# nianticlabs/mickey

Hardware: NVIDIA H100
Metric: image-pairs/sec @720x540 (higher is better)
Workload: dtype f16 operands / f32 accumulate (tensor core), f32 matcher+solver

## Files before the change

include/mickey_b200.h:

```cpp
#ifndef MICKEY_B200_H
#define MICKEY_B200_H

#ifdef __cplusplus
extern "C" {
#endif

typedef struct mk_handle mk_handle;

typedef struct mk_config {
  int embed_dim, depth, heads;
  int down_factor;
  int block_dims[4];
  int desc_dim;
  int use_softmax;
  int depth_sigmoid;
  float max_depth;
  int kp_pos_enc, dsc_pos_enc;
  int norm_dsc;
  float temperature;
  int use_dustbin;
  int it_matches, it_ransac;
  int num_sampled, num_corr, num_refine;
  float th_inlier, th_soft_inlier;
} mk_config;

int mk_create(int device, const mk_config* cfg, mk_handle** out);
int mk_destroy(mk_handle* h);
const char* mk_last_error(void);
const char* mk_version(void);
int mk_sizeof(const char* type);

int mk_set_tensor(mk_handle* h, const char* name, const void* ptr_dev, int dtype, long long numel);
int mk_finalize(mk_handle* h, int img_h, int img_w);

long long mk_workspace_bytes(mk_handle* h, int n_pairs, int img_h, int img_w);
long long mk_workspace_bytes_for(mk_handle* h, int n_img, int n_pairs, int img_h, int img_w);
long long mk_workspace_offset(mk_handle* h, const char* name, int n_pairs, int img_h, int img_w);

int mk_extract(mk_handle* h, const float* images_dev, int n_pairs, int img_h, int img_w, float* kps_dev,
               float* depth_dev, float* scr_dev, float* dsc_dev, void* ws_dev, long long ws_bytes, void* stream);

int mk_extract_u8(mk_handle* h, const unsigned char* images_u8_dev, int n_pairs, int img_h, int img_w, float* kps_dev,
                  float* depth_dev, float* scr_dev, float* dsc_dev, void* ws_dev, long long ws_bytes, void* stream);

int mk_extract_images(mk_handle* h, const float* images_dev, int n_img, int img_h, int img_w, float* kps_dev,
                      float* depth_dev, float* scr_dev, float* dsc_dev, void* ws_dev, long long ws_bytes, void* stream);
int mk_extract_images_u8(mk_handle* h, const unsigned char* images_u8_dev, int n_img, int img_h, int img_w, float* kps_dev,
                         float* depth_dev, float* scr_dev, float* dsc_dev, void* ws_dev, long long ws_bytes, void* stream);

long long mk_backbone_ws_bytes(mk_handle* h, int n_img, int img_h, int img_w);
int mk_backbone_features(mk_handle* h, const float* images_dev, int n_img, int img_h, int img_w, float* out_dev,
                         void* ws_dev, long long ws_bytes, void* stream);

int mk_match(mk_handle* h, int n_pairs, float* scores_dev, float* kp_scores_dev, float* final_scores_dev, long long nn_pitch,
             void* ws_dev, long long ws_bytes, void* stream);

int mk_solve_pose(mk_handle* h, const float* final_scores_dev, long long nn_pitch, const float* kps_dev, const float* depth_dev,
                  const float* K0_dev, const float* K1_dev, int n_pairs, int n_kpts, unsigned long long seed,
                  const int* outer_idx_dev, const int* inner_idx_dev, float* pose_dev, int* best_set_dev,
                  float* inlier_mask_dev, int* sampled_idx_out_dev, float* hyp_scores_out_dev, int* status_dev,
                  void* ws_dev, long long ws_bytes, void* stream);

long long mk_procrustes_ws_bytes(int B, int N, int it_matches, int it_ransac, int num_sampled);
int mk_procrustes_solve(const float* final_scores_dev, long long nn_pitch, const float* kps_dev, const float* depth_dev,
                        const float* K0_dev, const float* K1_dev, int B, int N, int it_matches, int it_ransac,
                        int num_sampled, int num_corr, int num_refine, float th_inlier, float th_soft_inlier,
                        unsigned long long seed, const int* outer_idx_dev, const int* inner_idx_dev, float* pose_dev,
                        int* best_set_dev, float* inlier_mask_dev, int* sampled_idx_out_dev, float* hyp_scores_out_dev,
                        int* status_dev, void* ws_dev, long long ws_bytes, void* stream);

#define MK_VCRE_POINTS 196
#define MK_MAPFREE_MAX_FRAMES 67108863
int mk_mapfree_frame_metrics(const double* q_est_dev, const double* t_est_dev, const double* q_gt_dev,
                             const double* t_gt_dev, const double* K_dev, const double* grid_dev, int P, int W, int H,
                             double* err_dev, void* stream);

int mk_forward(mk_handle* h, const float* images_dev, const float* K0_dev, const float* K1_dev, int n_pairs,
               int img_h, int img_w, unsigned long long seed, float* kps_dev, float* depth_dev, float* scr_dev,
               float* dsc_dev, float* scores_dev, float* kp_scores_dev, float* final_scores_dev, long long nn_pitch,
               float* pose_dev, int* best_set_dev, float* inlier_mask_dev, int* sampled_idx_out_dev, int* status_dev,
               void* ws_dev, long long ws_bytes, void* stream);

int mk_forward_u8(mk_handle* h, const unsigned char* images_u8_dev, const float* K0_dev, const float* K1_dev, int n_pairs,
                  int img_h, int img_w, unsigned long long seed, float* kps_dev, float* depth_dev, float* scr_dev,
                  float* dsc_dev, float* scores_dev, float* kp_scores_dev, float* final_scores_dev, long long nn_pitch,
                  float* pose_dev, int* best_set_dev, float* inlier_mask_dev, int* sampled_idx_out_dev, int* status_dev,
                  void* ws_dev, long long ws_bytes, void* stream);

int mk_forward_pairs(mk_handle* h, const float* kps0_dev, const float* depth0_dev, const float* scr0_dev, const float* dsc0_dev,
                     int n0, const float* kps1_dev, const float* depth1_dev, const float* scr1_dev, const float* dsc1_dev, int n1,
                     const int* idx0_dev, const int* idx1_dev, const float* K0_dev, const float* K1_dev, int n_pairs,
                     unsigned long long seed, float* kps_dev, float* depth_dev, float* scores_dev, float* kp_scores_dev,
                     float* final_scores_dev, long long nn_pitch, float* pose_dev, int* best_set_dev, float* inlier_mask_dev,
                     int* sampled_idx_out_dev, int* status_dev, void* ws_dev, long long ws_bytes, void* stream);

int mk_pose_to_submission(const float* pose_dev, int n_pairs, double* out_dev, void* stream);

int mk_mutual_matches(const float* scores_dev, long long nn_pitch, int B, int N, float min_conf, int* matches_dev,
                      float* match_scores_dev, int* count_dev, void* ws_dev, long long ws_bytes, void* stream);
long long mk_mutual_matches_ws_bytes(int B, int N);

#define MK_LOSS_STATUS_PRECHECK 16
#define MK_LOSS_STATUS_INNER 32
int mk_loss_search(const float* final_scores_dev, long long nn_pitch, const float* kps0_dev, const float* depth0_dev,
                   const float* kps1_dev, const float* depth1_dev, const float* K0_dev, const float* K1_dev, int B, int N,
                   int it_matches, int it_ransac, int n_sample, int n_corr, int n_ref, float th_ref, unsigned long long seed,
                   const int* outer_idx_dev, const int* inner_idx_dev, int* sampled_idx_out_dev, int* inner_idx_out_dev,
                   unsigned int* inliers_out_dev, int* status_dev, void* ws_dev, long long ws_bytes, void* stream);
long long mk_loss_search_ws_bytes(int B, int it_matches);
int mk_loss_gradient(const int* sampled_idx_dev, const float* loss_value_dev, const float* baseline_dev, const float* mask_topk_dev,
                     int B, int N, int it_matches, int n_sample, float* probs_grad_dev, void* ws_dev, long long ws_bytes,
                     void* stream);
long long mk_loss_gradient_ws_bytes(int B, int it_matches, int n_sample);

long long mk_dual_softmax_ws_bytes(int B, int N);
long long mk_dual_softmax_backward_ws_bytes(int B, int N);
int mk_dual_softmax(const float* dsc0_dev, const float* dsc1_dev, const float* scr0_dev, const float* scr1_dev,
                    const float* dustbin_dev, float temperature, int B, int N, int unit_norm, float* scores_dev,
                    float* kp_scores_dev, float* final_scores_dev, long long nn_pitch, float* lse_r_dev, float* lse_c_dev,
                    void* ws_dev, long long ws_bytes, void* stream);
int mk_dual_softmax_backward(const float* dsc0_dev, const float* dsc1_dev, const float* scr0_dev, const float* scr1_dev,
                             const float* dustbin_dev, float temperature, int B, int N, const float* lse_r_dev,
                             const float* lse_c_dev, const float* grad_scores_dev, long long gs_pitch, const float* grad_kp_dev,
                             long long gk_pitch, const float* grad_final_dev, long long gf_pitch, float* ddsc0_dev,
                             float* ddsc1_dev, float* dscr0_dev, float* dscr1_dev, float* ddustbin_dev, void* ws_dev,
                             long long ws_bytes, void* stream);

typedef struct mk_htr_layer {
  const float* q_proj; const float* k_proj; const float* v_proj; const float* merge; const float* mlp0; const float* mlp2;
  const float* norm1_w; const float* norm1_b; const float* norm2_w; const float* norm2_b;
} mk_htr_layer;
typedef struct mk_htr_layer_grads {
  float* q_proj; float* k_proj; float* v_proj; float* merge; float* mlp0; float* mlp2;
  float* norm1_w; float* norm1_b; float* norm2_w; float* norm2_b;
} mk_htr_layer_grads;
long long mk_head_transformer_ws_bytes(int B, int h, int w, int num_layers, int save);
long long mk_head_transformer_backward_ws_bytes(int B, int h, int w, int num_layers);
int mk_head_transformer(const float* x_dev, const float* pe_dev, int B, int h, int w, const mk_htr_layer* layers_host,
                        int num_layers, float* out_dev, int save, void* ws_dev, long long ws_bytes, void* stream);
int mk_head_transformer_backward(const void* saved_dev, const float* grad_out_dev, int B, int h, int w,
                                 const mk_htr_layer* layers_host, int num_layers, float* grad_x_dev,
                                 mk_htr_layer_grads* grads_host, void* ws_dev, long long ws_bytes, void* stream);

#define MK_RB_TRAIN 1
#define MK_RB_RELU 2
#define MK_RB_SAVE 4
#define MK_RB_BN 8
#define MK_RB_GRAD_X 1
#define MK_RB_GRAD_W1 2
#define MK_RB_GRAD_W2 4
#define MK_RB_GRAD_WSC 8
#define MK_RB_GRAD_BN1_W 16
#define MK_RB_GRAD_BN1_B 32
#define MK_RB_GRAD_BN2_W 64
#define MK_RB_GRAD_BN2_B 128
typedef struct mk_resblock_params {
  const float* w1; const float* w2; const float* wsc;
  const float* bn1_w; const float* bn1_b; float* bn1_mean; float* bn1_var;
  const float* bn2_w; const float* bn2_b; float* bn2_mean; float* bn2_var;
  float eps1, eps2, momentum1, momentum2;
} mk_resblock_params;
typedef struct mk_resblock_grads {
  float* dx; float* w1; float* w2; float* wsc; float* bn1_w; float* bn1_b; float* bn2_w; float* bn2_b;
} mk_resblock_grads;
long long mk_resblock_ws_bytes(int B, int h, int w, int cin, int cout);
long long mk_resblock_saved_bytes(int B, int h, int w, int cin, int cout);
long long mk_resblock_backward_ws_bytes(int B, int h, int w, int cin, int cout);
int mk_resblock_forward(const float* x_dev, const long long* x_strides_host, int B, int h, int w, int cin, int cout,
                        const mk_resblock_params* params_host, int flags, float* out_dev, void* saved_dev,
                        long long saved_bytes, void* ws_dev, long long ws_bytes, void* stream);
int mk_resblock_backward(const void* saved_dev, const float* grad_out_dev, const long long* g_strides_host,
                         const float* out_dev, int B, int h, int w, int cin, int cout, const mk_resblock_params* params_host,
                         int flags, int want, const mk_resblock_grads* grads_host, void* ws_dev, long long ws_bytes,
                         void* stream);

#define MK_HO_SCORE_SOFTMAX 0
#define MK_HO_SCORE_SIGMOID 1
#define MK_HO_OFFSET 2
#define MK_HO_DEPTH 3
#define MK_HO_DEPTH_SIGMOID 4
#define MK_HO_DESC_L2 5
long long mk_head_out_backward_ws_bytes(int kind, int B, int h, int w, int C);
int mk_head_out_forward(int kind, const float* x_dev, const long long* x_strides_host, int B, int C, int h, int w,
                        const float* weight_dev, const float* eps_dev, float temperature, float max_depth, float* out_dev,
                        float* norm_dev, void* stream);
int mk_head_out_backward(int kind, const float* x_dev, const long long* x_strides_host, int B, int C, int h, int w,
                         const float* weight_dev, float temperature, float max_depth, const float* out_dev,
                         const float* norm_dev, const float* grad_out_dev, float* grad_x_dev, float* grad_w_dev, void* ws_dev,
                         long long ws_bytes, void* stream);

int mk_set_seed(mk_handle* h, unsigned long long seed, void* stream);

long long mk_launch_count(mk_handle* h);
int mk_pdl_enabled(void);
int mk_profile_enable(mk_handle* h, int enable);
int mk_profile_read(mk_handle* h, char* buf, int buf_bytes);

typedef struct mk_gemm_args {
  int epi;
  int impl;
  const void* a; long long a_rows, a_cols, a_ld;
  const void* b; long long b_rows, b_cols, b_ld;
  int M, N, k_chunks, chunks_per_tap, num_taps;
  int tap_shift[9];
  int groups, a_row_group_off, a_col_group_off, a_col_base, b_row_group_off;
  int act;
  const float* bias; int bias_group_off;
  const float* gamma; const float* beta; int ln_group_off;
  float* out_f; long long out_f_ld, out_f_group_off;
  void* out_h; long long out_h_ld, out_h_group_off;
  const void* res_h; long long res_h_ld, res_h_group_off;
  const float* aux; int aux_group_mask;
  int pad_h2, pad_w2, tok_per_img;
  float eps;
  int n_valid; float inv_temp;
  const float* dustbin;
  float* part_row; float* part_col; int part_ld;
  const float* lse_r; const float* lse_c;
  const float* scr0; const float* scr1;
  float* scores; float* kp_scores; float* final_scores;
  float lse_bound;
  long long out_pitch;
} mk_gemm_args;

int mk_op_gemm(const mk_gemm_args* args, void* stream);
int mk_op_patch_gather(const float* img, void* patches_h, int n_img, int H, int W, int kpad, float* x_f,
                       const float* cls_pos, int D, void* stream);
int mk_op_ingest_u8(const unsigned char* img_u8, void* patches_h, int n_img, int H, int W, int kpad, float* x_f,
                    const float* cls_pos, int D, void* stream);
int mk_op_layernorm(const float* x, const float* w, const float* b, void* out_h, int rows, int D, float eps, int mode,
                    int gh, int gw, void* stream);
int mk_op_attention(const void* qkv_h, void* out_h, int n_img, int T, int D, int heads, int impl, void* stream);
int mk_op_linattn(const float* qkv_f, float* kv_part_f, float* kv_f, void* msg_h, int n_img, int G, int h2, int w2, float eps,
                  void* stream);
int mk_op_matcher_reduce(const float* part_row, const float* part_col, const float* dustbin, int B, int N, int part_ld,
                         float* lse_r, float* lse_c, void* stream);
int mk_op_sample(const float* final_scores, int B, int N, long long pitch, int IM, int n_sample, unsigned long long seed, void* ws,
                 long long ws_bytes, int* idx_out, int* status, void* stream);
long long mk_op_sample_workspace_bytes(int B, int IM);
int mk_op_kabsch(const double* H, double* R, int n, void* stream);

int mk_resblock_layout(int B, int h, int w, int cin, int cout, long long* saved_off, long long* bwd_off);
long long mk_op_conv_tf32_ws_bytes(int mode, int B, int h, int w, int cin, int cout, int taps);
int mk_op_conv_tf32(int mode, const float* a, const float* b, float* out, int B, int h, int w, int cin, int cout, int taps,
                    void* ws, long long ws_bytes, void* stream);

#ifdef __cplusplus
}
#endif
#endif
```

mickey_b200/_lib.py:

```python
from __future__ import annotations

import ctypes as C
import math
import os

import torch

_HERE = os.path.dirname(os.path.abspath(__file__))
LIB_PATH = os.path.join(_HERE, "_C", "libmickey_b200.so")


class MkConfig(C.Structure):
    _fields_ = [
        ("embed_dim", C.c_int), ("depth", C.c_int), ("heads", C.c_int),
        ("down_factor", C.c_int),
        ("block_dims", C.c_int * 4),
        ("desc_dim", C.c_int),
        ("use_softmax", C.c_int), ("depth_sigmoid", C.c_int), ("max_depth", C.c_float),
        ("kp_pos_enc", C.c_int), ("dsc_pos_enc", C.c_int), ("norm_dsc", C.c_int),
        ("temperature", C.c_float), ("use_dustbin", C.c_int),
        ("it_matches", C.c_int), ("it_ransac", C.c_int),
        ("num_sampled", C.c_int), ("num_corr", C.c_int), ("num_refine", C.c_int),
        ("th_inlier", C.c_float), ("th_soft_inlier", C.c_float),
    ]


class MkGemmArgs(C.Structure):
    _fields_ = [
        ("epi", C.c_int), ("impl", C.c_int),
        ("a", C.c_void_p), ("a_rows", C.c_longlong), ("a_cols", C.c_longlong), ("a_ld", C.c_longlong),
        ("b", C.c_void_p), ("b_rows", C.c_longlong), ("b_cols", C.c_longlong), ("b_ld", C.c_longlong),
        ("M", C.c_int), ("N", C.c_int), ("k_chunks", C.c_int), ("chunks_per_tap", C.c_int), ("num_taps", C.c_int),
        ("tap_shift", C.c_int * 9),
        ("groups", C.c_int), ("a_row_group_off", C.c_int), ("a_col_group_off", C.c_int), ("a_col_base", C.c_int),
        ("b_row_group_off", C.c_int),
        ("act", C.c_int),
        ("bias", C.c_void_p), ("bias_group_off", C.c_int),
        ("gamma", C.c_void_p), ("beta", C.c_void_p), ("ln_group_off", C.c_int),
        ("out_f", C.c_void_p), ("out_f_ld", C.c_longlong), ("out_f_group_off", C.c_longlong),
        ("out_h", C.c_void_p), ("out_h_ld", C.c_longlong), ("out_h_group_off", C.c_longlong),
        ("res_h", C.c_void_p), ("res_h_ld", C.c_longlong), ("res_h_group_off", C.c_longlong),
        ("aux", C.c_void_p), ("aux_group_mask", C.c_int),
        ("pad_h2", C.c_int), ("pad_w2", C.c_int), ("tok_per_img", C.c_int),
        ("eps", C.c_float),
        ("n_valid", C.c_int), ("inv_temp", C.c_float),
        ("dustbin", C.c_void_p),
        ("part_row", C.c_void_p), ("part_col", C.c_void_p), ("part_ld", C.c_int),
        ("lse_r", C.c_void_p), ("lse_c", C.c_void_p), ("scr0", C.c_void_p), ("scr1", C.c_void_p),
        ("scores", C.c_void_p), ("kp_scores", C.c_void_p), ("final_scores", C.c_void_p),
        ("lse_bound", C.c_float),
        ("out_pitch", C.c_longlong),
    ]


class MkHtrLayer(C.Structure):
    _fields_ = [(n, C.c_void_p) for n in ("q_proj", "k_proj", "v_proj", "merge", "mlp0", "mlp2",
                                          "norm1_w", "norm1_b", "norm2_w", "norm2_b")]


MkHtrLayerGrads = MkHtrLayer


class MkResblockParams(C.Structure):
    _fields_ = [(n, C.c_void_p) for n in ("w1", "w2", "wsc", "bn1_w", "bn1_b", "bn1_mean", "bn1_var",
                                          "bn2_w", "bn2_b", "bn2_mean", "bn2_var")] + \
               [(n, C.c_float) for n in ("eps1", "eps2", "momentum1", "momentum2")]


class MkResblockGrads(C.Structure):
    _fields_ = [(n, C.c_void_p) for n in ("dx", "w1", "w2", "wsc", "bn1_w", "bn1_b", "bn2_w", "bn2_b")]


EXPORTS = {
    "mk_create": (C.c_int, [C.c_int, C.POINTER(MkConfig), C.POINTER(C.c_void_p)]),
    "mk_destroy": (C.c_int, [C.c_void_p]),
    "mk_last_error": (C.c_char_p, []),
    "mk_version": (C.c_char_p, []),
    "mk_sizeof": (C.c_int, [C.c_char_p]),
    "mk_set_tensor": (C.c_int, [C.c_void_p, C.c_char_p, C.c_void_p, C.c_int, C.c_longlong]),
    "mk_finalize": (C.c_int, [C.c_void_p, C.c_int, C.c_int]),
    "mk_workspace_bytes": (C.c_longlong, [C.c_void_p, C.c_int, C.c_int, C.c_int]),
    "mk_workspace_offset": (C.c_longlong, [C.c_void_p, C.c_char_p, C.c_int, C.c_int, C.c_int]),
    "mk_extract": (C.c_int, [C.c_void_p, C.c_void_p, C.c_int, C.c_int, C.c_int, C.c_void_p, C.c_void_p, C.c_void_p,
                             C.c_void_p, C.c_void_p, C.c_longlong, C.c_void_p]),
    "mk_extract_u8": (C.c_int, [C.c_void_p, C.c_void_p, C.c_int, C.c_int, C.c_int, C.c_void_p, C.c_void_p, C.c_void_p,
                                C.c_void_p, C.c_void_p, C.c_longlong, C.c_void_p]),
    "mk_workspace_bytes_for": (C.c_longlong, [C.c_void_p, C.c_int, C.c_int, C.c_int, C.c_int]),
    "mk_extract_images": (C.c_int, [C.c_void_p, C.c_void_p, C.c_int, C.c_int, C.c_int, C.c_void_p, C.c_void_p, C.c_void_p,
                                    C.c_void_p, C.c_void_p, C.c_longlong, C.c_void_p]),
    "mk_extract_images_u8": (C.c_int, [C.c_void_p, C.c_void_p, C.c_int, C.c_int, C.c_int, C.c_void_p, C.c_void_p, C.c_void_p,
                                       C.c_void_p, C.c_void_p, C.c_longlong, C.c_void_p]),
    "mk_forward_pairs": (C.c_int, [C.c_void_p, C.c_void_p, C.c_void_p, C.c_void_p, C.c_void_p, C.c_int,
                                   C.c_void_p, C.c_void_p, C.c_void_p, C.c_void_p, C.c_int,
                                   C.c_void_p, C.c_void_p, C.c_void_p, C.c_void_p, C.c_int, C.c_ulonglong,
                                   C.c_void_p, C.c_void_p, C.c_void_p, C.c_void_p, C.c_void_p, C.c_longlong,
                                   C.c_void_p, C.c_void_p, C.c_void_p, C.c_void_p, C.c_void_p, C.c_void_p, C.c_longlong,
                                   C.c_void_p]),
    "mk_backbone_ws_bytes": (C.c_longlong, [C.c_void_p, C.c_int, C.c_int, C.c_int]),
    "mk_backbone_features": (C.c_int, [C.c_void_p, C.c_void_p, C.c_int, C.c_int, C.c_int, C.c_void_p, C.c_void_p,
                                       C.c_longlong, C.c_void_p]),
    "mk_match": (C.c_int, [C.c_void_p, C.c_int, C.c_void_p, C.c_void_p, C.c_void_p, C.c_longlong, C.c_void_p, C.c_longlong, C.c_void_p]),
    "mk_solve_pose": (C.c_int, [C.c_void_p, C.c_void_p, C.c_longlong, C.c_void_p, C.c_void_p, C.c_void_p, C.c_void_p, C.c_int, C.c_int,
                                C.c_ulonglong, C.c_void_p, C.c_void_p, C.c_void_p, C.c_void_p, C.c_void_p, C.c_void_p,
                                C.c_void_p, C.c_void_p, C.c_void_p, C.c_longlong, C.c_void_p]),
    "mk_procrustes_ws_bytes": (C.c_longlong, [C.c_int, C.c_int, C.c_int, C.c_int, C.c_int]),
    "mk_procrustes_solve": (C.c_int, [C.c_void_p, C.c_longlong, C.c_void_p, C.c_void_p, C.c_void_p, C.c_void_p, C.c_int,
                                      C.c_int, C.c_int, C.c_int, C.c_int, C.c_int, C.c_int, C.c_float, C.c_float,
                                      C.c_ulonglong, C.c_void_p, C.c_void_p, C.c_void_p, C.c_void_p, C.c_void_p,
                                      C.c_void_p, C.c_void_p, C.c_void_p, C.c_void_p, C.c_longlong, C.c_void_p]),
    "mk_mapfree_frame_metrics": (C.c_int, [C.c_void_p, C.c_void_p, C.c_void_p, C.c_void_p, C.c_void_p, C.c_void_p,
                                           C.c_int, C.c_int, C.c_int, C.c_void_p, C.c_void_p]),
    "mk_forward": (C.c_int, [C.c_void_p, C.c_void_p, C.c_void_p, C.c_void_p, C.c_int, C.c_int, C.c_int, C.c_ulonglong,
                             C.c_void_p, C.c_void_p, C.c_void_p, C.c_void_p, C.c_void_p, C.c_void_p, C.c_void_p, C.c_longlong,
                             C.c_void_p, C.c_void_p, C.c_void_p, C.c_void_p, C.c_void_p, C.c_void_p, C.c_longlong,
                             C.c_void_p]),
    "mk_forward_u8": (C.c_int, [C.c_void_p, C.c_void_p, C.c_void_p, C.c_void_p, C.c_int, C.c_int, C.c_int, C.c_ulonglong,
                                C.c_void_p, C.c_void_p, C.c_void_p, C.c_void_p, C.c_void_p, C.c_void_p, C.c_void_p, C.c_longlong,
                                C.c_void_p, C.c_void_p, C.c_void_p, C.c_void_p, C.c_void_p, C.c_void_p, C.c_longlong,
                                C.c_void_p]),
    "mk_mutual_matches": (C.c_int, [C.c_void_p, C.c_longlong, C.c_int, C.c_int, C.c_float, C.c_void_p, C.c_void_p,
                                    C.c_void_p, C.c_void_p, C.c_longlong, C.c_void_p]),
    "mk_mutual_matches_ws_bytes": (C.c_longlong, [C.c_int, C.c_int]),
    "mk_loss_search": (C.c_int, [C.c_void_p, C.c_longlong, C.c_void_p, C.c_void_p, C.c_void_p, C.c_void_p, C.c_void_p,
                                 C.c_void_p, C.c_int, C.c_int, C.c_int, C.c_int, C.c_int, C.c_int, C.c_int, C.c_float,
                                 C.c_ulonglong, C.c_void_p, C.c_void_p, C.c_void_p, C.c_void_p, C.c_void_p, C.c_void_p,
                                 C.c_void_p, C.c_longlong, C.c_void_p]),
    "mk_loss_search_ws_bytes": (C.c_longlong, [C.c_int, C.c_int]),
    "mk_loss_gradient": (C.c_int, [C.c_void_p, C.c_void_p, C.c_void_p, C.c_void_p, C.c_int, C.c_int, C.c_int, C.c_int,
                                   C.c_void_p, C.c_void_p, C.c_longlong, C.c_void_p]),
    "mk_loss_gradient_ws_bytes": (C.c_longlong, [C.c_int, C.c_int, C.c_int]),
    "mk_dual_softmax_ws_bytes": (C.c_longlong, [C.c_int, C.c_int]),
    "mk_dual_softmax_backward_ws_bytes": (C.c_longlong, [C.c_int, C.c_int]),
    "mk_dual_softmax": (C.c_int, [C.c_void_p, C.c_void_p, C.c_void_p, C.c_void_p, C.c_void_p, C.c_float, C.c_int, C.c_int,
                                  C.c_int, C.c_void_p, C.c_void_p, C.c_void_p, C.c_longlong, C.c_void_p, C.c_void_p,
                                  C.c_void_p, C.c_longlong, C.c_void_p]),
    "mk_dual_softmax_backward": (C.c_int, [C.c_void_p, C.c_void_p, C.c_void_p, C.c_void_p, C.c_void_p, C.c_float, C.c_int,
                                           C.c_int, C.c_void_p, C.c_void_p, C.c_void_p, C.c_longlong, C.c_void_p,
                                           C.c_longlong, C.c_void_p, C.c_longlong, C.c_void_p, C.c_void_p, C.c_void_p,
                                           C.c_void_p, C.c_void_p, C.c_void_p, C.c_longlong, C.c_void_p]),
    "mk_head_transformer_ws_bytes": (C.c_longlong, [C.c_int, C.c_int, C.c_int, C.c_int, C.c_int]),
    "mk_head_transformer_backward_ws_bytes": (C.c_longlong, [C.c_int, C.c_int, C.c_int, C.c_int]),
    "mk_head_transformer": (C.c_int, [C.c_void_p, C.c_void_p, C.c_int, C.c_int, C.c_int, C.POINTER(MkHtrLayer), C.c_int,
                                      C.c_void_p, C.c_int, C.c_void_p, C.c_longlong, C.c_void_p]),
    "mk_head_transformer_backward": (C.c_int, [C.c_void_p, C.c_void_p, C.c_int, C.c_int, C.c_int, C.POINTER(MkHtrLayer),
                                               C.c_int, C.c_void_p, C.POINTER(MkHtrLayerGrads), C.c_void_p, C.c_longlong,
                                               C.c_void_p]),
    "mk_resblock_ws_bytes": (C.c_longlong, [C.c_int, C.c_int, C.c_int, C.c_int, C.c_int]),
    "mk_resblock_saved_bytes": (C.c_longlong, [C.c_int, C.c_int, C.c_int, C.c_int, C.c_int]),
    "mk_resblock_backward_ws_bytes": (C.c_longlong, [C.c_int, C.c_int, C.c_int, C.c_int, C.c_int]),
    "mk_resblock_forward": (C.c_int, [C.c_void_p, C.POINTER(C.c_longlong), C.c_int, C.c_int, C.c_int, C.c_int, C.c_int,
                                      C.POINTER(MkResblockParams), C.c_int, C.c_void_p, C.c_void_p, C.c_longlong,
                                      C.c_void_p, C.c_longlong, C.c_void_p]),
    "mk_resblock_layout": (C.c_int, [C.c_int, C.c_int, C.c_int, C.c_int, C.c_int, C.POINTER(C.c_longlong),
                                     C.POINTER(C.c_longlong)]),
    "mk_resblock_backward": (C.c_int, [C.c_void_p, C.c_void_p, C.POINTER(C.c_longlong), C.c_void_p, C.c_int, C.c_int,
                                       C.c_int, C.c_int, C.c_int, C.POINTER(MkResblockParams), C.c_int, C.c_int,
                                       C.POINTER(MkResblockGrads), C.c_void_p, C.c_longlong, C.c_void_p]),
    "mk_head_out_backward_ws_bytes": (C.c_longlong, [C.c_int, C.c_int, C.c_int, C.c_int, C.c_int]),
    "mk_head_out_forward": (C.c_int, [C.c_int, C.c_void_p, C.POINTER(C.c_longlong), C.c_int, C.c_int, C.c_int, C.c_int,
                                      C.c_void_p, C.c_void_p, C.c_float, C.c_float, C.c_void_p, C.c_void_p, C.c_void_p]),
    "mk_head_out_backward": (C.c_int, [C.c_int, C.c_void_p, C.POINTER(C.c_longlong), C.c_int, C.c_int, C.c_int, C.c_int,
                                       C.c_void_p, C.c_float, C.c_float, C.c_void_p, C.c_void_p, C.c_void_p, C.c_void_p,
                                       C.c_void_p, C.c_void_p, C.c_longlong, C.c_void_p]),
    "mk_pose_to_submission": (C.c_int, [C.c_void_p, C.c_int, C.c_void_p, C.c_void_p]),
    "mk_launch_count": (C.c_longlong, [C.c_void_p]),
    "mk_pdl_enabled": (C.c_int, []),
    "mk_set_seed": (C.c_int, [C.c_void_p, C.c_ulonglong, C.c_void_p]),
    "mk_profile_enable": (C.c_int, [C.c_void_p, C.c_int]),
    "mk_profile_read": (C.c_int, [C.c_void_p, C.c_char_p, C.c_int]),
    "mk_op_gemm": (C.c_int, [C.POINTER(MkGemmArgs), C.c_void_p]),
    "mk_op_patch_gather": (C.c_int, [C.c_void_p, C.c_void_p, C.c_int, C.c_int, C.c_int, C.c_int, C.c_void_p, C.c_void_p,
                                     C.c_int, C.c_void_p]),
    "mk_op_ingest_u8": (C.c_int, [C.c_void_p, C.c_void_p, C.c_int, C.c_int, C.c_int, C.c_int, C.c_void_p, C.c_void_p,
                                  C.c_int, C.c_void_p]),
    "mk_op_layernorm": (C.c_int, [C.c_void_p, C.c_void_p, C.c_void_p, C.c_void_p, C.c_int, C.c_int, C.c_float, C.c_int,
                                  C.c_int, C.c_int, C.c_void_p]),
    "mk_op_attention": (C.c_int, [C.c_void_p, C.c_void_p, C.c_int, C.c_int, C.c_int, C.c_int, C.c_int, C.c_void_p]),
    "mk_op_linattn": (C.c_int, [C.c_void_p, C.c_void_p, C.c_void_p, C.c_void_p, C.c_int, C.c_int, C.c_int, C.c_int, C.c_float, C.c_void_p]),
    "mk_op_matcher_reduce": (C.c_int, [C.c_void_p, C.c_void_p, C.c_void_p, C.c_int, C.c_int, C.c_int, C.c_void_p, C.c_void_p, C.c_void_p]),
    "mk_op_sample": (C.c_int, [C.c_void_p, C.c_int, C.c_int, C.c_longlong, C.c_int, C.c_int, C.c_ulonglong, C.c_void_p, C.c_longlong,
                               C.c_void_p, C.c_void_p, C.c_void_p]),
    "mk_op_sample_workspace_bytes": (C.c_longlong, [C.c_int, C.c_int]),
    "mk_op_kabsch": (C.c_int, [C.c_void_p, C.c_void_p, C.c_int, C.c_void_p]),
    "mk_op_conv_tf32_ws_bytes": (C.c_longlong, [C.c_int, C.c_int, C.c_int, C.c_int, C.c_int, C.c_int, C.c_int]),
    "mk_op_conv_tf32": (C.c_int, [C.c_int, C.c_void_p, C.c_void_p, C.c_void_p, C.c_int, C.c_int, C.c_int, C.c_int, C.c_int,
                                  C.c_int, C.c_void_p, C.c_longlong, C.c_void_p]),
}

STRUCTS = {"mk_config": MkConfig, "mk_gemm_args": MkGemmArgs, "mk_htr_layer": MkHtrLayer,
           "mk_htr_layer_grads": MkHtrLayerGrads, "mk_resblock_params": MkResblockParams,
           "mk_resblock_grads": MkResblockGrads}

_lib = None


class MickeyB200Error(RuntimeError):
    pass


def load():
    global _lib
    if _lib is not None:
        return _lib
    if not os.path.exists(LIB_PATH):
        raise MickeyB200Error(
            f"{LIB_PATH} not found. Build it with `python -m mickey_b200.build` (needs nvcc; sm_90a only). "
            "mickey_b200 has no CPU or PyTorch fallback.")
    lib = C.CDLL(LIB_PATH)
    for name, (res, args) in EXPORTS.items():
        fn = getattr(lib, name)
        fn.restype = res
        fn.argtypes = args
    sizes = {name: (lib.mk_sizeof(name.encode()), C.sizeof(st)) for name, st in STRUCTS.items()}
    bad = [f"{name} {lib_size} vs {py_size}" for name, (lib_size, py_size) in sizes.items() if lib_size != py_size]
    if bad:
        raise MickeyB200Error("ctypes struct layout does not match the library (stale build?): " + ", ".join(bad))
    _lib = lib
    return lib


def check(rc: int, what: str = ""):
    if rc != 0:
        msg = load().mk_last_error().decode(errors="replace")
        raise MickeyB200Error(f"{what} failed (code {rc}): {msg}")


def ptr(t):
    return None if t is None else C.c_void_p(t.data_ptr())


def stream(dev=None):
    return C.c_void_p(torch.cuda.current_stream(dev).cuda_stream)


def workspace(nbytes, dev, what: str):
    nbytes = int(nbytes)
    if nbytes < 0:
        raise MickeyB200Error(f"{what} returned {nbytes}: {load().mk_last_error().decode(errors='replace')}")
    return torch.empty(max(nbytes, 1), dtype=torch.uint8, device=dev)


def pitched(t):
    B, N, _ = t.shape
    s0, s1, s2 = t.stride()
    if s2 == 1 and s1 >= N and (B == 1 or s0 == N * s1):
        return t, s1
    return t.contiguous(), N


class Handle:

    def __init__(self, device, cfg: MkConfig):
        self.lib = load()
        self.device = device
        h = C.c_void_p()
        check(self.lib.mk_create(device.index or 0, C.byref(cfg), C.byref(h)), "mk_create")
        self.h = h

    def __del__(self):
        try:
            if getattr(self, "h", None):
                self.lib.mk_destroy(self.h)
        except Exception:
            pass

    def register(self, name: str, t):
        assert t.is_contiguous() and t.device == self.device
        dt = {torch.float32: 0, torch.float16: 1}[t.dtype]
        check(self.lib.mk_set_tensor(self.h, name.encode(), ptr(t), dt, t.numel()), f"mk_set_tensor({name})")

    def workspace_view(self, ws, n_pairs: int, H: int, W: int, name: str, dtype, shape):
        off = self.lib.mk_workspace_offset(self.h, name.encode(), n_pairs, H, W)
        if off < 0:
            raise MickeyB200Error(self.lib.mk_last_error().decode())
        nbytes = math.prod(shape) * torch.empty((), dtype=dtype).element_size()
        return ws[off:off + nbytes].view(dtype).reshape(shape)
```

mickey_b200/csrc/engine.cu:

```cuda
#include "../../include/mickey_b200.h"
#include "gemm.h"
#include "ops.h"

#include <algorithm>
#include <cfloat>
#include <cstring>
#include <string>
#include <unordered_map>
#include <vector>

using namespace mk;

struct Tensor { const void* ptr; int dtype; long long numel; };

struct mk_handle {
  int device;
  mk_config cfg;
  std::unordered_map<std::string, Tensor> tensors;
  int geo_h = 0, geo_w = 0;
  bool finalized = false;
  unsigned long long* seed_dev = nullptr;
  long long launches = 0;
  bool profiling = false;
  struct ProfRec { std::string tag; cudaEvent_t e0, e1; };
  std::vector<ProfRec> prof;
};

namespace {

struct Geo {
  int H, W, gh, gw, N, T, h2, w2, per_img, n_img, n_pairs;
  long long M, Mp, R;
};

Geo make_geo(int n_img, int n_pairs, int H, int W) {
  Geo g;
  g.H = H; g.W = W; g.gh = H / 14; g.gw = W / 14;
  g.N = g.gh * g.gw; g.T = g.N + 1; g.h2 = g.gh + 2; g.w2 = g.gw + 2; g.per_img = g.h2 * g.w2;
  g.n_img = n_img; g.n_pairs = n_pairs;
  g.M = (long long)g.n_img * g.T; g.Mp = (long long)g.n_img * g.N; g.R = (long long)g.n_img * g.per_img;
  return g;
}

constexpr int KPAD = 640;
constexpr int G = 4;

struct Carver {
  uint8_t* base; size_t off = 0;
  explicit Carver(void* b) : base(reinterpret_cast<uint8_t*>(b)) {}
  template <typename T> T* take(size_t count) {
    off = (off + 255) & ~(size_t)255;
    T* p = base ? reinterpret_cast<T*>(base + off) : nullptr;
    off += count * sizeof(T);
    return p;
  }
};

struct SolverWs { void* samp_ws; int* idx; float* hyp_scores; float* hyp_Rt; int* status; int* best_hyp; };

void carve_solver(Carver& cv, int n_pairs, int it_matches, int it_ransac, int num_sampled, SolverWs& s) {
  const size_t streams = (size_t)n_pairs * it_matches;
  s.samp_ws = cv.take<uint8_t>(sampler_workspace_bytes(n_pairs, it_matches));
  s.idx = cv.take<int>(streams * num_sampled);
  s.hyp_scores = cv.take<float>(streams * it_ransac);
  s.hyp_Rt = cv.take<float>(streams * it_ransac * 12);
  s.status = cv.take<int>(SOLVER_COUNTER_BASE + n_pairs);
  s.best_hyp = cv.take<int>(n_pairs);
}

struct Workspace {
  __half* P; float* X; __half* XN; __half* QKV; __half* ATT; __half* H1;
  __half* F; __half *T1, *S1, *O1, *T2, *S2, *O2, *T3, *S3, *CAT, *MSG, *HM, *T4k, *S4k, *T4d;
  float *X32, *QKV32, *KV, *KVP, *Y4k, *Y4d;
  float* score_raw; __half* DSCX; float* nrm2; float* scr_copy;
  float *part_row, *part_col, *lse_r, *lse_c;
  SolverWs sol;
  size_t bytes;
};

void carve_backbone(Carver& cv, const mk_config& c, const Geo& g, Workspace& w) {
  const size_t D = c.embed_dim, M = g.M;
  w.P = cv.take<__half>((size_t)g.Mp * KPAD);
  w.X = cv.take<float>(M * D);
  w.XN = cv.take<__half>(M * D);
  w.QKV = cv.take<__half>(M * 3 * D);
  w.ATT = cv.take<__half>(M * D);
  w.H1 = cv.take<__half>(M * 4 * D);
}

size_t backbone_ws_bytes(const mk_config& c, const Geo& g) {
  Carver cv(nullptr);
  Workspace w;
  carve_backbone(cv, c, g, w);
  return (cv.off + 255) & ~(size_t)255;
}

Workspace carve(void* base, const mk_config& c, const Geo& g) {
  Workspace w;
  Carver cv(base);
  const int n_pairs = g.n_pairs;
  const size_t D = c.embed_dim, R = g.R;
  const size_t n_op = (size_t)std::max(g.n_img, 2 * g.n_pairs);
  const int* bd = c.block_dims;
  carve_backbone(cv, c, g, w);
  w.F = cv.take<__half>(R * D);
  w.T1 = cv.take<__half>(R * G * bd[0]); w.S1 = cv.take<__half>(R * G * bd[0]); w.O1 = cv.take<__half>(R * G * bd[0]);
  w.T2 = cv.take<__half>(R * G * bd[1]); w.S2 = cv.take<__half>(R * G * bd[1]); w.O2 = cv.take<__half>(R * G * bd[1]);
  w.T3 = cv.take<__half>(R * G * bd[2]); w.S3 = cv.take<__half>(R * G * bd[2]);
  w.CAT = cv.take<__half>(R * G * 256); w.MSG = cv.take<__half>(R * G * 128); w.HM = cv.take<__half>(R * G * 256);
  w.T4k = cv.take<__half>(R * 3 * bd[3]); w.S4k = cv.take<__half>(R * 3 * bd[3]); w.T4d = cv.take<__half>(R * c.desc_dim);
  w.X32 = cv.take<float>(R * G * 128); w.QKV32 = cv.take<float>(R * G * 384);
  w.KV = cv.take<float>((size_t)g.n_img * G * 8 * 272);
  w.KVP = cv.take<float>((size_t)g.n_img * G * linattn_kv_chunks(g.h2, g.w2) * 8 * 272);
  w.Y4k = cv.take<float>(R * 3 * bd[3]); w.Y4d = cv.take<float>(R * c.desc_dim);
  w.score_raw = cv.take<float>((size_t)g.n_img * g.N);
  w.DSCX = cv.take<__half>(n_op * g.N * 384);
  w.nrm2 = cv.take<float>((size_t)g.n_img * g.N);
  w.scr_copy = cv.take<float>(n_op * g.N);
  const size_t npad = (size_t)ceil_div(g.N, 128) * 128;
  w.part_row = cv.take<float>((size_t)n_pairs * (npad / 64) * npad * 2); w.part_col = cv.take<float>((size_t)n_pairs * (npad / 32) * npad * 2);
  w.lse_r = cv.take<float>((size_t)n_pairs * npad); w.lse_c = cv.take<float>((size_t)n_pairs * npad);
  carve_solver(cv, n_pairs, c.it_matches, c.it_ransac, c.num_sampled, w.sol);
  w.bytes = cv.off + 256;
  return w;
}

struct Lookup {
  mk_handle* h; bool ok = true;
  const void* get(const std::string& name, int dtype, long long numel) {
    auto it = h->tensors.find(name);
    if (it == h->tensors.end()) { set_last_error("missing tensor '%s'", name.c_str()); ok = false; return nullptr; }
    if (it->second.dtype != dtype || it->second.numel != numel) {
      set_last_error("tensor '%s': expected dtype %d numel %lld, got dtype %d numel %lld", name.c_str(), dtype, numel,
                     it->second.dtype, it->second.numel);
      ok = false; return nullptr;
    }
    return it->second.ptr;
  }
  const float* f(const std::string& n, long long numel) { return reinterpret_cast<const float*>(get(n, 0, numel)); }
  const __half* hh(const std::string& n, long long numel) { return reinterpret_cast<const __half*>(get(n, 1, numel)); }
};

GemmParams base_params(long long M, int N, int K) {
  GemmParams p;
  memset(&p, 0, sizeof(p));
  p.M = (int)M; p.N = N; p.k_chunks = K / 64; p.chunks_per_tap = p.k_chunks; p.num_taps = 1; p.groups = 1;
  return p;
}

void set_conv_taps(GemmParams& p, int cin, int w2, bool three) {
  p.chunks_per_tap = cin / 64;
  if (three) {
    p.num_taps = 9;
    for (int ky = 0; ky < 3; ++ky)
      for (int kx = 0; kx < 3; ++kx) p.tap_shift[ky * 3 + kx] = (ky - 1) * w2 + (kx - 1);
  } else {
    p.num_taps = 1; p.tap_shift[0] = 0;
  }
  p.k_chunks = p.num_taps * p.chunks_per_tap;
}

struct ProfScope {
  mk_handle* h; cudaStream_t st; int slot = -1;
  ProfScope(mk_handle* h_, const char* tag, cudaStream_t st_) : h(h_), st(st_) {
    if (!h || !h->profiling) return;
    mk_handle::ProfRec r;
    r.tag = tag;
    if (cudaEventCreate(&r.e0) != cudaSuccess || cudaEventCreate(&r.e1) != cudaSuccess) return;
    cudaEventRecord(r.e0, st);
    h->prof.push_back(r);
    slot = (int)h->prof.size() - 1;
  }
  ~ProfScope() { if (slot >= 0) cudaEventRecord(h->prof[slot].e1, st); }
};

int gemm(mk_handle* h, const char* tag, int epi, const void* a, long long a_rows, long long a_cols, const void* b,
         long long b_rows, long long b_cols, const GemmParams& p, cudaStream_t st) {
  GemmOperand A{a, a_rows, a_cols, a_cols}, B{b, b_rows, b_cols, b_cols};
  h->launches++;
  ProfScope ps(h, tag, st);
  return launch_gemm(epi, A, B, p, st);
}
#define MK_KERNEL(tag, call) do { ProfScope ps_(h, tag, st); h->launches++; MK_TRY(call); } while (0)

int run_backbone(mk_handle* h, const void* images, int img_fmt, const Geo& g, Workspace& w, cudaStream_t st) {
  const mk_config& c = h->cfg;
  const int H = g.H, W = g.W;
  const int D = c.embed_dim;
  Lookup L{h};
  if (img_fmt == 1)
    MK_KERNEL("vit.ingest_u8", ingest_u8(reinterpret_cast<const uint8_t*>(images), w.P, g.n_img, H, W, KPAD, w.X, L.f("patch.clspos", D), D, st));
  else
    MK_KERNEL("vit.patch_gather", patch_gather(reinterpret_cast<const float*>(images), w.P, g.n_img, H, W, KPAD, w.X, L.f("patch.clspos", D), D, st));
  {
    GemmParams p = base_params(g.Mp, D, KPAD);
    p.aux = L.f("patch.posb", (long long)g.N * D); p.tok_per_img = g.N; p.out_f = w.X; p.out_f_ld = D;
    const __half* wt = L.hh("patch.w", (long long)D * KPAD);
    if (!L.ok) return MK_ERR_MISSING_TENSOR;
    MK_TRY(gemm(h, "vit.patch_embed", EPI_PATCH, w.P, g.Mp, KPAD, wt, D, KPAD, p, st));
  }
  const bool fuse_ln = gemm_resid_ln_supported((int)g.M, D, D / 64) && gemm_resid_ln_supported((int)g.M, D, 4 * D / 64);
  for (int i = 0; i < c.depth; ++i) {
    const std::string b = "blk" + std::to_string(i) + ".";
    const float *ln1w = L.f(b + "ln1.w", D), *ln1b = L.f(b + "ln1.b", D), *ln2w = L.f(b + "ln2.w", D), *ln2b = L.f(b + "ln2.b", D);
    const __half *wqkv = L.hh(b + "qkv.w", 3LL * D * D), *wproj = L.hh(b + "proj.w", (long long)D * D);
    const __half *wfc1 = L.hh(b + "fc1.w", 4LL * D * D), *wfc2 = L.hh(b + "fc2.w", 4LL * D * D);
    const float *bqkv = L.f(b + "qkv.b", 3 * D), *bproj = L.f(b + "proj.b", D), *bfc1 = L.f(b + "fc1.b", 4 * D), *bfc2 = L.f(b + "fc2.b", D);
    const float *ls1 = L.f(b + "ls1", D), *ls2 = L.f(b + "ls2", D);
    if (!L.ok) return MK_ERR_MISSING_TENSOR;
    if (i == 0 || !fuse_ln) MK_KERNEL("vit.layernorm", layernorm(w.X, ln1w, ln1b, w.XN, (int)g.M, D, 1e-6f, 0, 0, 0, st));
    { GemmParams p = base_params(g.M, 3 * D, D); p.bias = bqkv; p.out_h = w.QKV; p.out_h_ld = 3 * D;
      MK_TRY(gemm(h, "vit.qkv", EPI_STORE_H, w.XN, g.M, D, wqkv, 3 * D, D, p, st)); }
    MK_KERNEL("vit.attention", attention_dispatch(w.QKV, w.ATT, g.n_img, g.T, D, c.heads, 0, st));
    { GemmParams p = base_params(g.M, D, D); p.bias = bproj; p.gamma = ls1; p.out_f = w.X; p.out_f_ld = D;
      if (fuse_ln) { p.aux = ln2w; p.beta = ln2b; p.out_h = w.XN; p.out_h_ld = D; p.eps = 1e-6f; }
      MK_TRY(gemm(h, "vit.proj", fuse_ln ? EPI_RESID_LN : EPI_RESID_F, w.ATT, g.M, D, wproj, D, D, p, st)); }
    if (!fuse_ln) MK_KERNEL("vit.layernorm", layernorm(w.X, ln2w, ln2b, w.XN, (int)g.M, D, 1e-6f, 0, 0, 0, st));
    { GemmParams p = base_params(g.M, 4 * D, D); p.bias = bfc1; p.act = ACT_GELU; p.out_h = w.H1; p.out_h_ld = 4 * D;
      MK_TRY(gemm(h, "vit.fc1", EPI_STORE_H, w.XN, g.M, D, wfc1, 4 * D, D, p, st)); }
    { GemmParams p = base_params(g.M, D, 4 * D); p.bias = bfc2; p.gamma = ls2; p.out_f = w.X; p.out_f_ld = D;
      const bool fuse_next = fuse_ln && i + 1 < c.depth;
      if (fuse_next) {
        const std::string nb = "blk" + std::to_string(i + 1) + ".";
        p.aux = L.f(nb + "ln1.w", D); p.beta = L.f(nb + "ln1.b", D); p.out_h = w.XN; p.out_h_ld = D; p.eps = 1e-6f;
        if (!L.ok) return MK_ERR_MISSING_TENSOR;
      }
      MK_TRY(gemm(h, "vit.fc2", fuse_next ? EPI_RESID_LN : EPI_RESID_F, w.H1, g.M, 4 * D, wfc2, D, 4 * D, p, st)); }
  }
  return MK_OK;
}

int run_extract(mk_handle* h, const void* images, int img_fmt, const Geo& g, float* kps, float* depth, float* scr,
                float* dsc, Workspace& w, cudaStream_t st) {
  const mk_config& c = h->cfg;
  const int D = c.embed_dim;
  Lookup L{h};
  MK_TRY(run_backbone(h, images, img_fmt, g, w, st));
  MK_CUDA_CHECK(cudaMemsetAsync(w.F, 0, (size_t)g.R * D * sizeof(__half), st));
  MK_KERNEL("vit.layernorm", layernorm(w.X, L.f("norm.w", D), L.f("norm.b", D), w.F, (int)g.M, D, 1e-6f, 1, g.gh, g.gw, st));
  if (!L.ok) return MK_ERR_MISSING_TENSOR;

  const int* bd = c.block_dims;
  struct Rb { const char* name; const __half* in; int cin; int in_goff; __half *T, *S, *O; int cout; };
  const Rb rbs[3] = {{"rb1", w.F, D, 0, w.T1, w.S1, w.O1, bd[0]},
                     {"rb2", w.O1, bd[0], bd[0], w.T2, w.S2, w.O2, bd[1]},
                     {"rb3", w.O2, bd[1], bd[1], w.T3, w.S3, nullptr, bd[2]}};
  if (bd[2] != 128) { set_last_error("KP_HEADS.BLOCKS_DIM[2] must be 128 (transformer width)"); return MK_ERR_UNSUPPORTED; }
  for (int r = 0; r < 3; ++r) {
    const Rb& rb = rbs[r];
    const std::string n = std::string(rb.name) + ".";
    const long long in_cols = (r == 0) ? D : (long long)G * rb.cin;
    const __half *wc1 = L.hh(n + "c1.w", (long long)G * rb.cout * 9 * rb.cin), *wsc = L.hh(n + "sc.w", (long long)G * rb.cout * rb.cin);
    const __half* wc2 = L.hh(n + "c2.w", (long long)G * rb.cout * 9 * rb.cout);
    const float *b1 = L.f(n + "c1.b", G * rb.cout), *b2 = L.f(n + "c2.b", G * rb.cout);
    if (!L.ok) return MK_ERR_MISSING_TENSOR;
    {
      GemmParams p = base_params(g.R, rb.cout, 64); set_conv_taps(p, rb.cin, g.w2, true);
      p.groups = G; p.a_col_group_off = rb.in_goff; p.b_row_group_off = rb.cout; p.bias = b1; p.bias_group_off = rb.cout;
      p.act = ACT_RELU; p.pad_h2 = g.h2; p.pad_w2 = g.w2; p.out_h = rb.T; p.out_h_ld = (long long)G * rb.cout; p.out_h_group_off = rb.cout;
      MK_TRY(gemm(h, "head.conv3x3", EPI_CONV, rb.in, g.R, in_cols, wc1, (long long)G * rb.cout, 9LL * rb.cin, p, st));
    }
    {
      GemmParams p = base_params(g.R, rb.cout, 64); set_conv_taps(p, rb.cin, g.w2, false);
      p.groups = G; p.a_col_group_off = rb.in_goff; p.b_row_group_off = rb.cout;
      p.out_h = rb.S; p.out_h_ld = (long long)G * rb.cout; p.out_h_group_off = rb.cout;
      MK_TRY(gemm(h, "head.conv1x1", EPI_CONV, rb.in, g.R, in_cols, wsc, (long long)G * rb.cout, rb.cin, p, st));
    }
    {
      GemmParams p = base_params(g.R, rb.cout, 64); set_conv_taps(p, rb.cout, g.w2, true);
      p.groups = G; p.a_col_group_off = rb.cout; p.b_row_group_off = rb.cout; p.bias = b2; p.bias_group_off = rb.cout;
      p.res_h = rb.S; p.res_h_ld = (long long)G * rb.cout; p.res_h_group_off = rb.cout;
      p.act = ACT_RELU; p.pad_h2 = g.h2; p.pad_w2 = g.w2;
      if (r < 2) { p.out_h = rb.O; p.out_h_ld = (long long)G * rb.cout; p.out_h_group_off = rb.cout; }
      else {
        p.out_h = w.CAT; p.out_h_ld = G * 256; p.out_h_group_off = 256;
        p.out_f = w.X32; p.out_f_ld = G * 128; p.out_f_group_off = 128;
        p.aux = L.f("head.pe", (long long)g.per_img * 128);
        p.aux_group_mask = (c.kp_pos_enc ? 0x7 : 0) | (c.dsc_pos_enc ? 0x8 : 0);
        if (!L.ok) return MK_ERR_MISSING_TENSOR;
      }
      MK_TRY(gemm(h, "head.conv3x3", EPI_CONV, rb.T, g.R, (long long)G * rb.cout, wc2, (long long)G * rb.cout, 9LL * rb.cout, p, st));
    }
  }
  for (int l = 0; l < 3; ++l) {
    const std::string n = "att" + std::to_string(l) + ".";
    const __half *wqkv = L.hh(n + "qkv.w", (long long)G * 384 * 128), *wmerge = L.hh(n + "merge.w", (long long)G * 128 * 128);
    const __half *wm0 = L.hh(n + "mlp0.w", (long long)G * 256 * 256), *wm2 = L.hh(n + "mlp2.w", (long long)G * 128 * 256);
    const float *n1w = L.f(n + "n1.w", G * 128), *n1b = L.f(n + "n1.b", G * 128), *n2w = L.f(n + "n2.w", G * 128), *n2b = L.f(n + "n2.b", G * 128);
    if (!L.ok) return MK_ERR_MISSING_TENSOR;
    { GemmParams p = base_params(g.R, 384, 128); p.groups = G; p.a_col_group_off = 256; p.b_row_group_off = 384;
      p.out_f = w.QKV32; p.out_f_ld = G * 384; p.out_f_group_off = 384;
      MK_TRY(gemm(h, "head.att.qkv", EPI_STORE_F, w.CAT, g.R, G * 256, wqkv, G * 384, 128, p, st)); }
    { ProfScope ps_(h, "head.att.kv", st); h->launches += 2; MK_TRY(linattn_kv(w.QKV32, w.KVP, w.KV, g.n_img, G, g.h2, g.w2, st)); }
    MK_KERNEL("head.att.msg", linattn_msg(w.QKV32, w.KV, w.MSG, g.n_img, G, g.h2, g.w2, 1e-6f, st));
    { GemmParams p = base_params(g.R, 128, 128); p.groups = G; p.a_col_group_off = 128; p.b_row_group_off = 128;
      p.gamma = n1w; p.beta = n1b; p.ln_group_off = 128; p.eps = 1e-5f;
      p.out_h = w.CAT + 128; p.out_h_ld = G * 256; p.out_h_group_off = 256;
      MK_TRY(gemm(h, "head.att.merge_ln", EPI_LN, w.MSG, g.R, G * 128, wmerge, G * 128, 128, p, st)); }
    { GemmParams p = base_params(g.R, 256, 256); p.groups = G; p.a_col_group_off = 256; p.b_row_group_off = 256; p.act = ACT_RELU;
      p.out_h = w.HM; p.out_h_ld = G * 256; p.out_h_group_off = 256;
      MK_TRY(gemm(h, "head.att.mlp0", EPI_STORE_H, w.CAT, g.R, G * 256, wm0, G * 256, 256, p, st)); }
    { GemmParams p = base_params(g.R, 128, 256); p.groups = G; p.a_col_group_off = 256; p.b_row_group_off = 128;
      p.gamma = n2w; p.beta = n2b; p.ln_group_off = 128; p.eps = 1e-5f;
      p.out_f = w.X32; p.out_f_ld = G * 128; p.out_f_group_off = 128;
      p.out_h = w.CAT; p.out_h_ld = G * 256; p.out_h_group_off = 256;
      if (l == 2) { p.pad_h2 = g.h2; p.pad_w2 = g.w2; }
      MK_TRY(gemm(h, "head.att.mlp2_ln", EPI_LN, w.HM, g.R, G * 256, wm2, G * 128, 256, p, st)); }
  }
  {
    const int co = bd[3];
    const __half *wc1 = L.hh("rb4k.c1.w", 3LL * co * 9 * 128), *wsc = L.hh("rb4k.sc.w", 3LL * co * 128), *wc2 = L.hh("rb4k.c2.w", 3LL * co * 9 * co);
    const float *b1 = L.f("rb4k.c1.b", 3 * co), *b2 = L.f("rb4k.c2.b", 3 * co);
    if (!L.ok) return MK_ERR_MISSING_TENSOR;
    { GemmParams p = base_params(g.R, co, 64); set_conv_taps(p, 128, g.w2, true);
      p.groups = 3; p.a_col_group_off = 256; p.b_row_group_off = co; p.bias = b1; p.bias_group_off = co; p.act = ACT_RELU;
      p.pad_h2 = g.h2; p.pad_w2 = g.w2; p.out_h = w.T4k; p.out_h_ld = 3 * co; p.out_h_group_off = co;
      MK_TRY(gemm(h, "head.conv3x3", EPI_CONV, w.CAT, g.R, G * 256, wc1, 3 * co, 9 * 128, p, st)); }
    { GemmParams p = base_params(g.R, co, 64); set_conv_taps(p, 128, g.w2, false);
      p.groups = 3; p.a_col_group_off = 256; p.b_row_group_off = co; p.out_h = w.S4k; p.out_h_ld = 3 * co; p.out_h_group_off = co;
      MK_TRY(gemm(h, "head.conv1x1", EPI_CONV, w.CAT, g.R, G * 256, wsc, 3 * co, 128, p, st)); }
    { GemmParams p = base_params(g.R, co, 64); set_conv_taps(p, co, g.w2, true);
      p.groups = 3; p.a_col_group_off = co; p.b_row_group_off = co; p.bias = b2; p.bias_group_off = co; p.act = ACT_RELU;
      p.res_h = w.S4k; p.res_h_ld = 3 * co; p.res_h_group_off = co; p.pad_h2 = g.h2; p.pad_w2 = g.w2;
      p.out_f = w.Y4k; p.out_f_ld = 3 * co; p.out_f_group_off = co;
      MK_TRY(gemm(h, "head.conv3x3", EPI_CONV, w.T4k, g.R, 3 * co, wc2, 3 * co, 9 * co, p, st)); }
  }
  {
    const int co = c.desc_dim;
    const __half *wc1 = L.hh("rb4d.c1.w", (long long)co * 9 * 128), *wc2 = L.hh("rb4d.c2.w", (long long)co * 9 * co);
    const float *b1 = L.f("rb4d.c1.b", co), *b2 = L.f("rb4d.c2.b", co);
    if (co != 128) { set_last_error("DSC_HEAD.LAST_DIM must be 128"); return MK_ERR_UNSUPPORTED; }
    if (!L.ok) return MK_ERR_MISSING_TENSOR;
    { GemmParams p = base_params(g.R, co, 64); set_conv_taps(p, 128, g.w2, true);
      p.a_col_base = 3 * 256; p.bias = b1; p.act = ACT_RELU; p.pad_h2 = g.h2; p.pad_w2 = g.w2; p.out_h = w.T4d; p.out_h_ld = co;
      MK_TRY(gemm(h, "head.conv3x3", EPI_CONV, w.CAT, g.R, G * 256, wc1, co, 9 * 128, p, st)); }
    { GemmParams p = base_params(g.R, co, 64); set_conv_taps(p, co, g.w2, true);
      p.bias = b2; p.act = ACT_NONE; p.res_h = w.CAT + 3 * 256; p.res_h_ld = G * 256;
      p.pad_h2 = g.h2; p.pad_w2 = g.w2; p.out_f = w.Y4d; p.out_f_ld = co;
      MK_TRY(gemm(h, "head.conv3x3", EPI_CONV, w.T4d, g.R, co, wc2, co, 9 * co, p, st)); }
  }
  { ProfScope ps_(h, "head.kp_out", st); h->launches += 2;
    MK_TRY(kp_head_out(w.Y4k, L.f("out.depth.w", bd[3]), L.f("out.xy.w", 2 * bd[3]), L.f("out.score.w", bd[3]), depth, kps,
                       w.score_raw, scr, g.n_img, g.gh, g.gw, c.depth_sigmoid, c.max_depth, (float)c.down_factor, c.use_softmax, st)); }
  if (!L.ok) return MK_ERR_MISSING_TENSOR;
  if (bd[3] != 64) { set_last_error("KP_HEADS.BLOCKS_DIM[3] must be 64"); return MK_ERR_UNSUPPORTED; }
  MK_KERNEL("head.desc_out", desc_out(w.Y4d, dsc, w.DSCX, w.nrm2, g.n_img, g.gh, g.gw, c.norm_dsc, st));
  MK_CUDA_CHECK(cudaMemcpyAsync(w.scr_copy, scr, (size_t)g.n_img * g.N * sizeof(float), cudaMemcpyDeviceToDevice, st));
  return MK_OK;
}

int run_match(mk_handle* h, int n_pairs, int N, float* scores, float* kp_scores, float* final_scores, long long nn_pitch,
              Workspace& w, cudaStream_t st) {
  const mk_config& c = h->cfg;
  Lookup L{h};
  const float* dust = c.use_dustbin ? L.f("dustbin", 1) : nullptr;
  if (!L.ok) return MK_ERR_MISSING_TENSOR;
  if (!final_scores || ((scores == nullptr) != (kp_scores == nullptr))) {
    set_last_error("mk_match: final_scores is required; scores and kp_scores are given together or both NULL (lean mode)");
    return MK_ERR_INVALID;
  }
  MK_TRY(resolve_pitch(nn_pitch, N, "mk_match: nn_pitch"));
  const bool tma_ok = nn_pitch % 4 == 0 && reinterpret_cast<uintptr_t>(final_scores) % 16 == 0 &&
                      (!scores || (reinterpret_cast<uintptr_t>(scores) % 16 == 0 && reinterpret_cast<uintptr_t>(kp_scores) % 16 == 0));
  const float inv_t = 1.0f / c.temperature;
  const __half* A0 = w.DSCX;
  const __half* A1 = w.DSCX + (size_t)n_pairs * N * 384;
  const long long rows = (long long)n_pairs * N;
  const int npad = ceil_div(N, 128) * 128;
  auto mp = [&]() {
    GemmParams p = base_params(N, N, 384);
    p.groups = n_pairs; p.a_row_group_off = N; p.b_row_group_off = N; p.n_valid = N; p.inv_temp = inv_t; p.part_ld = npad;
    return p;
  };
  { GemmParams p = mp(); p.part_row = reinterpret_cast<float2*>(w.part_row); p.part_col = reinterpret_cast<float2*>(w.part_col);
    p.lse_bound = (c.norm_dsc && inv_t <= 25.0f) ? 1.001f : 0.0f;
    MK_TRY(gemm(h, "match.lse", EPI_LSE, A0, rows, 384, A1, rows, 384, p, st)); }
  MK_KERNEL("match.reduce", matcher_lse_reduce(w.part_row, w.part_col, dust, n_pairs, N, npad, w.lse_r, w.lse_c, st));
  { GemmParams p = mp(); p.lse_r = w.lse_r; p.lse_c = w.lse_c; p.scr0 = w.scr_copy; p.scr1 = w.scr_copy + (size_t)n_pairs * N;
    p.scores = scores; p.kp_scores = kp_scores; p.final_scores = final_scores; p.out_pitch = nn_pitch; p.out_tma = tma_ok ? 1 : 0;
    MK_TRY(gemm(h, "match.dual_softmax", EPI_DUAL, A0, rows, 384, A1, rows, 384, p, st)); }
  return MK_OK;
}

int run_solve(mk_handle* h, const RansacParams& rp, const float* final_scores, long long nn_pitch, const float* kps,
              const float* depth, const float* K0, const float* K1, int n_pairs, int N, const int* outer_idx,
              const int* inner_idx, float* pose, int* best_set, float* inl_mask, int* sampled_out, float* hyp_scores_out,
              int* status_out, const SolverWs& s, cudaStream_t st) {
  MK_CUDA_CHECK(cudaMemsetAsync(s.status, 0, (size_t)(SOLVER_COUNTER_BASE + n_pairs) * sizeof(int), st));
  const size_t n_idx = (size_t)n_pairs * rp.it_matches * rp.n_sample;
  const int* idx = outer_idx;
  if (!idx) {
    { ProfScope ps_(h, "solve.sample_outer", st); if (h) h->launches += 4;
      MK_TRY(sample_outer(final_scores, n_pairs, N, nn_pitch, rp.it_matches, rp.n_sample, rp.seed, s.samp_ws, s.idx, s.status, st)); }
    idx = s.idx;
  }
  const float* kps0 = kps;
  const float* kps1 = kps + (size_t)n_pairs * 2 * N;
  const float* d0 = depth;
  const float* d1 = depth + (size_t)n_pairs * N;
  int* bs = best_set ? best_set : s.best_hyp;
  { ProfScope ps_(h, "solve.ransac", st); if (h) h->launches += 1;
    MK_TRY(ransac_solve(final_scores, nn_pitch, kps0, d0, kps1, d1, K0, K1, n_pairs, N, rp, idx, inner_idx, s.hyp_scores,
                        s.hyp_Rt, s.status, pose, bs, inl_mask, best_set ? s.best_hyp : nullptr, st)); }
  if (sampled_out) MK_CUDA_CHECK(cudaMemcpyAsync(sampled_out, idx, n_idx * sizeof(int), cudaMemcpyDeviceToDevice, st));
  if (hyp_scores_out)
    MK_CUDA_CHECK(cudaMemcpyAsync(hyp_scores_out, s.hyp_scores, (size_t)n_pairs * rp.it_matches * rp.it_ransac * sizeof(float),
                                  cudaMemcpyDeviceToDevice, st));
  if (status_out) MK_CUDA_CHECK(cudaMemcpyAsync(status_out, s.status, sizeof(int), cudaMemcpyDeviceToDevice, st));
  return MK_OK;
}

int run_solve_handle(mk_handle* h, const float* final_scores, long long nn_pitch, const float* kps, const float* depth,
                     const float* K0, const float* K1, int n_pairs, int N, unsigned long long seed, const int* outer_idx,
                     const int* inner_idx, float* pose, int* best_set, float* inl_mask, int* sampled_out,
                     float* hyp_scores_out, int* status_out, Workspace& w, cudaStream_t st) {
  const mk_config& c = h->cfg;
  RansacParams rp{c.it_matches, c.it_ransac, c.num_sampled, c.num_corr, c.num_refine, c.th_inlier, c.th_soft_inlier, h->seed_dev};
  MK_TRY(resolve_pitch(nn_pitch, N, "mk_solve_pose: nn_pitch"));
  if (seed != 0) MK_TRY(seed_set(h->seed_dev, seed, st));
  MK_TRY(run_solve(h, rp, final_scores, nn_pitch, kps, depth, K0, K1, n_pairs, N, outer_idx, inner_idx, pose, best_set,
                   inl_mask, sampled_out, hyp_scores_out, status_out, w.sol, st));
  return seed_advance(h->seed_dev, st);
}

constexpr int PROC_MAX_SAMPLED = 2048, PROC_SAMPLED_STEP = 256, PROC_MAX_GRID = 65535;

bool procrustes_sizes_ok(int B, int N, int it_matches, int it_ransac, int num_sampled) {
  return B >= 1 && B <= PROC_MAX_GRID && N >= 1 && (long long)N * N <= 0x7fffffffLL && it_matches >= 1 &&
         it_matches <= PROC_MAX_GRID && it_ransac >= 1 && (long long)it_matches * it_ransac <= 0x7fffffffLL &&
         (long long)B * it_matches <= 0x7fffffffLL && num_sampled >= PROC_SAMPLED_STEP && num_sampled <= PROC_MAX_SAMPLED &&
         num_sampled % PROC_SAMPLED_STEP == 0;
}

size_t procrustes_carve(void* ws, int B, int it_matches, int it_ransac, int num_sampled, SolverWs& s,
                        unsigned long long** seed_word) {
  Carver cv(ws);
  carve_solver(cv, B, it_matches, it_ransac, num_sampled, s);
  *seed_word = cv.take<unsigned long long>(1);
  return (cv.off + 255) & ~(size_t)255;
}

int check_ws(mk_handle* h, int n_img, int n_pairs, int H, int W, void* ws, long long ws_bytes, Workspace& out) {
  if (!h || !h->finalized) { set_last_error("handle not finalized"); return MK_ERR_INVALID; }
  MK_CUDA_CHECK(cudaSetDevice(h->device));
  if (H != h->geo_h || W != h->geo_w) {
    set_last_error("geometry %dx%d does not match the finalized geometry %dx%d", H, W, h->geo_h, h->geo_w);
    return MK_ERR_INVALID;
  }
  const Geo g = make_geo(n_img, n_pairs, H, W);
  out = carve(ws, h->cfg, g);
  if (!ws || (long long)out.bytes > ws_bytes) {
    set_last_error("workspace too small: need %zu bytes, got %lld", out.bytes, ws_bytes);
    return MK_ERR_INVALID;
  }
  return MK_OK;
}

}

extern "C" {

const char* mk_last_error(void) { return mk::last_error(); }
const char* mk_version(void) { return "mickey_b200 0.1.0 (sm_90a)"; }
int mk_sizeof(const char* type) {
  const std::unordered_map<std::string, int> sizes = {
      {"mk_config", sizeof(mk_config)}, {"mk_gemm_args", sizeof(mk_gemm_args)}, {"mk_htr_layer", sizeof(mk_htr_layer)},
      {"mk_htr_layer_grads", sizeof(mk_htr_layer_grads)}, {"mk_resblock_params", sizeof(mk_resblock_params)},
      {"mk_resblock_grads", sizeof(mk_resblock_grads)}};
  const auto it = type ? sizes.find(type) : sizes.end();
  return it == sizes.end() ? -1 : it->second;
}

int mk_create(int device, const mk_config* cfg, mk_handle** out) {
  if (!cfg || !out) { set_last_error("null argument"); return MK_ERR_INVALID; }
  if (cfg->embed_dim != cfg->heads * 64 || cfg->embed_dim % 128) {
    set_last_error("unsupported backbone: embed_dim %d heads %d", cfg->embed_dim, cfg->heads);
    return MK_ERR_UNSUPPORTED;
  }
  int count = 0;
  if (cudaGetDeviceCount(&count) != cudaSuccess || device < 0 || device >= count) {
    set_last_error("CUDA device %d not available (an H100 is required; there is no CPU path)", device);
    return MK_ERR_CUDA;
  }
  cudaDeviceProp prop;
  MK_CUDA_CHECK(cudaGetDeviceProperties(&prop, device));
  if (prop.major != 9 || prop.minor != 0) {
    set_last_error("device %d is sm_%d%d; this library contains sm_90a code only", device, prop.major, prop.minor);
    return MK_ERR_UNSUPPORTED;
  }
  mk_handle* h = new mk_handle();
  h->device = device;
  h->cfg = *cfg;
  MK_CUDA_CHECK(cudaSetDevice(device));
  MK_CUDA_CHECK(cudaMalloc(&h->seed_dev, sizeof(unsigned long long)));
  const unsigned long long s0 = 0x243F6A8885A308D3ull;
  MK_CUDA_CHECK(cudaMemcpy(h->seed_dev, &s0, sizeof(s0), cudaMemcpyHostToDevice));
  *out = h;
  return MK_OK;
}

int mk_destroy(mk_handle* h) {
  if (h) {
    if (h->seed_dev) cudaFree(h->seed_dev);
    for (auto& r : h->prof) { cudaEventDestroy(r.e0); cudaEventDestroy(r.e1); }
    delete h;
  }
  return MK_OK;
}

int mk_set_tensor(mk_handle* h, const char* name, const void* ptr, int dtype, long long numel) {
  if (!h || !name || !ptr) { set_last_error("null argument"); return MK_ERR_INVALID; }
  h->tensors[name] = Tensor{ptr, dtype, numel};
  return MK_OK;
}

int mk_finalize(mk_handle* h, int H, int W) {
  if (!h) return MK_ERR_INVALID;
  if (H < 14 * 7 || W < 14 * 7) { set_last_error("image %dx%d too small (3-px border mask needs >= 7 cells)", H, W); return MK_ERR_INVALID; }
  h->geo_h = H; h->geo_w = W; h->finalized = true;
  return MK_OK;
}

long long mk_workspace_bytes(mk_handle* h, int n_pairs, int H, int W) {
  if (!h) return -1;
  return (long long)carve(nullptr, h->cfg, make_geo(2 * n_pairs, n_pairs, H, W)).bytes;
}

long long mk_workspace_bytes_for(mk_handle* h, int n_img, int n_pairs, int H, int W) {
  if (!h || n_img < 0 || n_pairs < 0) return -1;
  const Geo g = make_geo(n_img, n_pairs, H, W);
  return (long long)carve(nullptr, h->cfg, g).bytes;
}

int mk_extract(mk_handle* h, const float* images, int n_pairs, int H, int W, float* kps, float* depth, float* scr,
               float* dsc, void* ws, long long ws_bytes, void* stream) {
  Workspace w;
  MK_TRY(check_ws(h, 2 * n_pairs, n_pairs, H, W, ws, ws_bytes, w));
  return run_extract(h, images, 0, make_geo(2 * n_pairs, n_pairs, H, W), kps, depth, scr, dsc, w, (cudaStream_t)stream);
}

int mk_extract_u8(mk_handle* h, const unsigned char* images, int n_pairs, int H, int W, float* kps, float* depth, float* scr,
                  float* dsc, void* ws, long long ws_bytes, void* stream) {
  Workspace w;
  MK_TRY(check_ws(h, 2 * n_pairs, n_pairs, H, W, ws, ws_bytes, w));
  return run_extract(h, images, 1, make_geo(2 * n_pairs, n_pairs, H, W), kps, depth, scr, dsc, w, (cudaStream_t)stream);
}

static int extract_images_any(mk_handle* h, const void* images, int img_fmt, int n_img, int H, int W, float* kps, float* depth,
                              float* scr, float* dsc, void* ws, long long ws_bytes, void* stream) {
  if (n_img <= 0 || !images || !kps || !depth || !scr || !dsc) {
    set_last_error("mk_extract_images: n_img %d must be positive and every pointer non-NULL", n_img);
    return MK_ERR_INVALID;
  }
  Workspace w;
  MK_TRY(check_ws(h, n_img, 0, H, W, ws, ws_bytes, w));
  return run_extract(h, images, img_fmt, make_geo(n_img, 0, H, W), kps, depth, scr, dsc, w, (cudaStream_t)stream);
}

int mk_extract_images(mk_handle* h, const float* images, int n_img, int H, int W, float* kps, float* depth, float* scr,
                      float* dsc, void* ws, long long ws_bytes, void* stream) {
  return extract_images_any(h, images, 0, n_img, H, W, kps, depth, scr, dsc, ws, ws_bytes, stream);
}

int mk_extract_images_u8(mk_handle* h, const unsigned char* images, int n_img, int H, int W, float* kps, float* depth, float* scr,
                         float* dsc, void* ws, long long ws_bytes, void* stream) {
  return extract_images_any(h, images, 1, n_img, H, W, kps, depth, scr, dsc, ws, ws_bytes, stream);
}

long long mk_backbone_ws_bytes(mk_handle* h, int n_img, int H, int W) {
  if (!h || n_img < 1 || H < 98 || W < 98 || H % 14 || W % 14) return -1;
  return (long long)backbone_ws_bytes(h->cfg, make_geo(n_img, 0, H, W));
}

int mk_backbone_features(mk_handle* h, const float* images, int n_img, int H, int W, float* out, void* ws, long long ws_bytes,
                         void* stream) {
  if (!h || !images || !out || !ws) { set_last_error("mk_backbone_features: null argument"); return MK_ERR_INVALID; }
  if (n_img < 1) { set_last_error("mk_backbone_features: n_img %d must be positive", n_img); return MK_ERR_INVALID; }
  if (H < 98 || W < 98 || H % 14 || W % 14) {
    set_last_error("mk_backbone_features: image %dx%d must be multiples of 14 and at least 98", H, W);
    return MK_ERR_INVALID;
  }
  if (!h->finalized) { set_last_error("mk_backbone_features: handle not finalized"); return MK_ERR_INVALID; }
  if (H != h->geo_h || W != h->geo_w) {
    set_last_error("mk_backbone_features: geometry %dx%d does not match the finalized geometry %dx%d", H, W, h->geo_h, h->geo_w);
    return MK_ERR_INVALID;
  }
  const Geo g = make_geo(n_img, 0, H, W);
  const size_t need = backbone_ws_bytes(h->cfg, g);
  if ((long long)need > ws_bytes) {
    set_last_error("mk_backbone_features: workspace too small: need %zu bytes, got %lld", need, ws_bytes);
    return MK_ERR_INVALID;
  }
  MK_CUDA_CHECK(cudaSetDevice(h->device));
  const int D = h->cfg.embed_dim;
  Lookup L{h};
  const float *nw = L.f("norm.w", D), *nb = L.f("norm.b", D);
  if (!L.ok) return MK_ERR_MISSING_TENSOR;
  Workspace w;
  Carver cv(ws);
  carve_backbone(cv, h->cfg, g, w);
  cudaStream_t st = (cudaStream_t)stream;
  MK_TRY(run_backbone(h, images, 0, g, w, st));
  MK_KERNEL("vit.layernorm_cm", layernorm_channel_major(w.X, nw, nb, out, n_img, g.N, D, 1e-6f, st));
  return MK_OK;
}

int mk_match(mk_handle* h, int n_pairs, float* scores, float* kp_scores, float* final_scores, long long nn_pitch, void* ws,
             long long ws_bytes, void* stream) {
  Workspace w;
  MK_TRY(check_ws(h, 2 * n_pairs, n_pairs, h ? h->geo_h : 0, h ? h->geo_w : 0, ws, ws_bytes, w));
  const Geo g = make_geo(2 * n_pairs, n_pairs, h->geo_h, h->geo_w);
  return run_match(h, n_pairs, g.N, scores, kp_scores, final_scores, nn_pitch, w, (cudaStream_t)stream);
}

int mk_solve_pose(mk_handle* h, const float* final_scores, long long nn_pitch, const float* kps, const float* depth, const float* K0,
                  const float* K1, int n_pairs, int n_kpts, unsigned long long seed, const int* outer_idx,
                  const int* inner_idx, float* pose, int* best_set, float* inl_mask, int* sampled_out,
                  float* hyp_scores_out, int* status, void* ws, long long ws_bytes, void* stream) {
  Workspace w;
  MK_TRY(check_ws(h, 2 * n_pairs, n_pairs, h ? h->geo_h : 0, h ? h->geo_w : 0, ws, ws_bytes, w));
  const Geo g = make_geo(2 * n_pairs, n_pairs, h->geo_h, h->geo_w);
  if (n_kpts != g.N) { set_last_error("n_kpts %d does not match the geometry (%d)", n_kpts, g.N); return MK_ERR_INVALID; }
  return run_solve_handle(h, final_scores, nn_pitch, kps, depth, K0, K1, n_pairs, n_kpts, seed, outer_idx, inner_idx, pose,
                          best_set, inl_mask, sampled_out, hyp_scores_out, status, w, (cudaStream_t)stream);
}

long long mk_procrustes_ws_bytes(int B, int N, int it_matches, int it_ransac, int num_sampled) {
  if (!procrustes_sizes_ok(B, N, it_matches, it_ransac, num_sampled)) return -1;
  SolverWs s;
  unsigned long long* seed_word;
  return (long long)procrustes_carve(nullptr, B, it_matches, it_ransac, num_sampled, s, &seed_word);
}

int mk_procrustes_solve(const float* final_scores, long long nn_pitch, const float* kps, const float* depth, const float* K0,
                        const float* K1, int B, int N, int it_matches, int it_ransac, int num_sampled, int num_corr,
                        int num_refine, float th_inlier, float th_soft_inlier, unsigned long long seed, const int* outer_idx,
                        const int* inner_idx, float* pose, int* best_set, float* inl_mask, int* sampled_out,
                        float* hyp_scores_out, int* status, void* ws, long long ws_bytes, void* stream) {
  if (!final_scores || !kps || !depth || !K0 || !K1 || !pose || !ws) {
    set_last_error("mk_procrustes_solve: final_scores, kps, depth, K0, K1, pose and the workspace must be non-NULL");
    return MK_ERR_INVALID;
  }
  if (!procrustes_sizes_ok(B, N, it_matches, it_ransac, num_sampled) || num_corr != 3 || num_refine < 0 ||
      !(th_inlier > 0.f && th_inlier <= FLT_MAX) || !(th_soft_inlier > 0.f && th_soft_inlier <= FLT_MAX)) {
    set_last_error("mk_procrustes_solve: need 1 <= B <= %d, N >= 1 with N*N < 2^31, 1 <= it_matches <= %d, it_ransac >= 1, "
                   "it_matches*it_ransac and B*it_matches < 2^31, num_sampled a multiple of %d up to %d, num_corr 3, "
                   "num_refine >= 0 and finite positive thresholds (got B %d N %d it_matches %d it_ransac %d num_sampled %d "
                   "num_corr %d num_refine %d th_inlier %g th_soft_inlier %g)", PROC_MAX_GRID, PROC_MAX_GRID,
                   PROC_SAMPLED_STEP, PROC_MAX_SAMPLED, B, N, it_matches, it_ransac, num_sampled, num_corr, num_refine,
                   (double)th_inlier, (double)th_soft_inlier);
    return MK_ERR_INVALID;
  }
  MK_TRY(resolve_pitch(nn_pitch, N, "mk_procrustes_solve: nn_pitch"));
  SolverWs s;
  unsigned long long* seed_word;
  const size_t need = procrustes_carve(ws, B, it_matches, it_ransac, num_sampled, s, &seed_word);
  if ((long long)need > ws_bytes) {
    set_last_error("mk_procrustes_solve: workspace of %lld bytes, %zu needed", ws_bytes, need);
    return MK_ERR_INVALID;
  }
  cudaStream_t st = (cudaStream_t)stream;
  const RansacParams rp{it_matches, it_ransac, num_sampled, num_corr, num_refine, th_inlier, th_soft_inlier, seed_word};
  MK_TRY(seed_set(seed_word, seed, st));
  return run_solve(nullptr, rp, final_scores, nn_pitch, kps, depth, K0, K1, B, N, outer_idx, inner_idx, pose, best_set,
                   inl_mask, sampled_out, hyp_scores_out, status, s, st);
}

static int forward_any(mk_handle* h, const void* images, int img_fmt, const float* K0, const float* K1, int n_pairs, int H, int W,
                       unsigned long long seed, float* kps, float* depth, float* scr, float* dsc, float* scores,
                       float* kp_scores, float* final_scores, long long nn_pitch, float* pose, int* best_set, float* inl_mask,
                       int* sampled_out, int* status, void* ws, long long ws_bytes, void* stream) {
  Workspace w;
  MK_TRY(check_ws(h, 2 * n_pairs, n_pairs, H, W, ws, ws_bytes, w));
  const Geo g = make_geo(2 * n_pairs, n_pairs, H, W);
  cudaStream_t st = (cudaStream_t)stream;
  MK_TRY(run_extract(h, images, img_fmt, g, kps, depth, scr, dsc, w, st));
  MK_TRY(run_match(h, n_pairs, g.N, scores, kp_scores, final_scores, nn_pitch, w, st));
  return run_solve_handle(h, final_scores, nn_pitch, kps, depth, K0, K1, n_pairs, g.N, seed, nullptr, nullptr, pose, best_set,
                          inl_mask, sampled_out, nullptr, status, w, st);
}

int mk_forward(mk_handle* h, const float* images, const float* K0, const float* K1, int n_pairs, int H, int W,
               unsigned long long seed, float* kps, float* depth, float* scr, float* dsc, float* scores,
               float* kp_scores, float* final_scores, long long nn_pitch, float* pose, int* best_set, float* inl_mask,
               int* sampled_out, int* status, void* ws, long long ws_bytes, void* stream) {
  return forward_any(h, images, 0, K0, K1, n_pairs, H, W, seed, kps, depth, scr, dsc, scores, kp_scores, final_scores, nn_pitch,
                     pose, best_set, inl_mask, sampled_out, status, ws, ws_bytes, stream);
}

int mk_forward_u8(mk_handle* h, const unsigned char* images, const float* K0, const float* K1, int n_pairs, int H, int W,
                  unsigned long long seed, float* kps, float* depth, float* scr, float* dsc, float* scores,
                  float* kp_scores, float* final_scores, long long nn_pitch, float* pose, int* best_set, float* inl_mask,
                  int* sampled_out, int* status, void* ws, long long ws_bytes, void* stream) {
  return forward_any(h, images, 1, K0, K1, n_pairs, H, W, seed, kps, depth, scr, dsc, scores, kp_scores, final_scores, nn_pitch,
                     pose, best_set, inl_mask, sampled_out, status, ws, ws_bytes, stream);
}

int mk_forward_pairs(mk_handle* h, const float* kps0, const float* depth0, const float* scr0, const float* dsc0, int n0,
                     const float* kps1, const float* depth1, const float* scr1, const float* dsc1, int n1, const int* idx0,
                     const int* idx1, const float* K0, const float* K1, int n_pairs, unsigned long long seed, float* kps, float* depth,
                     float* scores, float* kp_scores, float* final_scores, long long nn_pitch, float* pose, int* best_set,
                     float* inl_mask, int* sampled_out, int* status, void* ws, long long ws_bytes, void* stream) {
  if (n_pairs <= 0 || n0 <= 0 || n1 <= 0 || !kps0 || !depth0 || !scr0 || !dsc0 || !kps1 || !depth1 || !scr1 || !dsc1 || !idx0 ||
      !idx1 || !K0 || !K1 || !kps || !depth || !pose) {
    set_last_error("mk_forward_pairs: n_pairs %d, bank sizes %d / %d must be positive; banks, indices, K, kps, depth and pose "
                   "must be non-NULL", n_pairs, n0, n1);
    return MK_ERR_INVALID;
  }
  Workspace w;
  MK_TRY(check_ws(h, 0, n_pairs, h ? h->geo_h : 0, h ? h->geo_w : 0, ws, ws_bytes, w));
  const Geo g = make_geo(0, n_pairs, h->geo_h, h->geo_w);
  cudaStream_t st = (cudaStream_t)stream;
  const BankView b0{kps0, depth0, scr0, dsc0, idx0, n0}, b1{kps1, depth1, scr1, dsc1, idx1, n1};
  MK_KERNEL("pairs.gather", bank_gather(b0, b1, n_pairs, g.N, w.DSCX, kps, depth, w.scr_copy, st));
  MK_TRY(run_match(h, n_pairs, g.N, scores, kp_scores, final_scores, nn_pitch, w, st));
  MK_TRY(run_solve_handle(h, final_scores, nn_pitch, kps, depth, K0, K1, n_pairs, g.N, seed, nullptr, nullptr, pose, best_set,
                          inl_mask, sampled_out, nullptr, status, w, st));
  MK_KERNEL("pairs.index_check", bank_index_check(b0, b1, n_pairs, pose, status, st));
  return MK_OK;
}

int mk_pose_to_submission(const float* pose, int n_pairs, double* out, void* stream) {
  if (!pose || !out || n_pairs < 0) { set_last_error("null argument"); return MK_ERR_INVALID; }
  return pose_to_submission(pose, n_pairs, out, (cudaStream_t)stream);
}

long long mk_mutual_matches_ws_bytes(int B, int N) { return mutual_matches_ws_bytes(B, N); }
int mk_mutual_matches(const float* scores, long long nn_pitch, int B, int N, float min_conf, int* matches, float* match_scores,
                      int* count, void* ws, long long ws_bytes, void* stream) {
  return mutual_matches(scores, nn_pitch, B, N, min_conf, matches, match_scores, count, ws, ws_bytes, (cudaStream_t)stream);
}

long long mk_loss_search_ws_bytes(int B, int IM) { return (B > 0 && IM > 0) ? loss_search_ws_bytes(B, IM) : 0; }
int mk_loss_search(const float* final_scores, long long nn_pitch, const float* kps0, const float* depth0, const float* kps1,
                   const float* depth1, const float* K0, const float* K1, int B, int N, int it_matches, int it_ransac,
                   int n_sample, int n_corr, int n_ref, float th_ref, unsigned long long seed, const int* outer_idx,
                   const int* inner_idx, int* sampled_idx_out, int* inner_idx_out, unsigned int* inliers_out, int* status,
                   void* ws, long long ws_bytes, void* stream) {
  return loss_search(final_scores, nn_pitch, kps0, depth0, kps1, depth1, K0, K1, B, N, it_matches, it_ransac, n_sample, n_corr,
                     n_ref, th_ref, seed, outer_idx, inner_idx, sampled_idx_out, inner_idx_out, inliers_out, status, ws, ws_bytes,
                     (cudaStream_t)stream);
}
long long mk_loss_gradient_ws_bytes(int B, int it_matches, int n_sample) { return loss_gradient_ws_bytes(B, it_matches, n_sample); }
int mk_loss_gradient(const int* sampled_idx, const float* loss_value, const float* baseline, const float* mask_topk, int B, int N,
                     int it_matches, int n_sample, float* probs_grad, void* ws, long long ws_bytes, void* stream) {
  return loss_gradient(sampled_idx, loss_value, baseline, mask_topk, B, N, it_matches, n_sample, probs_grad, ws, ws_bytes,
                       (cudaStream_t)stream);
}

long long mk_launch_count(mk_handle* h) { return h ? h->launches : -1; }

int mk_pdl_enabled(void) { return pdl_enabled() ? 1 : 0; }

int mk_set_seed(mk_handle* h, unsigned long long seed, void* stream) {
  if (!h) return MK_ERR_INVALID;
  return seed_set(h->seed_dev, seed, (cudaStream_t)stream);
}

long long mk_workspace_offset(mk_handle* h, const char* name, int n_pairs, int H, int W) {
  if (!h || !name) return -1;
  const Geo g = make_geo(2 * n_pairs, n_pairs, H, W);
  uint8_t* base = reinterpret_cast<uint8_t*>(0x1000);
  Workspace w = carve(base, h->cfg, g);
  const std::unordered_map<std::string, const void*> m = {
      {"P", w.P}, {"X", w.X}, {"XN", w.XN}, {"QKV", w.QKV}, {"ATT", w.ATT}, {"H1", w.H1}, {"F", w.F}, {"T1", w.T1},
      {"S1", w.S1}, {"O1", w.O1}, {"T2", w.T2}, {"S2", w.S2}, {"O2", w.O2}, {"T3", w.T3}, {"S3", w.S3}, {"CAT", w.CAT},
      {"MSG", w.MSG}, {"HM", w.HM}, {"T4k", w.T4k}, {"S4k", w.S4k}, {"T4d", w.T4d}, {"X32", w.X32}, {"QKV32", w.QKV32},
      {"KV", w.KV}, {"Y4k", w.Y4k}, {"Y4d", w.Y4d}, {"score_raw", w.score_raw}, {"DSCX", w.DSCX}, {"nrm2", w.nrm2},
      {"lse_r", w.lse_r}, {"lse_c", w.lse_c}, {"idx", w.sol.idx}, {"hyp_scores", w.sol.hyp_scores},
      {"hyp_Rt", w.sol.hyp_Rt}};
  auto it = m.find(name);
  if (it == m.end()) { set_last_error("unknown workspace buffer '%s'", name); return -1; }
  return (long long)(reinterpret_cast<const uint8_t*>(it->second) - base);
}

int mk_profile_enable(mk_handle* h, int enable) {
  if (!h) return MK_ERR_INVALID;
  for (auto& r : h->prof) { cudaEventDestroy(r.e0); cudaEventDestroy(r.e1); }
  h->prof.clear();
  h->profiling = enable != 0;
  return MK_OK;
}

int mk_profile_read(mk_handle* h, char* buf, int buf_bytes) {
  if (!h || !buf || buf_bytes <= 0) return MK_ERR_INVALID;
  MK_CUDA_CHECK(cudaDeviceSynchronize());
  std::vector<std::string> order;
  std::unordered_map<std::string, std::pair<int, double>> acc;
  for (auto& r : h->prof) {
    float ms = 0.f;
    if (cudaEventElapsedTime(&ms, r.e0, r.e1) != cudaSuccess) continue;
    if (!acc.count(r.tag)) order.push_back(r.tag);
    acc[r.tag].first += 1;
    acc[r.tag].second += ms;
  }
  std::string out;
  char line[256];
  for (auto& t : order) {
    snprintf(line, sizeof(line), "%s %d %.6f\n", t.c_str(), acc[t].first, acc[t].second);
    out += line;
  }
  if ((int)out.size() + 1 > buf_bytes) { set_last_error("profile buffer too small"); return MK_ERR_INVALID; }
  memcpy(buf, out.c_str(), out.size() + 1);
  return MK_OK;
}

int mk_op_gemm(const mk_gemm_args* a, void* stream) {
  if (!a) return MK_ERR_INVALID;
  GemmParams p;
  memset(&p, 0, sizeof(p));
  p.M = a->M; p.N = a->N; p.k_chunks = a->k_chunks; p.chunks_per_tap = a->chunks_per_tap; p.num_taps = a->num_taps;
  for (int i = 0; i < 9; ++i) p.tap_shift[i] = a->tap_shift[i];
  p.groups = a->groups; p.a_row_group_off = a->a_row_group_off; p.a_col_group_off = a->a_col_group_off;
  p.a_col_base = a->a_col_base; p.b_row_group_off = a->b_row_group_off; p.act = a->act;
  p.bias = a->bias; p.bias_group_off = a->bias_group_off; p.gamma = a->gamma; p.beta = a->beta; p.ln_group_off = a->ln_group_off;
  p.out_f = a->out_f; p.out_f_ld = a->out_f_ld; p.out_f_group_off = a->out_f_group_off;
  p.out_h = (__half*)a->out_h; p.out_h_ld = a->out_h_ld; p.out_h_group_off = a->out_h_group_off;
  p.res_h = (const __half*)a->res_h; p.res_h_ld = a->res_h_ld; p.res_h_group_off = a->res_h_group_off;
  p.aux = a->aux; p.aux_group_mask = a->aux_group_mask; p.pad_h2 = a->pad_h2; p.pad_w2 = a->pad_w2; p.tok_per_img = a->tok_per_img;
  p.eps = a->eps; p.n_valid = a->n_valid; p.inv_temp = a->inv_temp; p.dustbin = a->dustbin;
  p.part_row = reinterpret_cast<float2*>(a->part_row); p.part_col = reinterpret_cast<float2*>(a->part_col); p.part_ld = a->part_ld;
  p.lse_r = a->lse_r; p.lse_c = a->lse_c; p.scr0 = a->scr0; p.scr1 = a->scr1; p.lse_bound = a->lse_bound;
  p.out_pitch = a->out_pitch > 0 ? a->out_pitch : a->n_valid;
  p.out_tma = (a->final_scores && p.out_pitch % 4 == 0 && reinterpret_cast<uintptr_t>(a->final_scores) % 16 == 0 &&
               (!a->scores || (reinterpret_cast<uintptr_t>(a->scores) % 16 == 0 && reinterpret_cast<uintptr_t>(a->kp_scores) % 16 == 0))) ? 1 : 0;
  p.scores = a->scores; p.kp_scores = a->kp_scores; p.final_scores = a->final_scores;
  GemmOperand A{a->a, a->a_rows, a->a_cols, a->a_ld}, B{a->b, a->b_rows, a->b_cols, a->b_ld};
  return launch_gemm(a->epi, A, B, p, (cudaStream_t)stream, a->impl);
}

int mk_op_patch_gather(const float* img, void* P, int n_img, int H, int W, int kpad, float* X, const float* cls_pos,
                       int D, void* stream) {
  return patch_gather(img, P, n_img, H, W, kpad, X, cls_pos, D, (cudaStream_t)stream);
}
int mk_op_ingest_u8(const unsigned char* img, void* P, int n_img, int H, int W, int kpad, float* X, const float* cls_pos,
                    int D, void* stream) {
  return ingest_u8(img, P, n_img, H, W, kpad, X, cls_pos, D, (cudaStream_t)stream);
}
int mk_op_layernorm(const float* x, const float* w, const float* b, void* out, int rows, int D, float eps, int mode,
                    int gh, int gw, void* stream) {
  return layernorm(x, w, b, out, rows, D, eps, mode, gh, gw, (cudaStream_t)stream);
}
int mk_op_attention(const void* qkv, void* out, int n_img, int T, int D, int heads, int impl, void* stream) {
  return attention_dispatch(qkv, out, n_img, T, D, heads, impl, (cudaStream_t)stream);
}
int mk_op_linattn(const float* qkv, float* kv_part, float* kv, void* msg, int n_img, int Gn, int h2, int w2, float eps,
                  void* stream) {
  MK_TRY(linattn_kv(qkv, kv_part, kv, n_img, Gn, h2, w2, (cudaStream_t)stream));
  return linattn_msg(qkv, kv, msg, n_img, Gn, h2, w2, eps, (cudaStream_t)stream);
}
int mk_op_matcher_reduce(const float* part_row, const float* part_col, const float* dustbin, int B, int N, int part_ld,
                         float* lse_r, float* lse_c, void* stream) {
  return matcher_lse_reduce(part_row, part_col, dustbin, B, N, part_ld, lse_r, lse_c, (cudaStream_t)stream);
}
long long mk_op_sample_workspace_bytes(int B, int IM) { return (long long)sampler_workspace_bytes(B, IM) + 512; }
int mk_op_sample(const float* fs, int B, int N, long long pitch, int IM, int n_sample, unsigned long long seed, void* ws,
                 long long ws_bytes, int* idx_out, int* status, void* stream) {
  MK_TRY(resolve_pitch(pitch, N, "mk_op_sample: pitch"));
  if ((long long)sampler_workspace_bytes(B, IM) + 256 > ws_bytes) { set_last_error("sampler workspace too small"); return MK_ERR_INVALID; }
  MK_CUDA_CHECK(cudaMemsetAsync(status, 0, sizeof(int), (cudaStream_t)stream));
  const size_t off = ((size_t)sampler_workspace_bytes(B, IM) + 255) & ~(size_t)255;
  unsigned long long* sd = reinterpret_cast<unsigned long long*>(reinterpret_cast<uint8_t*>(ws) + off);
  MK_TRY(seed_set(sd, seed, (cudaStream_t)stream));
  return sample_outer(fs, B, N, pitch, IM, n_sample, sd, ws, idx_out, status, (cudaStream_t)stream);
}
int mk_op_kabsch(const double* H, double* R, int n, void* stream) { return kabsch_batch(H, R, n, (cudaStream_t)stream); }

}
```

mickey_b200/csrc/epilogue.cuh:

```cuda
#pragma once
#include "common.cuh"

namespace mk {

__device__ __forceinline__ float rcp_approx(float x) { float y; asm("rcp.approx.ftz.f32 %0, %1;" : "=f"(y) : "f"(x)); return y; }
__device__ __forceinline__ float ex2_approx_f(float x) { float y; asm("ex2.approx.ftz.f32 %0, %1;" : "=f"(y) : "f"(x)); return y; }
__device__ __forceinline__ float gelu_erf(float x) {
  const float z = fabsf(x) * 0.70710678118654752f;
  const float t = rcp_approx(fmaf(0.3275911f, z, 1.0f));
  float poly = fmaf(1.061405429f, t, -1.453152027f);
  poly = fmaf(poly, t, 1.421413741f);
  poly = fmaf(poly, t, -0.284496736f);
  poly = fmaf(poly, t, 0.254829592f);
  const float erf_abs = fmaf(-poly * t, ex2_approx_f(-1.4426950408889634f * z * z), 1.0f);
  const float hx = 0.5f * x;
  return fmaf(hx, copysignf(erf_abs, x), hx);
}

__device__ __forceinline__ void fma2_f32(float& d0, float& d1, float a0, float a1, float b0, float b1, float c0, float c1) {
  d0 = __fmaf_rn(a0, b0, c0);
  d1 = __fmaf_rn(a1, b1, c1);
}
__device__ __forceinline__ void mul2_f32(float& d0, float& d1, float a0, float a1, float b0, float b1) {
  d0 = __fmul_rn(a0, b0);
  d1 = __fmul_rn(a1, b1);
}
__device__ __forceinline__ void gelu_erf2(float x0, float x1, float& y0, float& y1) {
  float z0, z1, d0, d1, n0, n1, q0, q1, w0, w1, e0, e1, h0, h1;
  mul2_f32(z0, z1, fabsf(x0), fabsf(x1), 0.70710678118654752f, 0.70710678118654752f);
  fma2_f32(d0, d1, z0, z1, 0.3275911f, 0.3275911f, 1.0f, 1.0f);
  const float t0 = rcp_approx(d0), t1 = rcp_approx(d1);
  fma2_f32(n0, n1, t0, t1, -1.061405429f, -1.061405429f, 1.453152027f, 1.453152027f);
  fma2_f32(n0, n1, n0, n1, t0, t1, -1.421413741f, -1.421413741f);
  fma2_f32(n0, n1, n0, n1, t0, t1, 0.284496736f, 0.284496736f);
  fma2_f32(n0, n1, n0, n1, t0, t1, -0.254829592f, -0.254829592f);
  mul2_f32(q0, q1, n0, n1, t0, t1);
  mul2_f32(w0, w1, z0, z1, -1.4426950408889634f, -1.4426950408889634f);
  mul2_f32(w0, w1, w0, w1, z0, z1);
  const float x20 = ex2_approx_f(w0), x21 = ex2_approx_f(w1);
  fma2_f32(e0, e1, q0, q1, x20, x21, 1.0f, 1.0f);
  mul2_f32(h0, h1, x0, x1, 0.5f, 0.5f);
  fma2_f32(y0, y1, h0, h1, copysignf(e0, x0), copysignf(e1, x1), h0, h1);
}

__device__ __forceinline__ float apply_act(float x, int act) {
  if (act == ACT_GELU) return gelu_erf(x);
  if (act == ACT_RELU) return fmaxf(x, 0.0f);
  return x;
}

__device__ __forceinline__ void store_h32(__half* dst, const float* v) {
#pragma unroll
  for (int q = 0; q < 4; ++q) {
    __half2 h0 = __floats2half2_rn(v[q * 8 + 0], v[q * 8 + 1]);
    __half2 h1 = __floats2half2_rn(v[q * 8 + 2], v[q * 8 + 3]);
    __half2 h2 = __floats2half2_rn(v[q * 8 + 4], v[q * 8 + 5]);
    __half2 h3 = __floats2half2_rn(v[q * 8 + 6], v[q * 8 + 7]);
    uint4 u;
    u.x = *reinterpret_cast<uint32_t*>(&h0);
    u.y = *reinterpret_cast<uint32_t*>(&h1);
    u.z = *reinterpret_cast<uint32_t*>(&h2);
    u.w = *reinterpret_cast<uint32_t*>(&h3);
    reinterpret_cast<uint4*>(dst)[q] = u;
  }
}

__device__ __forceinline__ void add_vec32(float (&v)[32], const float* __restrict__ b) {
#pragma unroll
  for (int q = 0; q < 8; ++q) {
    const float4 t = __ldg(reinterpret_cast<const float4*>(b) + q);
    v[q * 4 + 0] += t.x; v[q * 4 + 1] += t.y; v[q * 4 + 2] += t.z; v[q * 4 + 3] += t.w;
  }
}

__device__ __forceinline__ bool pad_valid(const GemmParams& p, int m, int& pos) {
  const int per_img = p.pad_h2 * p.pad_w2;
  pos = m % per_img;
  const int y = pos / p.pad_w2, x = pos % p.pad_w2;
  return y >= 1 && y <= p.pad_h2 - 2 && x >= 1 && x <= p.pad_w2 - 2;
}

template <int EPI>
__device__ __forceinline__ void epilogue_chunk(const GemmParams& p, int g, int m, int n0, float (&v)[32]) {
  if constexpr (EPI == EPI_STORE_H) {
    if (m >= p.M) return;
    if (p.bias) add_vec32(v, p.bias + (size_t)g * p.bias_group_off + n0);
    if (p.act == ACT_GELU) {
#pragma unroll
      for (int j = 0; j < 32; ++j) v[j] = gelu_erf(v[j]);
    } else if (p.act == ACT_RELU) {
#pragma unroll
      for (int j = 0; j < 32; ++j) v[j] = fmaxf(v[j], 0.0f);
    }
    store_h32(p.out_h + (size_t)g * p.out_h_group_off + (size_t)m * p.out_h_ld + n0, v);
  } else if constexpr (EPI == EPI_RESID_F) {
    if (m >= p.M) return;
    float* o = p.out_f + (size_t)m * p.out_f_ld + n0;
#pragma unroll
    for (int q = 0; q < 8; ++q) {
      float4 x = reinterpret_cast<float4*>(o)[q];
      const float4 gm = __ldg(reinterpret_cast<const float4*>(p.gamma + n0) + q);
      const float4 bs = __ldg(reinterpret_cast<const float4*>(p.bias + n0) + q);
      x.x += gm.x * (v[q * 4 + 0] + bs.x);
      x.y += gm.y * (v[q * 4 + 1] + bs.y);
      x.z += gm.z * (v[q * 4 + 2] + bs.z);
      x.w += gm.w * (v[q * 4 + 3] + bs.w);
      reinterpret_cast<float4*>(o)[q] = x;
    }
  } else if constexpr (EPI == EPI_PATCH) {
    if (m >= p.M) return;
    const int img = m / p.tok_per_img, tk = m % p.tok_per_img;
    float* o = p.out_f + ((size_t)img * (p.tok_per_img + 1) + 1 + tk) * p.out_f_ld + n0;
    const float* a = p.aux + (size_t)tk * p.N + n0;
#pragma unroll
    for (int q = 0; q < 8; ++q) {
      const float4 t = __ldg(reinterpret_cast<const float4*>(a) + q);
      float4 x;
      x.x = v[q * 4 + 0] + t.x; x.y = v[q * 4 + 1] + t.y; x.z = v[q * 4 + 2] + t.z; x.w = v[q * 4 + 3] + t.w;
      reinterpret_cast<float4*>(o)[q] = x;
    }
  } else if constexpr (EPI == EPI_CONV) {
    if (m >= p.M) return;
    int pos = 0;
    const bool valid = p.pad_h2 ? pad_valid(p, m, pos) : true;
    if (p.bias) add_vec32(v, p.bias + (size_t)g * p.bias_group_off + n0);
    if (p.res_h) {
      const uint4* r = reinterpret_cast<const uint4*>(p.res_h + (size_t)g * p.res_h_group_off + (size_t)m * p.res_h_ld + n0);
#pragma unroll
      for (int q = 0; q < 4; ++q) {
        uint4 u = r[q];
        const __half2* h = reinterpret_cast<const __half2*>(&u);
#pragma unroll
        for (int e = 0; e < 4; ++e) {
          float2 f = __half22float2(h[e]);
          v[q * 8 + e * 2] += f.x;
          v[q * 8 + e * 2 + 1] += f.y;
        }
      }
    }
#pragma unroll
    for (int j = 0; j < 32; ++j) v[j] = apply_act(v[j], p.act);
    if (p.aux && ((p.aux_group_mask >> g) & 1)) add_vec32(v, p.aux + (size_t)pos * p.N + n0);
    if (!valid) {
#pragma unroll
      for (int j = 0; j < 32; ++j) v[j] = 0.0f;
    }
    if (p.out_f) {
      float* o = p.out_f + (size_t)g * p.out_f_group_off + (size_t)m * p.out_f_ld + n0;
#pragma unroll
      for (int q = 0; q < 8; ++q)
        reinterpret_cast<float4*>(o)[q] = make_float4(v[q * 4], v[q * 4 + 1], v[q * 4 + 2], v[q * 4 + 3]);
    }
    if (p.out_h) store_h32(p.out_h + (size_t)g * p.out_h_group_off + (size_t)m * p.out_h_ld + n0, v);
  } else if constexpr (EPI == EPI_STORE_F) {
    if (m >= p.M) return;
    float* o = p.out_f + (size_t)g * p.out_f_group_off + (size_t)m * p.out_f_ld + n0;
#pragma unroll
    for (int q = 0; q < 8; ++q)
      reinterpret_cast<float4*>(o)[q] = make_float4(v[q * 4], v[q * 4 + 1], v[q * 4 + 2], v[q * 4 + 3]);
  }
}

template <int W> __device__ __forceinline__ int acc_idx(int r, int c) {
  const int k = c >> 2;
  const int h = 2 * (r & 3) + ((r ^ (r >> 2) ^ (k >> 3)) & 1);
  return r * W + ((k ^ h) << 2) + (c & 3);
}

template <int CPL> struct VecF;
template <> struct VecF<1> { using T = float; };
template <> struct VecF<2> { using T = float2; };

template <int CPL> __device__ __forceinline__ void ld_f(const float* p, float (&v)[CPL]) {
  if constexpr (CPL == 2) { const float2 t = *reinterpret_cast<const float2*>(p); v[0] = t.x; v[1] = t.y; } else { v[0] = *p; }
}
template <int CPL> __device__ __forceinline__ void ldg_f(const float* p, float (&v)[CPL]) {
  if constexpr (CPL == 2) { const float2 t = __ldg(reinterpret_cast<const float2*>(p)); v[0] = t.x; v[1] = t.y; } else { v[0] = __ldg(p); }
}
template <int CPL> __device__ __forceinline__ void st_f(float* p, const float (&v)[CPL]) {
  if constexpr (CPL == 2) { *reinterpret_cast<float2*>(p) = make_float2(v[0], v[1]); } else { *p = v[0]; }
}
template <int CPL> __device__ __forceinline__ void st_h(__half* p, const float (&v)[CPL]) {
  if constexpr (CPL == 2) { *reinterpret_cast<__half2*>(p) = __floats2half2_rn(v[0], v[1]); } else { *p = __float2half_rn(v[0]); }
}
template <int CPL> __device__ __forceinline__ void ld_h(const __half* p, float (&v)[CPL]) {
  if constexpr (CPL == 2) { const float2 t = __half22float2(*reinterpret_cast<const __half2*>(p)); v[0] = t.x; v[1] = t.y; }
  else { v[0] = __half2float(*p); }
}

__device__ __forceinline__ float warp_rowsum32(float (&part)[32], int lane) {
#pragma unroll
  for (int o = 16; o >= 1; o >>= 1) {
    const bool upper = (lane & o) != 0;
#pragma unroll
    for (int i = 0; i < o; ++i) {
      const float send = upper ? part[i] : part[i + o];
      const float keep = upper ? part[i + o] : part[i];
      part[i] = keep + __shfl_xor_sync(0xffffffffu, send, o);
    }
  }
  return part[0];
}

__device__ __forceinline__ float resid_ln_pass1(const GemmParams& p, int row0, int lane, int col_base, float* stage) {
  constexpr int RB = 8;
  const int col = col_base + lane * 2;
  const float2 bias = __ldg(reinterpret_cast<const float2*>(p.bias + col)), gam = __ldg(reinterpret_cast<const float2*>(p.gamma + col));
  const int rows = min(32, p.M - row0);
  float part[32];
#pragma unroll
  for (int r0 = 0; r0 < 32; r0 += RB) {
    float2 v[RB], x[RB];
#pragma unroll
    for (int i = 0; i < RB; ++i) {
      const int r = r0 + i;
      v[i] = *reinterpret_cast<const float2*>(stage + acc_idx<64>(r, lane * 2));
      x[i] = make_float2(0.f, 0.f);
      if (r < rows) x[i] = *reinterpret_cast<const float2*>(p.out_f + (size_t)(row0 + r) * p.out_f_ld + col);
    }
#pragma unroll
    for (int i = 0; i < RB; ++i) {
      const int r = r0 + i;
      float2 y = make_float2(0.f, 0.f);
      if (r < rows) {
        y.x = fmaf(gam.x, v[i].x + bias.x, x[i].x); y.y = fmaf(gam.y, v[i].y + bias.y, x[i].y);
        *reinterpret_cast<float2*>(p.out_f + (size_t)(row0 + r) * p.out_f_ld + col) = y;
      }
      *reinterpret_cast<float2*>(stage + acc_idx<64>(r, lane * 2)) = y;
      part[r] = y.x + y.y;
    }
  }
  return warp_rowsum32(part, lane);
}

__device__ __forceinline__ float resid_ln_pass2(int lane, const float* stage, float mean_l) {
  float part[32];
#pragma unroll
  for (int r = 0; r < 32; ++r) {
    const float2 x = *reinterpret_cast<const float2*>(stage + acc_idx<64>(r, lane * 2));
    const float mean = __shfl_sync(0xffffffffu, mean_l, r);
    const float d0 = x.x - mean, d1 = x.y - mean;
    part[r] = d0 * d0 + d1 * d1;
  }
  return warp_rowsum32(part, lane);
}

__device__ __forceinline__ void resid_ln_pass3(const GemmParams& p, int row0, int lane, int col_base, const float* stage,
                                               float mean_l, float rstd_l) {
  const int col = col_base + lane * 2;
  const float2 w = __ldg(reinterpret_cast<const float2*>(p.aux + col)), b = __ldg(reinterpret_cast<const float2*>(p.beta + col));
  const int rows = min(32, p.M - row0);
#pragma unroll 8
  for (int r = 0; r < 32; ++r) {
    const float2 x = *reinterpret_cast<const float2*>(stage + acc_idx<64>(r, lane * 2));
    const float mean = __shfl_sync(0xffffffffu, mean_l, r), rstd = __shfl_sync(0xffffffffu, rstd_l, r);
    if (r < rows)
      *reinterpret_cast<__half2*>(p.out_h + (size_t)(row0 + r) * p.out_h_ld + col) =
          __floats2half2_rn((x.x - mean) * rstd * w.x + b.x, (x.y - mean) * rstd * w.y + b.y);
  }
}

__device__ __forceinline__ void ld8(const float* p, float (&v)[8]) {
  const float4 a = *reinterpret_cast<const float4*>(p), b = *reinterpret_cast<const float4*>(p + 4);
  v[0] = a.x; v[1] = a.y; v[2] = a.z; v[3] = a.w; v[4] = b.x; v[5] = b.y; v[6] = b.z; v[7] = b.w;
}
__device__ __forceinline__ void ldg8(const float* p, float (&v)[8]) {
  const float4 a = __ldg(reinterpret_cast<const float4*>(p)), b = __ldg(reinterpret_cast<const float4*>(p) + 1);
  v[0] = a.x; v[1] = a.y; v[2] = a.z; v[3] = a.w; v[4] = b.x; v[5] = b.y; v[6] = b.z; v[7] = b.w;
}
__device__ __forceinline__ void st8(float* p, const float (&v)[8]) {
  reinterpret_cast<float4*>(p)[0] = make_float4(v[0], v[1], v[2], v[3]);
  reinterpret_cast<float4*>(p)[1] = make_float4(v[4], v[5], v[6], v[7]);
}
__device__ __forceinline__ void st8h(__half* p, const float (&v)[8]) {
  __half2 h0 = __floats2half2_rn(v[0], v[1]), h1 = __floats2half2_rn(v[2], v[3]);
  __half2 h2 = __floats2half2_rn(v[4], v[5]), h3 = __floats2half2_rn(v[6], v[7]);
  uint4 u;
  u.x = *reinterpret_cast<uint32_t*>(&h0); u.y = *reinterpret_cast<uint32_t*>(&h1);
  u.z = *reinterpret_cast<uint32_t*>(&h2); u.w = *reinterpret_cast<uint32_t*>(&h3);
  *reinterpret_cast<uint4*>(p) = u;
}
__device__ __forceinline__ void ld8h(const __half* p, float (&v)[8]) {
  const uint4 u = *reinterpret_cast<const uint4*>(p);
  const __half2* h = reinterpret_cast<const __half2*>(&u);
#pragma unroll
  for (int e = 0; e < 4; ++e) { const float2 f = __half22float2(h[e]); v[2 * e] = f.x; v[2 * e + 1] = f.y; }
}

template <int EPI, int W, int ACT>
__device__ __forceinline__ void epilogue_rows_impl(const GemmParams& p, int g, int row0, int lane, int col_base,
                                                   const float* __restrict__ stage, float mean_l, float rstd_l) {
  constexpr int LPR = W / 8;
  constexpr int RPS = 32 / LPR;
  constexpr int STEPS = 32 / RPS;
  constexpr bool GLOBAL_IN = (EPI == EPI_RESID_F || EPI == EPI_PATCH || EPI == EPI_CONV || EPI == EPI_LN);
  constexpr int U = GLOBAL_IN ? 2 : 4;
  static_assert(W % 8 == 0 && 32 % LPR == 0 && STEPS % U == 0, "staged epilogue: W in {32, 64}");
  const int seg = lane % LPR, rsub = lane / LPR;
  const int col = col_base + seg * 8;
  float bias[8], gam[8], bet[8];
#pragma unroll
  for (int i = 0; i < 8; ++i) { bias[i] = 0.f; gam[i] = 1.f; bet[i] = 0.f; }
  if constexpr (EPI == EPI_STORE_H || EPI == EPI_CONV) { if (p.bias) ldg8(p.bias + (size_t)g * p.bias_group_off + col, bias); }
  if constexpr (EPI == EPI_RESID_F) { ldg8(p.bias + col, bias); ldg8(p.gamma + col, gam); }
  if constexpr (EPI == EPI_LN) { ldg8(p.gamma + (size_t)g * p.ln_group_off + col, gam); ldg8(p.beta + (size_t)g * p.ln_group_off + col, bet); }
  const bool use_aux = (EPI == EPI_CONV) && p.aux && ((p.aux_group_mask >> g) & 1);
  const bool use_res = (EPI == EPI_CONV) && p.res_h;
  const bool ln_res = (EPI == EPI_LN) && p.out_f;
  const int rows = min(32, p.M - row0);
  int my_pos = 0, my_valid = 1, my_orow = 0;
  {
    const int mr = row0 + lane;
    if constexpr (EPI == EPI_CONV || EPI == EPI_LN) {
      if (p.pad_h2) { int pos; my_valid = pad_valid(p, mr, pos) ? 1 : 0; my_pos = pos; }
    }
    if constexpr (EPI == EPI_PATCH) {
      const int img = mr / p.tok_per_img;
      my_pos = mr - img * p.tok_per_img;
      my_orow = img * (p.tok_per_img + 1) + 1 + my_pos;
    }
  }
  float* out_f = p.out_f ? p.out_f + (size_t)g * p.out_f_group_off + col : nullptr;
  __half* out_h = p.out_h ? p.out_h + (size_t)g * p.out_h_group_off + col : nullptr;
#pragma unroll 1
  for (int s0 = 0; s0 < STEPS; s0 += U) {
    float v[U][8], x[U][8], a[U][8];
    int pos[U], orow[U];
    bool valid[U], live[U];
    float mean[U], rstd[U];
#pragma unroll
    for (int u = 0; u < U; ++u) {
      const int r = (s0 + u) * RPS + rsub;
      const size_t m = (size_t)(row0 + r);
      live[u] = r < rows;
      {
        const float4 a = *reinterpret_cast<const float4*>(stage + acc_idx<W>(r, seg * 8));
        const float4 b = *reinterpret_cast<const float4*>(stage + acc_idx<W>(r, seg * 8 + 4));
        v[u][0] = a.x; v[u][1] = a.y; v[u][2] = a.z; v[u][3] = a.w; v[u][4] = b.x; v[u][5] = b.y; v[u][6] = b.z; v[u][7] = b.w;
      }
      pos[u] = __shfl_sync(0xffffffffu, my_pos, r);
      orow[u] = __shfl_sync(0xffffffffu, my_orow, r);
      valid[u] = __shfl_sync(0xffffffffu, my_valid, r) != 0;
      mean[u] = 0.f; rstd[u] = 0.f;
      if constexpr (EPI == EPI_LN) { mean[u] = __shfl_sync(0xffffffffu, mean_l, r); rstd[u] = __shfl_sync(0xffffffffu, rstd_l, r); }
#pragma unroll
      for (int k = 0; k < 8; ++k) { x[u][k] = 0.f; a[u][k] = 0.f; }
      if (live[u]) {
        if constexpr (EPI == EPI_RESID_F) ld8(out_f + m * p.out_f_ld, x[u]);
        if constexpr (EPI == EPI_PATCH) ldg8(p.aux + (size_t)pos[u] * p.N + col, a[u]);
        if constexpr (EPI == EPI_CONV) {
          if (use_res) ld8h(p.res_h + (size_t)g * p.res_h_group_off + m * p.res_h_ld + col, x[u]);
          if (use_aux) ldg8(p.aux + (size_t)pos[u] * p.N + col, a[u]);
        }
        if constexpr (EPI == EPI_LN) { if (ln_res) ld8(out_f + m * p.out_f_ld, x[u]); }
      }
    }
#pragma unroll
    for (int u = 0; u < U; ++u) {
      if (!live[u]) continue;
      const int r = (s0 + u) * RPS + rsub;
      const size_t m = (size_t)(row0 + r);
      if constexpr (EPI == EPI_STORE_H) {
        if constexpr (ACT == ACT_GELU) {
#pragma unroll
          for (int k = 0; k < 8; k += 2) gelu_erf2(v[u][k] + bias[k], v[u][k + 1] + bias[k + 1], v[u][k], v[u][k + 1]);
        } else {
#pragma unroll
          for (int k = 0; k < 8; ++k) {
            const float t = v[u][k] + bias[k];
            v[u][k] = (ACT == ACT_RELU) ? fmaxf(t, 0.f) : t;
          }
        }
        st8h(out_h + m * p.out_h_ld, v[u]);
      } else if constexpr (EPI == EPI_RESID_F) {
#pragma unroll
        for (int k = 0; k < 8; ++k) x[u][k] = fmaf(gam[k], v[u][k] + bias[k], x[u][k]);
        st8(out_f + m * p.out_f_ld, x[u]);
      } else if constexpr (EPI == EPI_PATCH) {
#pragma unroll
        for (int k = 0; k < 8; ++k) v[u][k] += a[u][k];
        st8(out_f + (size_t)orow[u] * p.out_f_ld, v[u]);
      } else if constexpr (EPI == EPI_CONV) {
#pragma unroll
        for (int k = 0; k < 8; ++k) {
          float t = v[u][k] + bias[k] + x[u][k];
          t = ((ACT == ACT_RELU) ? fmaxf(t, 0.f) : ((ACT == ACT_GELU) ? gelu_erf(t) : t)) + a[u][k];
          v[u][k] = valid[u] ? t : 0.f;
        }
        if (out_f) st8(out_f + m * p.out_f_ld, v[u]);
        if (out_h) st8h(out_h + m * p.out_h_ld, v[u]);
      } else if constexpr (EPI == EPI_STORE_F) {
        st8(out_f + m * p.out_f_ld, v[u]);
      } else if constexpr (EPI == EPI_LN) {
#pragma unroll
        for (int k = 0; k < 8; ++k) {
          const float t = (v[u][k] - mean[u]) * rstd[u] * gam[k] + bet[k] + x[u][k];
          v[u][k] = valid[u] ? t : 0.f;
        }
        if (ln_res) st8(out_f + m * p.out_f_ld, v[u]);
        st8h(out_h + m * p.out_h_ld, v[u]);
      }
    }
  }
}

template <int EPI, int W>
__device__ __forceinline__ void epilogue_rows(const GemmParams& p, int g, int row0, int lane, int col_base,
                                              const float* __restrict__ stage, float mean_l, float rstd_l) {
  if constexpr (EPI == EPI_STORE_H || EPI == EPI_CONV) {
    if (p.act == ACT_GELU) epilogue_rows_impl<EPI, W, ACT_GELU>(p, g, row0, lane, col_base, stage, mean_l, rstd_l);
    else if (p.act == ACT_RELU) epilogue_rows_impl<EPI, W, ACT_RELU>(p, g, row0, lane, col_base, stage, mean_l, rstd_l);
    else epilogue_rows_impl<EPI, W, ACT_NONE>(p, g, row0, lane, col_base, stage, mean_l, rstd_l);
  } else {
    epilogue_rows_impl<EPI, W, ACT_NONE>(p, g, row0, lane, col_base, stage, mean_l, rstd_l);
  }
}

__device__ __forceinline__ void tma_store_3d(const CUtensorMap* map, uint32_t src_smem, int c0, int c1, int c2) {
  asm volatile("cp.async.bulk.tensor.3d.global.shared::cta.bulk_group [%0, {%2, %3, %4}], [%1];"
               ::"l"(map), "r"(src_smem), "r"(c0), "r"(c1), "r"(c2) : "memory");
}
__device__ __forceinline__ void tma_store_commit() { asm volatile("cp.async.bulk.commit_group;" ::: "memory"); }
__device__ __forceinline__ void tma_store_wait_read() { asm volatile("cp.async.bulk.wait_group.read 0;" ::: "memory"); }
__device__ __forceinline__ void tma_store_wait_all() { asm volatile("cp.async.bulk.wait_group 0;" ::: "memory"); }
__device__ __forceinline__ void fence_async_smem() { asm volatile("fence.proxy.async.shared::cta;" ::: "memory"); }

__device__ __forceinline__ float warp_colmax32(float (&part)[32], int lane) {
#pragma unroll
  for (int o = 16; o >= 1; o >>= 1) {
    const bool upper = (lane & o) != 0;
#pragma unroll
    for (int i = 0; i < o; ++i) {
      const float send = upper ? part[i] : part[i + o];
      const float keep = upper ? part[i + o] : part[i];
      part[i] = fmaxf(keep, __shfl_xor_sync(0xffffffffu, send, o));
    }
  }
  return part[0];
}

#define MK_NEG_INF (__int_as_float(0xff800000))

__device__ __forceinline__ void lse_chunk(const GemmParams& p, int g, int col0, int lane, int col_slot, bool row_ok,
                                          const float (&v)[32], float& rmax, float& rsum) {
  const float k2 = p.inv_temp * 1.4426950408889634f;
  float x[32], t[32];
  float cm = MK_NEG_INF;
#pragma unroll
  for (int j = 0; j < 32; ++j) {
    x[j] = (row_ok && col0 + j < p.n_valid) ? v[j] * k2 : MK_NEG_INF;
    cm = fmaxf(cm, x[j]);
    t[j] = x[j];
  }
  const float nm = fmaxf(rmax, cm);
  const float base = (nm == MK_NEG_INF) ? 0.f : nm;
  float acc = 0.f;
#pragma unroll
  for (int j = 0; j < 32; ++j) acc += ex2_approx_f(x[j] - base);
  rsum = rsum * ex2_approx_f(rmax - base) + acc;
  rmax = nm;
  const float cmax_l = warp_colmax32(t, lane);
#pragma unroll
  for (int j = 0; j < 32; ++j) {
    const float cj = __shfl_sync(0xffffffffu, cmax_l, j);
    t[j] = ex2_approx_f(x[j] - ((cj == MK_NEG_INF) ? 0.f : cj));
  }
  const float csum_l = warp_rowsum32(t, lane);
  const int col = col0 + lane;
  if (col < p.n_valid) p.part_col[((size_t)g * (p.part_ld / 32) + col_slot) * p.part_ld + col] = make_float2(cmax_l, csum_l);
}

__device__ __forceinline__ void lse_chunk_bounded(const GemmParams& p, int g, int col0, int lane, int col_slot, bool row_ok,
                                                  const float (&v)[32], float& rsum) {
  const float k2 = p.inv_temp * 1.4426950408889634f, sh = p.lse_bound * k2;
  float t[32];
  float acc0 = 0.f, acc1 = 0.f;
#pragma unroll
  for (int j = 0; j < 32; j += 2) {
    const float e0 = (row_ok && col0 + j < p.n_valid) ? ex2_approx_f(fmaf(v[j], k2, -sh)) : 0.f;
    const float e1 = (row_ok && col0 + j + 1 < p.n_valid) ? ex2_approx_f(fmaf(v[j + 1], k2, -sh)) : 0.f;
    t[j] = e0; t[j + 1] = e1;
    acc0 += e0; acc1 += e1;
  }
  rsum += acc0 + acc1;
  const float csum_l = warp_rowsum32(t, lane);
  const int col = col0 + lane;
  if (col < p.n_valid) p.part_col[((size_t)g * (p.part_ld / 32) + col_slot) * p.part_ld + col] = make_float2(sh, csum_l);
}

__device__ __forceinline__ void dual_store_chunk(const GemmParams& p, int g, int row0, int lane, int n0,
                                                 const float (&v)[32], float* stage, float lr, float s0) {
  const float k2x2 = 2.0f * p.inv_temp * 1.4426950408889634f;
  const size_t gv = (size_t)g * p.n_valid;
  const size_t go = (size_t)g * p.n_valid * (size_t)p.out_pitch;
  const int col = n0 + lane;
  const bool col_ok = col < p.n_valid;
  float* lcs = stage + 32 * 33;
  const float lc_l = col_ok ? __ldg(p.lse_c + (size_t)g * p.part_ld + col) : -MK_NEG_INF;
  const float s1 = col_ok ? __ldg(p.scr1 + gv + col) : 0.0f;
  lcs[lane] = lc_l;
  __syncwarp();
#pragma unroll
  for (int j = 0; j < 32; ++j) stage[lane * 33 + j] = ex2_approx_f(fmaf(v[j], k2x2, -lr) - lcs[j]);
  __syncwarp();
  const int rows = min(32, p.n_valid - row0);
  const bool full = p.scores != nullptr;
#pragma unroll 4
  for (int r = 0; r < rows; ++r) {
    const float sc = stage[r * 33 + lane];
    const float kp = __shfl_sync(0xffffffffu, s0, r) * s1;
    if (col_ok) {
      const size_t o = go + (size_t)(row0 + r) * (size_t)p.out_pitch + col;
      if (full) { p.scores[o] = sc; p.kp_scores[o] = kp; }
      p.final_scores[o] = sc * kp;
    }
  }
  __syncwarp();
}

__device__ __forceinline__ void dual_store_chunk_tma(const GemmParams& p, const OutMaps& om, int g, int row0, int lane, int n0,
                                                     const float (&v)[32], float* stage, float* aux, float lr, float s0,
                                                     float lc_l, float s1_l) {
  const float k2x2 = 2.0f * p.inv_temp * 1.4426950408889634f;
  const bool full = p.scores != nullptr;
  if (lane == 0) tma_store_wait_read();
  __syncwarp();
  aux[lane] = lc_l;
  aux[32 + lane] = s1_l;
  __syncwarp();
  float4* b_sc = reinterpret_cast<float4*>(stage) + lane * 8;
  float4* b_kp = b_sc + 256;
  float4* b_fs = b_sc + 512;
  const int sw = lane & 7;
#pragma unroll
  for (int k = 0; k < 8; ++k) {
    const float4 lc = *reinterpret_cast<const float4*>(aux + 4 * k), s1 = *reinterpret_cast<const float4*>(aux + 32 + 4 * k);
    float4 sc, kp, fs;
    sc.x = ex2_approx_f(fmaf(v[4 * k + 0], k2x2, -lr) - lc.x); sc.y = ex2_approx_f(fmaf(v[4 * k + 1], k2x2, -lr) - lc.y);
    sc.z = ex2_approx_f(fmaf(v[4 * k + 2], k2x2, -lr) - lc.z); sc.w = ex2_approx_f(fmaf(v[4 * k + 3], k2x2, -lr) - lc.w);
    kp.x = s0 * s1.x; kp.y = s0 * s1.y; kp.z = s0 * s1.z; kp.w = s0 * s1.w;
    fs.x = sc.x * kp.x; fs.y = sc.y * kp.y; fs.z = sc.z * kp.z; fs.w = sc.w * kp.w;
    const int kk = k ^ sw;
    if (full) { b_sc[kk] = sc; b_kp[kk] = kp; }
    b_fs[kk] = fs;
  }
  fence_async_smem();
  __syncwarp();
  if (lane == 0) {
    const uint32_t sa = (uint32_t)__cvta_generic_to_shared(stage);
    if (full) { tma_store_3d(&om.m[0], sa, n0, row0, g); tma_store_3d(&om.m[1], sa + 4096, n0, row0, g); }
    tma_store_3d(&om.m[2], sa + 8192, n0, row0, g);
    tma_store_commit();
  }
}

__device__ __forceinline__ void ln_store_chunk(const GemmParams& p, int g, int m, int n0, float (&v)[32],
                                               float mean, float rstd) {
  if (m >= p.M) return;
  const float* gm = p.gamma + (size_t)g * p.ln_group_off + n0;
  const float* bt = p.beta + (size_t)g * p.ln_group_off + n0;
#pragma unroll
  for (int j = 0; j < 32; ++j) v[j] = (v[j] - mean) * rstd * __ldg(gm + j) + __ldg(bt + j);
  if (p.out_f) {
    float* o = p.out_f + (size_t)g * p.out_f_group_off + (size_t)m * p.out_f_ld + n0;
#pragma unroll
    for (int q = 0; q < 8; ++q) {
      float4 x = reinterpret_cast<float4*>(o)[q];
      v[q * 4 + 0] += x.x; v[q * 4 + 1] += x.y; v[q * 4 + 2] += x.z; v[q * 4 + 3] += x.w;
    }
  }
  if (p.pad_h2) {
    int pos;
    if (!pad_valid(p, m, pos)) {
#pragma unroll
      for (int j = 0; j < 32; ++j) v[j] = 0.0f;
    }
  }
  if (p.out_f) {
    float* o = p.out_f + (size_t)g * p.out_f_group_off + (size_t)m * p.out_f_ld + n0;
#pragma unroll
    for (int q = 0; q < 8; ++q)
      reinterpret_cast<float4*>(o)[q] = make_float4(v[q * 4], v[q * 4 + 1], v[q * 4 + 2], v[q * 4 + 3]);
  }
  store_h32(p.out_h + (size_t)g * p.out_h_group_off + (size_t)m * p.out_h_ld + n0, v);
}

}
```

mickey_b200/csrc/gemm.cu:

```cuda
#include "gemm.h"
#include "gemm_tc.cuh"

#include <algorithm>
#include <cstdarg>
#include <cstdlib>
#include <cstring>
#include <mutex>
#include <unordered_map>

namespace mk {

typedef CUresult (*PFN_encodeTiled)(CUtensorMap*, CUtensorMapDataType, cuuint32_t, void*, const cuuint64_t*,
                                    const cuuint64_t*, const cuuint32_t*, const cuuint32_t*, CUtensorMapInterleave,
                                    CUtensorMapSwizzle, CUtensorMapL2promotion, CUtensorMapFloatOOBfill);

static PFN_encodeTiled get_encode() {
  static PFN_encodeTiled fn = nullptr;
  static std::once_flag once;
  std::call_once(once, [] {
    void* p = nullptr;
    cudaDriverEntryPointQueryResult qres;
    if (cudaGetDriverEntryPoint("cuTensorMapEncodeTiled", &p, cudaEnableDefault, &qres) == cudaSuccess &&
        qres == cudaDriverEntryPointSuccess)
      fn = reinterpret_cast<PFN_encodeTiled>(p);
  });
  return fn;
}

struct MapKey {
  const void* ptr; long long rows, cols, ld; int box;
  long long groups;
  bool operator==(const MapKey& o) const {
    return ptr == o.ptr && rows == o.rows && cols == o.cols && ld == o.ld && box == o.box && groups == o.groups;
  }
};
struct MapKeyHash {
  size_t operator()(const MapKey& k) const {
    size_t h = reinterpret_cast<size_t>(k.ptr);
    h = h * 1000003u ^ (size_t)k.rows; h = h * 1000003u ^ (size_t)k.cols; h = h * 1000003u ^ (size_t)k.ld;
    h = h * 1000003u ^ (size_t)k.groups;
    return h * 1000003u ^ (size_t)k.box;
  }
};
static std::unordered_map<MapKey, CUtensorMap, MapKeyHash> g_map_cache;
static std::mutex g_map_mutex;

static int encode_tensor_map_out_f16(CUtensorMap* map, const void* ptr, long long groups, long long rows, long long cols,
                                     int box_rows);

static int cached_map(const MapKey& key, CUtensorMap* map) {
  std::lock_guard<std::mutex> lock(g_map_mutex);
  auto it = g_map_cache.find(key);
  if (it != g_map_cache.end()) { *map = it->second; return MK_OK; }
  int rc = key.groups ? encode_tensor_map_out_f16(map, key.ptr, key.groups, key.rows, key.cols, key.box)
                      : encode_tensor_map_2d(map, CU_TENSOR_MAP_DATA_TYPE_FLOAT16, key.ptr, key.rows, key.cols, key.ld, key.box);
  if (rc == MK_OK) {
    if (g_map_cache.size() > 4096) g_map_cache.clear();
    g_map_cache.emplace(key, *map);
  }
  return rc;
}

int make_tensor_map_f16(CUtensorMap* map, const void* ptr, long long rows, long long cols, long long ld_elems,
                        int box_rows) {
  return cached_map(MapKey{ptr, rows, cols, ld_elems, box_rows, 0}, map);
}

int make_tensor_map_out_f16(CUtensorMap* map, void* ptr, long long groups, long long rows, long long cols, int box_rows) {
  return cached_map(MapKey{ptr, rows, cols, cols, box_rows, groups}, map);
}

static_assert(BLOCK_K * 2 == 128, "an fp16 operand box is one 128-byte swizzle row wide");

int encode_tensor_map_2d(CUtensorMap* map, CUtensorMapDataType dtype, const void* ptr, long long rows, long long cols,
                         long long ld_elems, int box_rows) {
  PFN_encodeTiled enc = get_encode();
  if (!enc) { set_last_error("cuTensorMapEncodeTiled entry point not available"); return MK_ERR_CUDA; }
  const int esize = dtype == CU_TENSOR_MAP_DATA_TYPE_FLOAT32 ? 4 : 2;
  if ((reinterpret_cast<uintptr_t>(ptr) & 15) || (ld_elems * esize) % 16) {
    set_last_error("tensor map operand must be 16-byte aligned with ld %% %d == 0 (ptr=%p ld=%lld)", 16 / esize, ptr, ld_elems);
    return MK_ERR_INVALID;
  }
  cuuint64_t dims[2] = {(cuuint64_t)cols, (cuuint64_t)rows};
  cuuint64_t strides[1] = {(cuuint64_t)ld_elems * esize};
  cuuint32_t box[2] = {(cuuint32_t)(128 / esize), (cuuint32_t)box_rows};
  cuuint32_t estr[2] = {1, 1};
  CUresult r = enc(map, dtype, 2, const_cast<void*>(ptr), dims, strides, box, estr,
                   CU_TENSOR_MAP_INTERLEAVE_NONE, CU_TENSOR_MAP_SWIZZLE_128B, CU_TENSOR_MAP_L2_PROMOTION_L2_256B,
                   CU_TENSOR_MAP_FLOAT_OOB_FILL_NONE);
  if (r != CUDA_SUCCESS) { set_last_error("cuTensorMapEncodeTiled failed with CUresult %d", (int)r); return MK_ERR_CUDA; }
  return MK_OK;
}

static int encode_tensor_map_out_f16(CUtensorMap* map, const void* ptr, long long groups, long long rows, long long cols,
                                     int box_rows) {
  PFN_encodeTiled enc = get_encode();
  if (!enc) { set_last_error("cuTensorMapEncodeTiled entry point not available"); return MK_ERR_CUDA; }
  if ((reinterpret_cast<uintptr_t>(ptr) & 15) || (cols % 8)) {
    set_last_error("TMA output must be 16-byte aligned with cols %% 8 == 0 (ptr=%p cols=%lld)", ptr, cols);
    return MK_ERR_INVALID;
  }
  cuuint64_t dims[3] = {(cuuint64_t)cols, (cuuint64_t)rows, (cuuint64_t)groups};
  cuuint64_t strides[2] = {(cuuint64_t)cols * 2, (cuuint64_t)cols * 2 * (cuuint64_t)rows};
  cuuint32_t box[3] = {64, (cuuint32_t)box_rows, 1};
  cuuint32_t estr[3] = {1, 1, 1};
  CUresult r = enc(map, CU_TENSOR_MAP_DATA_TYPE_FLOAT16, 3, const_cast<void*>(ptr), dims, strides, box, estr,
                   CU_TENSOR_MAP_INTERLEAVE_NONE, CU_TENSOR_MAP_SWIZZLE_128B, CU_TENSOR_MAP_L2_PROMOTION_NONE,
                   CU_TENSOR_MAP_FLOAT_OOB_FILL_NONE);
  if (r != CUDA_SUCCESS) { set_last_error("cuTensorMapEncodeTiled (fp16 output) failed with CUresult %d", (int)r); return MK_ERR_CUDA; }
  return MK_OK;
}

static int encode_tensor_map_out_f32(CUtensorMap* map, const void* ptr, long long n, long long pitch, long long groups) {
  PFN_encodeTiled enc = get_encode();
  if (!enc) { set_last_error("cuTensorMapEncodeTiled entry point not available"); return MK_ERR_CUDA; }
  if ((reinterpret_cast<uintptr_t>(ptr) & 15) || (pitch % 4) || pitch < n) {
    set_last_error("TMA output needs a 16-byte aligned base and a row pitch that is a multiple of 4 floats (ptr=%p pitch=%lld)", ptr, pitch);
    return MK_ERR_INVALID;
  }
  cuuint64_t dims[3] = {(cuuint64_t)n, (cuuint64_t)n, (cuuint64_t)groups};
  cuuint64_t strides[2] = {(cuuint64_t)pitch * 4, (cuuint64_t)pitch * 4 * (cuuint64_t)n};
  cuuint32_t box[3] = {32, 32, 1};
  cuuint32_t estr[3] = {1, 1, 1};
  CUresult r = enc(map, CU_TENSOR_MAP_DATA_TYPE_FLOAT32, 3, const_cast<void*>(ptr), dims, strides, box, estr,
                   CU_TENSOR_MAP_INTERLEAVE_NONE, CU_TENSOR_MAP_SWIZZLE_128B, CU_TENSOR_MAP_L2_PROMOTION_NONE,
                   CU_TENSOR_MAP_FLOAT_OOB_FILL_NONE);
  if (r != CUDA_SUCCESS) { set_last_error("cuTensorMapEncodeTiled (fp32 output) failed with CUresult %d", (int)r); return MK_ERR_CUDA; }
  return MK_OK;
}

static const OutMaps& no_out_maps() { static OutMaps z = {}; return z; }

template <int BN, int EPI>
__global__ void __launch_bounds__(128)
gemm_simt_kernel(const __half* __restrict__ A, long long a_rows, long long lda, const __half* __restrict__ B,
                 long long b_rows, long long ldb, const GemmParams p) {
  __shared__ __align__(16) __half As[BLOCK_M][BLOCK_K + 8];
  __shared__ __half Bs[BN][BLOCK_K + 8];
  pdl_trigger();
  pdl_wait();
  const GemmTile tile = gemm_tile<BN>(p, blockIdx.x);
  const int g = tile.g, m0 = tile.m0, n0 = tile.n0;
  const int t = threadIdx.x;
  float acc[BN];
#pragma unroll
  for (int j = 0; j < BN; ++j) acc[j] = 0.f;
  const int a_col0 = p.a_col_base + g * p.a_col_group_off;
  const long long a_row0 = (long long)m0 + (long long)g * p.a_row_group_off;
  const long long b_row0 = (long long)n0 + (long long)g * p.b_row_group_off;
  for (int kc = 0; kc < p.k_chunks; ++kc) {
    const int tap = kc / p.chunks_per_tap, kin = kc - tap * p.chunks_per_tap;
    for (int idx = t; idx < BLOCK_M * BLOCK_K; idx += 128) {
      const int r = idx / BLOCK_K, c = idx % BLOCK_K;
      const long long row = a_row0 + r + p.tap_shift[tap];
      const long long col = a_col0 + kin * BLOCK_K + c;
      As[r][c] = (row >= 0 && row < a_rows && col < lda) ? A[row * lda + col] : __float2half(0.f);
    }
    for (int idx = t; idx < BN * BLOCK_K; idx += 128) {
      const int r = idx / BLOCK_K, c = idx % BLOCK_K;
      const long long row = b_row0 + r;
      Bs[r][c] = (row < b_rows) ? B[row * ldb + (long long)kc * BLOCK_K + c] : __float2half(0.f);
    }
    __syncthreads();
    for (int k = 0; k < BLOCK_K; ++k) {
      const float a = __half2float(As[t][k]);
#pragma unroll
      for (int j = 0; j < BN; ++j) acc[j] = fmaf(a, __half2float(Bs[j][k]), acc[j]);
    }
    __syncthreads();
  }
  const int m = m0 + t;
  float v[32];
  if constexpr (EPI == EPI_LN) {
    float sum = 0.f;
    for (int j = 0; j < BN; ++j) sum += acc[j];
    const float mean = sum / BN;
    float sq = 0.f;
    for (int j = 0; j < BN; ++j) { const float d = acc[j] - mean; sq += d * d; }
    const float rstd = rsqrtf(sq / BN + p.eps);
    for (int c = 0; c < BN / 32; ++c) {
      for (int j = 0; j < 32; ++j) v[j] = acc[c * 32 + j];
      ln_store_chunk(p, g, m, n0 + c * 32, v, mean, rstd);
    }
  } else if constexpr (EPI == EPI_LSE || EPI == EPI_DUAL) {
  } else {
    for (int c = 0; c < BN / 32; ++c) {
      if (n0 + c * 32 < p.N) {
        for (int j = 0; j < 32; ++j) v[j] = acc[c * 32 + j];
        epilogue_chunk<EPI>(p, g, m, n0 + c * 32, v);
      }
    }
  }
}

bool pdl_enabled() {
  static int v = -1;
  if (v < 0) { const char* e = getenv("MICKEY_PDL"); v = (e && strcmp(e, "0") == 0) ? 0 : 1; }
  return v == 1;
}

static bool use_simt() {
  static int v = -1;
  if (v < 0) {
    const char* e = getenv("MICKEY_GEMM_IMPL");
    v = (e && strcmp(e, "simt") == 0) ? 1 : 0;
  }
  return v == 1;
}

int sm_count() {
  static int n[64] = {0};
  int dev = 0;
  cudaGetDevice(&dev);
  int& c = n[dev & 63];
  if (!c) { cudaDeviceGetAttribute(&c, cudaDevAttrMultiProcessorCount, dev); if (c <= 0) c = 132; }
  return c;
}

template <int BN, int EPI, int STAGES, bool PERSISTENT, bool PAIR = false>
static int launch_tc(const CUtensorMap& tmA, const CUtensorMap& tmB, const GemmParams& p, cudaStream_t stream,
                     const OutMaps& om = no_out_maps()) {
  static unsigned long long attr_mask = 0;
  static int max_clusters[64] = {0};
  constexpr int smem = gemm_smem_bytes<BN, EPI, STAGES, PERSISTENT>();
  auto kernel = gemm_tc_kernel<BN, EPI, STAGES, PERSISTENT, PAIR>;
  cudaLaunchConfig_t cfg = {};
  cfg.blockDim = dim3(gemm_threads<PERSISTENT>()); cfg.dynamicSmemBytes = smem; cfg.stream = stream;
  cudaLaunchAttribute attr[2];
  int n_attr = 0;
  if constexpr (EPI == EPI_RESID_LN || PAIR) {
    attr[n_attr].id = cudaLaunchAttributeClusterDimension;
    attr[n_attr].val.clusterDim.x = PAIR ? 2 : p.N / BN; attr[n_attr].val.clusterDim.y = 1; attr[n_attr++].val.clusterDim.z = 1;
  }
  cfg.attrs = attr;
  cfg.numAttrs = n_attr;
  int dev = 0;
  if constexpr (PAIR) cudaGetDevice(&dev);
  if (first_use_on_device(attr_mask)) {
    MK_CUDA_CHECK(cudaFuncSetAttribute(kernel, cudaFuncAttributeMaxDynamicSharedMemorySize, smem));
    if constexpr (PAIR) {
      cfg.gridDim = dim3(2 * sm_count());
      MK_CUDA_CHECK(cudaOccupancyMaxActiveClusters(&max_clusters[dev & 63], kernel, &cfg));
    }
  }
  const int tiles = gemm_tile_count<BN>(p);
  if constexpr (PAIR) {
    const int n_clusters = max_clusters[dev & 63];
    if (n_clusters <= 0) { set_last_error("GEMM: no two-CTA cluster of %d bytes of shared memory fits on this device", smem); return MK_ERR_UNSUPPORTED; }
    cfg.gridDim = dim3(2 * std::min(gemm_tile_count<BN, 2>(p), n_clusters));
  } else {
    cfg.gridDim = dim3(PERSISTENT ? std::min(tiles, sm_count()) : tiles);
  }
  if (pdl_enabled()) {
    attr[n_attr].id = cudaLaunchAttributeProgrammaticStreamSerialization;
    attr[n_attr++].val.programmaticStreamSerializationAllowed = 1;
  }
  cfg.numAttrs = n_attr;
  MK_CUDA_CHECK(cudaLaunchKernelEx(&cfg, kernel, tmA, tmB, p, om));
  return MK_OK;
}

static bool deep_ring(int tiles, const GemmParams& p) {
  return (long long)tiles <= (long long)sm_count() * 5 / 4 && p.k_chunks > 3;
}
static bool persistent_grid(int tiles) { return tiles > 8 * sm_count(); }

template <int BN, int EPI>
static int launch_one(const GemmOperand& A, const GemmOperand& B, const GemmParams& p, cudaStream_t stream, int impl) {
  const int tiles = gemm_tile_count<BN>(p);
  if constexpr (EPI == EPI_RESID_LN) {
    if (impl == GEMM_IMPL_SIMT || BN != 128 || p.N / BN > 8 || p.groups != 1) { set_last_error("EPI_RESID_LN: wgmma path, N <= 1024, one group"); return MK_ERR_UNSUPPORTED; }
  }
  if (impl == GEMM_IMPL_SIMT) {
    if constexpr (EPI != EPI_RESID_LN)
    MK_CUDA_CHECK(launch_k(gemm_simt_kernel<BN, EPI>, dim3(tiles), dim3(128), 0, stream, reinterpret_cast<const __half*>(A.ptr),
                           (long long)A.rows, (long long)A.ld, reinterpret_cast<const __half*>(B.ptr), (long long)B.rows,
                           (long long)B.ld, p));
  } else {
    CUtensorMap tmA, tmB;
    int rc = make_tensor_map_f16(&tmA, A.ptr, A.rows, A.cols, A.ld, BLOCK_M);
    if (rc) return rc;
    if constexpr (persistent_epilogue<EPI>()) {
      const bool forced = impl == GEMM_IMPL_TC_PAIRED || impl == GEMM_IMPL_TC_UNPAIRED;
      if (forced || persistent_grid(tiles)) {
        const bool pair = impl != GEMM_IMPL_TC_UNPAIRED;
        rc = make_tensor_map_f16(&tmB, B.ptr, B.rows, B.cols, B.ld, pair ? BN / 2 : BN);
        if (rc) return rc;
        if (pair) return launch_tc<BN, EPI, ring_stages<BN>(), true, true>(tmA, tmB, p, stream);
        return launch_tc<BN, EPI, ring_stages<BN>(), true>(tmA, tmB, p, stream);
      }
    }
    rc = make_tensor_map_f16(&tmB, B.ptr, B.rows, B.cols, B.ld, BN);
    if (rc) return rc;
    if constexpr (EPI == EPI_DUAL) {
      if (p.out_tma) {
        OutMaps om = {};
        float* outs[3] = {p.scores, p.kp_scores, p.final_scores};
        for (int i = 0; i < 3; ++i)
          if (outs[i]) { rc = encode_tensor_map_out_f32(&om.m[i], outs[i], p.n_valid, p.out_pitch, p.groups); if (rc) return rc; }
        return launch_tc<BN, EPI, shallow_stages<BN>(), false>(tmA, tmB, p, stream, om);
      }
    }
    if (deep_ring(tiles, p)) return launch_tc<BN, EPI, deep_stages<BN>(), false>(tmA, tmB, p, stream);
    return launch_tc<BN, EPI, shallow_stages<BN>(), false>(tmA, tmB, p, stream);
  }
  MK_CUDA_CHECK(cudaGetLastError());
  return MK_OK;
}

template <int EPI>
static int launch_bn(int bn, const GemmOperand& A, const GemmOperand& B, const GemmParams& p, cudaStream_t s, int impl) {
  if (bn == 128) return launch_one<128, EPI>(A, B, p, s, impl);
  if (bn == 64) return launch_one<64, EPI>(A, B, p, s, impl);
  set_last_error("unsupported BLOCK_N %d", bn);
  return MK_ERR_INVALID;
}

bool gemm_resid_ln_supported(int M, int N, int k_chunks) {
  (void)M; (void)k_chunks;
  static int on = -1;
  if (on < 0) { const char* e = getenv("MICKEY_FUSE_LN"); on = (e && e[0] == '1') ? 1 : 0; }
  return on && !use_simt() && N % 128 == 0 && N <= 1024;
}

int launch_gemm(int epi, const GemmOperand& A, const GemmOperand& B, const GemmParams& p, cudaStream_t stream, int impl) {
  if (impl == GEMM_IMPL_DEFAULT) impl = use_simt() ? GEMM_IMPL_SIMT : GEMM_IMPL_TC;
  if (p.k_chunks <= 0 || p.M <= 0 || p.N <= 0 || p.groups <= 0) { set_last_error("bad GEMM shape"); return MK_ERR_INVALID; }
  const bool matcher = (epi == EPI_LSE || epi == EPI_DUAL);
  if (matcher && impl == GEMM_IMPL_SIMT) { set_last_error("the matcher epilogues run on the wgmma kernel only"); return MK_ERR_UNSUPPORTED; }
  if (matcher && (p.part_ld % 128 || p.part_ld < p.n_valid)) { set_last_error("matcher: part_ld must be n_valid rounded up to 128"); return MK_ERR_INVALID; }
  if (epi == EPI_DUAL && p.out_pitch < p.n_valid) { set_last_error("matcher: out_pitch %lld < n_valid %d", p.out_pitch, p.n_valid); return MK_ERR_INVALID; }
  if (!matcher && (p.N % 32)) { set_last_error("GEMM N=%d must be a multiple of 32", p.N); return MK_ERR_INVALID; }
  int bn = (matcher || p.N % 128 == 0) ? 128 : 64;
  if (!matcher && p.N % bn) { set_last_error("GEMM N=%d not tileable", p.N); return MK_ERR_INVALID; }
  if (epi == EPI_LN && p.N != 128) { set_last_error("EPI_LN needs N == 128"); return MK_ERR_INVALID; }
  if (epi == EPI_RESID_LN && (p.N % 128 || p.N > 1024 || p.groups != 1 || !p.aux || !p.beta || !p.out_h || !p.out_f)) {
    set_last_error("EPI_RESID_LN needs N % 128 == 0, N <= 1024, one group, LN weight (aux), LN bias (beta), out_f and out_h");
    return MK_ERR_INVALID;
  }
  switch (epi) {
    case EPI_STORE_H: return launch_bn<EPI_STORE_H>(bn, A, B, p, stream, impl);
    case EPI_RESID_F: return launch_bn<EPI_RESID_F>(bn, A, B, p, stream, impl);
    case EPI_RESID_LN: return launch_one<128, EPI_RESID_LN>(A, B, p, stream, impl);
    case EPI_PATCH:   return launch_bn<EPI_PATCH>(bn, A, B, p, stream, impl);
    case EPI_CONV:    return launch_bn<EPI_CONV>(bn, A, B, p, stream, impl);
    case EPI_STORE_F: return launch_bn<EPI_STORE_F>(bn, A, B, p, stream, impl);
    case EPI_LN:      return launch_one<128, EPI_LN>(A, B, p, stream, impl);
    case EPI_LSE:     return launch_one<128, EPI_LSE>(A, B, p, stream, impl);
    case EPI_DUAL:    return launch_one<128, EPI_DUAL>(A, B, p, stream, impl);
  }
  set_last_error("unknown epilogue %d", epi);
  return MK_ERR_INVALID;
}

static thread_local char g_err[512] = "";
void set_last_error(const char* fmt, ...) {
  va_list ap;
  va_start(ap, fmt);
  vsnprintf(g_err, sizeof(g_err), fmt, ap);
  va_end(ap);
}
const char* last_error() { return g_err; }

}
```

mickey_b200/csrc/gemm.h:

```cpp
#pragma once
#include "common.cuh"

namespace mk {

struct GemmOperand {
  const void* ptr;
  long long rows, cols, ld;
};

enum GemmImpl : int { GEMM_IMPL_DEFAULT = 0, GEMM_IMPL_TC = 1, GEMM_IMPL_SIMT = 2, GEMM_IMPL_TC_PAIRED = 3, GEMM_IMPL_TC_UNPAIRED = 4 };

int make_tensor_map_f16(CUtensorMap* map, const void* ptr, long long rows, long long cols, long long ld_elems, int box_rows);
int encode_tensor_map_2d(CUtensorMap* map, CUtensorMapDataType dtype, const void* ptr, long long rows, long long cols,
                         long long ld_elems, int box_rows);
int make_tensor_map_out_f16(CUtensorMap* map, void* ptr, long long groups, long long rows, long long cols, int box_rows);
int sm_count();
int launch_gemm(int epi, const GemmOperand& A, const GemmOperand& B, const GemmParams& p, cudaStream_t stream,
                int impl = GEMM_IMPL_DEFAULT);
bool gemm_resid_ln_supported(int M, int N, int k_chunks);
const char* last_error();

}
```

mickey_b200/csrc/gemm_tc.cuh:

```cuda
#pragma once
#include "common.cuh"
#include "epilogue.cuh"

namespace mk {

constexpr int BLOCK_M = 128;
constexpr int BLOCK_K = 64;
constexpr int WGMMA_K = 16;
constexpr int GEMM_WARP_EPI = 8;

template <int BN> constexpr int ring_stages() { return BN == 128 ? 4 : 6; }
template <int BN> constexpr int shallow_stages() { return BN == 128 ? 3 : 4; }
template <int BN> constexpr int deep_stages() { return BN == 128 ? 6 : 8; }
template <int EPI> constexpr bool persistent_epilogue() { return EPI != EPI_DUAL && EPI != EPI_RESID_LN && EPI != EPI_LN; }
template <bool PERSISTENT> constexpr int gemm_threads() { return PERSISTENT ? 640 : 288; }
template <bool PERSISTENT> constexpr int gemm_warp_tma() { return PERSISTENT ? 16 : 8; }

constexpr int DUAL_STAGE_BYTES = 3 * 4096;
constexpr int DUAL_AUX_BYTES = 8 * 64 * 4;
constexpr int DUAL_BYTES = 8 * DUAL_STAGE_BYTES + DUAL_AUX_BYTES;

template <int BN> constexpr int acc_block_floats() { return 32 * (BN / 2); }
template <int BN> constexpr int acc_tile_bytes() { return 8 * acc_block_floats<BN>() * 4; }
template <int BN, int STAGES> constexpr int ring_bytes() { return STAGES * (BLOCK_M * BLOCK_K * 2 + BN * BLOCK_K * 2); }
template <int BN, int EPI, int STAGES, bool PERSISTENT> constexpr int acc_tile_offset() {
  return PERSISTENT ? ring_bytes<BN, STAGES>() : EPI == EPI_DUAL ? DUAL_BYTES : 0;
}
template <int BN, int EPI, int STAGES, bool PERSISTENT>
constexpr int region_bytes() {
  return ring_bytes<BN, STAGES>() > acc_tile_offset<BN, EPI, STAGES, PERSISTENT>() + acc_tile_bytes<BN>()
             ? ring_bytes<BN, STAGES>() : acc_tile_offset<BN, EPI, STAGES, PERSISTENT>() + acc_tile_bytes<BN>();
}
template <int BN, int EPI, int STAGES, bool PERSISTENT> constexpr int gemm_smem_bytes() {
  return region_bytes<BN, EPI, STAGES, PERSISTENT>() + 1024 + 256 + 2048;
}
template <int BN, int EPI, int STAGES, bool PERSISTENT> constexpr int gemm_ctas_per_sm() {
  return !PERSISTENT && EPI != EPI_LN && EPI != EPI_RESID_LN && gemm_smem_bytes<BN, EPI, STAGES, PERSISTENT>() <= 113 * 1024 ? 2 : 1;
}

struct GemmTile { int g, m0, n0, n_tile; };
template <int BN, int MT = 1>
__host__ __device__ __forceinline__ int gemm_tile_count(const GemmParams& p) {
  return ((p.M + MT * BLOCK_M - 1) / (MT * BLOCK_M)) * ((p.N + BN - 1) / BN) * p.groups;
}
template <int BN, int MT = 1>
__device__ __forceinline__ GemmTile gemm_tile(const GemmParams& p, int t, int rank = 0) {
  const int n_tiles = (p.N + BN - 1) / BN, m_units = (p.M + MT * BLOCK_M - 1) / (MT * BLOCK_M);
  const int n = t % n_tiles;
  t /= n_tiles;
  int g, m;
  if (p.a_row_group_off == 0 && p.a_col_group_off == 0) { g = t % p.groups; m = t / p.groups; }
  else { m = t % m_units; g = t / m_units; }
  return {g, (m * MT + rank) * BLOCK_M, n * BN, n};
}

__device__ __forceinline__ uint32_t smem_u32(const void* p) { return (uint32_t)__cvta_generic_to_shared(p); }

__device__ __forceinline__ void mbar_init(uint32_t bar, uint32_t count) {
  asm volatile("mbarrier.init.shared::cta.b64 [%0], %1;" ::"r"(bar), "r"(count));
}
__device__ __forceinline__ void mbar_expect_tx(uint32_t bar, uint32_t bytes) {
  asm volatile("mbarrier.arrive.expect_tx.shared::cta.b64 _, [%0], %1;" ::"r"(bar), "r"(bytes) : "memory");
}
__device__ __forceinline__ void mbar_arrive(uint32_t bar) {
  asm volatile("mbarrier.arrive.shared::cta.b64 _, [%0];" ::"r"(bar) : "memory");
}
__device__ __forceinline__ void mbar_wait(uint32_t bar, uint32_t parity) {
  asm volatile(
      "{\n\t"
      ".reg .pred P1;\n\t"
      "WAIT_%=:\n\t"
      "mbarrier.try_wait.parity.shared::cta.b64 P1, [%0], %1;\n\t"
      "@P1 bra DONE_%=;\n\t"
      "bra WAIT_%=;\n\t"
      "DONE_%=:\n\t"
      "}" ::"r"(bar), "r"(parity) : "memory");
}
__device__ __forceinline__ void tma_load_2d(uint32_t dst, const CUtensorMap* map, uint32_t bar, int c0, int c1) {
  asm volatile(
      "cp.async.bulk.tensor.2d.shared::cluster.global.mbarrier::complete_tx::bytes [%0], [%1, {%3, %4}], [%2];"
      ::"r"(dst), "l"(map), "r"(bar), "r"(c0), "r"(c1) : "memory");
}
__device__ __forceinline__ void tma_load_2d_multicast(uint32_t dst, const CUtensorMap* map, uint32_t bar, int c0, int c1,
                                                      uint16_t cta_mask) {
  asm volatile(
      "cp.async.bulk.tensor.2d.shared::cluster.global.mbarrier::complete_tx::bytes.multicast::cluster [%0], [%1, {%3, %4}], [%2], %5;"
      ::"r"(dst), "l"(map), "r"(bar), "r"(c0), "r"(c1), "h"(cta_mask) : "memory");
}
__device__ __forceinline__ void mbar_arrive_cluster(uint32_t bar, uint32_t cta_rank) {
  asm volatile(
      "{\n\t.reg .b32 remote;\n\t"
      "mapa.shared::cluster.u32 remote, %0, %1;\n\t"
      "mbarrier.arrive.shared::cluster.b64 _, [remote];\n\t}"
      ::"r"(bar), "r"(cta_rank) : "memory");
}
__device__ __forceinline__ bool elect_one() {
  uint32_t pred = 0;
  asm volatile(
      "{\n\t"
      ".reg .pred P1;\n\t"
      "elect.sync _|P1, 0xFFFFFFFF;\n\t"
      "selp.b32 %0, 1, 0, P1;\n\t"
      "}" : "=r"(pred));
  return pred != 0;
}
constexpr int GEMM_REGS_PRODUCER = 40;
constexpr int GEMM_REGS_EPILOGUE = 120;
template <int R> __device__ __forceinline__ void setmaxnreg_dec() { asm volatile("setmaxnreg.dec.sync.aligned.u32 %0;" ::"n"(R)); }
template <int R> __device__ __forceinline__ void setmaxnreg_inc() { asm volatile("setmaxnreg.inc.sync.aligned.u32 %0;" ::"n"(R)); }
__device__ __forceinline__ void consumer_sync() { asm volatile("bar.sync 1, 256;" ::: "memory"); }

__device__ __forceinline__ uint64_t gmma_desc_sw128(uint32_t smem_addr) {
  uint64_t d = 0;
  d |= (uint64_t)((smem_addr & 0x3FFFF) >> 4);
  d |= (uint64_t)1 << 16;
  d |= (uint64_t)(1024 >> 4) << 32;
  d |= (uint64_t)1 << 62;
  return d;
}
__device__ __forceinline__ void wgmma_fence() { asm volatile("wgmma.fence.sync.aligned;" ::: "memory"); }
__device__ __forceinline__ void wgmma_commit() { asm volatile("wgmma.commit_group.sync.aligned;" ::: "memory"); }
template <int N> __device__ __forceinline__ void wgmma_wait() { asm volatile("wgmma.wait_group.sync.aligned %0;" ::"n"(N) : "memory"); }
template <int N> __device__ __forceinline__ void reg_fence(float (&d)[N]) {
#pragma unroll
  for (int i = 0; i < N; ++i) asm volatile("" : "+f"(d[i])::"memory");
}

__device__ __forceinline__ void wgmma_m64n64k16(float (&d)[32], uint64_t desc_a, uint64_t desc_b, uint32_t scale_d) {
  asm volatile(
      "{\n\t.reg .pred p;\n\tsetp.ne.b32 p, %34, 0;\n\t"
      "wgmma.mma_async.sync.aligned.m64n64k16.f32.f16.f16 "
      "{%0, %1, %2, %3, %4, %5, %6, %7, %8, %9, %10, %11, %12, %13, %14, %15, %16, %17, %18, %19, %20, %21, %22, %23, %24, %25, %26, %27, %28, %29, %30, %31}, %32, %33, p, 1, 1, 0, 0;\n\t}"
      : "+f"(d[0]), "+f"(d[1]), "+f"(d[2]), "+f"(d[3]), "+f"(d[4]), "+f"(d[5]), "+f"(d[6]), "+f"(d[7]), "+f"(d[8]), "+f"(d[9]), "+f"(d[10]), "+f"(d[11]), "+f"(d[12]), "+f"(d[13]), "+f"(d[14]), "+f"(d[15]), "+f"(d[16]), "+f"(d[17]), "+f"(d[18]), "+f"(d[19]), "+f"(d[20]), "+f"(d[21]), "+f"(d[22]), "+f"(d[23]), "+f"(d[24]), "+f"(d[25]), "+f"(d[26]), "+f"(d[27]), "+f"(d[28]), "+f"(d[29]), "+f"(d[30]), "+f"(d[31])
      : "l"(desc_a), "l"(desc_b), "r"(scale_d));
}

__device__ __forceinline__ void wgmma_m64n128k16(float (&d)[64], uint64_t desc_a, uint64_t desc_b, uint32_t scale_d) {
  asm volatile(
      "{\n\t.reg .pred p;\n\tsetp.ne.b32 p, %66, 0;\n\t"
      "wgmma.mma_async.sync.aligned.m64n128k16.f32.f16.f16 "
      "{%0, %1, %2, %3, %4, %5, %6, %7, %8, %9, %10, %11, %12, %13, %14, %15, %16, %17, %18, %19, %20, %21, %22, %23, %24, %25, %26, %27, %28, %29, %30, %31, %32, %33, %34, %35, %36, %37, %38, %39, %40, %41, %42, %43, %44, %45, %46, %47, %48, %49, %50, %51, %52, %53, %54, %55, %56, %57, %58, %59, %60, %61, %62, %63}, %64, %65, p, 1, 1, 0, 0;\n\t}"
      : "+f"(d[0]), "+f"(d[1]), "+f"(d[2]), "+f"(d[3]), "+f"(d[4]), "+f"(d[5]), "+f"(d[6]), "+f"(d[7]), "+f"(d[8]), "+f"(d[9]), "+f"(d[10]), "+f"(d[11]), "+f"(d[12]), "+f"(d[13]), "+f"(d[14]), "+f"(d[15]), "+f"(d[16]), "+f"(d[17]), "+f"(d[18]), "+f"(d[19]), "+f"(d[20]), "+f"(d[21]), "+f"(d[22]), "+f"(d[23]), "+f"(d[24]), "+f"(d[25]), "+f"(d[26]), "+f"(d[27]), "+f"(d[28]), "+f"(d[29]), "+f"(d[30]), "+f"(d[31]), "+f"(d[32]), "+f"(d[33]), "+f"(d[34]), "+f"(d[35]), "+f"(d[36]), "+f"(d[37]), "+f"(d[38]), "+f"(d[39]), "+f"(d[40]), "+f"(d[41]), "+f"(d[42]), "+f"(d[43]), "+f"(d[44]), "+f"(d[45]), "+f"(d[46]), "+f"(d[47]), "+f"(d[48]), "+f"(d[49]), "+f"(d[50]), "+f"(d[51]), "+f"(d[52]), "+f"(d[53]), "+f"(d[54]), "+f"(d[55]), "+f"(d[56]), "+f"(d[57]), "+f"(d[58]), "+f"(d[59]), "+f"(d[60]), "+f"(d[61]), "+f"(d[62]), "+f"(d[63])
      : "l"(desc_a), "l"(desc_b), "r"(scale_d));
}

template <int BN>
__device__ __forceinline__ void wgmma_tile(float (&d)[BN / 2], uint64_t desc_a, uint64_t desc_b, uint32_t scale_d) {
  if constexpr (BN == 128) wgmma_m64n128k16(d, desc_a, desc_b, scale_d);
  else wgmma_m64n64k16(d, desc_a, desc_b, scale_d);
}

__device__ __forceinline__ void cluster_sync_all() {
  asm volatile("barrier.cluster.arrive.release.aligned;\n\tbarrier.cluster.wait.acquire.aligned;" ::: "memory");
}
__device__ __forceinline__ uint32_t cluster_size() {
  uint32_t r;
  asm volatile("mov.u32 %0, %%cluster_nctarank;" : "=r"(r));
  return r;
}
__device__ __forceinline__ float ld_dsmem_f32(uint32_t local_smem_addr, uint32_t cta_rank) {
  uint32_t remote;
  asm volatile("mapa.shared::cluster.u32 %0, %1, %2;" : "=r"(remote) : "r"(local_smem_addr), "r"(cta_rank));
  float v;
  asm volatile("ld.shared::cluster.f32 %0, [%1];" : "=f"(v) : "r"(remote) : "memory");
  return v;
}

template <int BN>
__device__ __forceinline__ void acc_chunk(const float* acc, int q, int lane, int c, float (&v)[32]) {
  constexpr int W = BN / 2;
  const float* blk = acc + (q + 4 * ((c * 32) / W)) * acc_block_floats<BN>();
#pragma unroll
  for (int k4 = 0; k4 < 8; ++k4) {
    const float4 t = *reinterpret_cast<const float4*>(blk + acc_idx<W>(lane, (c * 32) % W + 4 * k4));
    v[k4 * 4] = t.x; v[k4 * 4 + 1] = t.y; v[k4 * 4 + 2] = t.z; v[k4 * 4 + 3] = t.w;
  }
}

template <int BN, int EPI>
__device__ __forceinline__ void tile_epilogue(const GemmParams& p, const OutMaps& om, int g, int m0, int n0, int n_tile, int q, int half,
                                              int lane, float* acc, float* red, uint32_t red_saddr, float* dual_stage, float* dual_aux) {
  constexpr int CHUNKS = BN / 32;
  constexpr int W = BN / 2;
  constexpr int CPH = CHUNKS / 2;
  const int c_begin = half * CPH, c_end = c_begin + CPH;
  const int m = m0 + q * 32 + lane;
  float* stage = acc + (q + 4 * half) * acc_block_floats<BN>();
  float v[32];
  if constexpr (EPI == EPI_LN) {
    float sum = 0.f;
#pragma unroll
    for (int c = 0; c < CHUNKS; ++c) {
      acc_chunk<BN>(acc, q, lane, c, v);
#pragma unroll
      for (int j = 0; j < 32; ++j) sum += v[j];
    }
    const float mean = sum * (1.0f / BN);
    float sq = 0.f;
#pragma unroll
    for (int c = 0; c < CHUNKS; ++c) {
      acc_chunk<BN>(acc, q, lane, c, v);
#pragma unroll
      for (int j = 0; j < 32; ++j) { const float d = v[j] - mean; sq += d * d; }
    }
    const float rstd = rsqrtf(sq * (1.0f / BN) + p.eps);
    epilogue_rows<EPI_LN, W>(p, g, m0 + q * 32, lane, n0 + half * W, stage, mean, rstd);
  } else if constexpr (EPI == EPI_RESID_LN) {
    static_assert(BN == 128, "EPI_RESID_LN: 128-wide tiles");
    const int row0 = m0 + q * 32, col_base = n0 + half * 64, slot = half * 128 + q * 32 + lane;
    const uint32_t n_cta = cluster_size();
    const float inv_n = 1.0f / (float)p.N;
    red[slot] = resid_ln_pass1(p, row0, lane, col_base, stage);
    cluster_sync_all();
    float tot = 0.f;
    for (uint32_t c = 0; c < n_cta; ++c)
      tot += ld_dsmem_f32(red_saddr + (q * 32 + lane) * 4, c) + ld_dsmem_f32(red_saddr + (128 + q * 32 + lane) * 4, c);
    const float mean = tot * inv_n;
    red[256 + slot] = resid_ln_pass2(lane, stage, mean);
    cluster_sync_all();
    float tot2 = 0.f;
    for (uint32_t c = 0; c < n_cta; ++c)
      tot2 += ld_dsmem_f32(red_saddr + (256 + q * 32 + lane) * 4, c) + ld_dsmem_f32(red_saddr + (384 + q * 32 + lane) * 4, c);
    const float rstd = rsqrtf(tot2 * inv_n + p.eps);
    resid_ln_pass3(p, row0, lane, col_base, stage, mean, rstd);
    cluster_sync_all();
  } else if constexpr (EPI == EPI_LSE) {
    static_assert(BN == 128, "matcher epilogues: 128-wide tiles");
    const bool row_ok = m < p.n_valid;
    float rmax = MK_NEG_INF, rsum = 0.f;
    if (p.lse_bound > 0.f) {
      rmax = p.lse_bound * p.inv_temp * 1.4426950408889634f;
      for (int c = c_begin; c < c_end; ++c) {
        if (n0 + c * 32 < p.n_valid) {
          acc_chunk<BN>(acc, q, lane, c, v);
          lse_chunk_bounded(p, g, n0 + c * 32, lane, (m0 / BLOCK_M) * 4 + q, row_ok, v, rsum);
        }
      }
    } else {
      for (int c = c_begin; c < c_end; ++c) {
        if (n0 + c * 32 < p.n_valid) {
          acc_chunk<BN>(acc, q, lane, c, v);
          lse_chunk(p, g, n0 + c * 32, lane, (m0 / BLOCK_M) * 4 + q, row_ok, v, rmax, rsum);
        }
      }
    }
    if (row_ok) p.part_row[((size_t)g * (p.part_ld / 64) + n_tile * 2 + half) * p.part_ld + m] = make_float2(rmax, rsum);
  } else if constexpr (EPI == EPI_DUAL) {
    static_assert(BN == 128, "matcher epilogues: 128-wide tiles");
    const bool row_ok = m < p.n_valid;
    const float lr = row_ok ? __ldg(p.lse_r + (size_t)g * p.part_ld + m) : -MK_NEG_INF;
    const float s0 = row_ok ? __ldg(p.scr0 + (size_t)g * p.n_valid + m) : 0.0f;
    if (p.out_tma) {
      float lc_pre[CPH], s1_pre[CPH];
#pragma unroll
      for (int ci = 0; ci < CPH; ++ci) {
        const int col = n0 + (c_begin + ci) * 32 + lane;
        const bool ok = col < p.n_valid;
        lc_pre[ci] = ok ? __ldg(p.lse_c + (size_t)g * p.part_ld + col) : -MK_NEG_INF;
        s1_pre[ci] = ok ? __ldg(p.scr1 + (size_t)g * p.n_valid + col) : 0.0f;
      }
#pragma unroll
      for (int ci = 0; ci < CPH; ++ci) {
        const int c = c_begin + ci;
        if (n0 + c * 32 < p.n_valid && m0 + q * 32 < p.n_valid) {
          acc_chunk<BN>(acc, q, lane, c, v);
          dual_store_chunk_tma(p, om, g, m0 + q * 32, lane, n0 + c * 32, v, dual_stage, dual_aux, lr, s0, lc_pre[ci], s1_pre[ci]);
        }
      }
    } else {
      for (int c = c_begin; c < c_end; ++c) {
        if (n0 + c * 32 < p.n_valid) {
          acc_chunk<BN>(acc, q, lane, c, v);
          dual_store_chunk(p, g, m0 + q * 32, lane, n0 + c * 32, v, dual_stage, lr, s0);
        }
      }
    }
  } else {
    epilogue_rows<EPI, W>(p, g, m0 + q * 32, lane, n0 + half * W, stage, 0.f, 0.f);
  }
}

template <int BN, int EPI, int STAGES, bool PERSISTENT, bool PAIR = false>
__global__ void __launch_bounds__((gemm_threads<PERSISTENT>()), (gemm_ctas_per_sm<BN, EPI, STAGES, PERSISTENT>()))
gemm_tc_kernel(const __grid_constant__ CUtensorMap tmA, const __grid_constant__ CUtensorMap tmB, const GemmParams p,
               const __grid_constant__ OutMaps om) {
  static_assert(BN == 64 || BN == 128, "wgmma tiles: N = 64 or 128");
  static_assert(gemm_smem_bytes<BN, EPI, STAGES, PERSISTENT>() <= 227 * 1024, "GEMM: shared memory");
  extern __shared__ uint8_t smem_raw[];
  constexpr int A_BYTES = BLOCK_M * BLOCK_K * 2;
  constexpr int B_BYTES = BN * BLOCK_K * 2;
  constexpr int STAGE_BYTES = A_BYTES + B_BYTES;
  constexpr int W = BN / 2;
  static_assert(!PERSISTENT || persistent_epilogue<EPI>(), "this epilogue runs one tile per CTA");
  static_assert(!PAIR || PERSISTENT, "CTA pairs: persistent kernel only");
  constexpr bool ONE_TILE = !PERSISTENT;
  constexpr int WARP_TMA = gemm_warp_tma<PERSISTENT>();
  constexpr int MT = PAIR ? 2 : 1;
  const int rank = PAIR ? (int)(blockIdx.x & 1) : 0;
  const int work0 = PAIR ? (int)(blockIdx.x >> 1) : (int)blockIdx.x;
  const int work_step = PAIR ? (int)(gridDim.x >> 1) : (int)gridDim.x;

  const uint32_t raw = smem_u32(smem_raw);
  const uint32_t base = (raw + 1023u) & ~1023u;
  const uint32_t bar_base = base + region_bytes<BN, EPI, STAGES, PERSISTENT>();
  const uint32_t full_bar0 = bar_base;
  const uint32_t empty_bar0 = bar_base + 8 * STAGES;
  const uint32_t acc_full_bar = bar_base + 16 * STAGES;
  const uint32_t acc_empty_bar = acc_full_bar + 8;
  const uint32_t red_saddr = bar_base + 256;
  uint8_t* const gbase = smem_raw + (base - raw);
  float* const acc = reinterpret_cast<float*>(gbase + acc_tile_offset<BN, EPI, STAGES, PERSISTENT>());

  const int warp = threadIdx.x >> 5;
  const int lane = threadIdx.x & 31;
  const int n_work = gemm_tile_count<BN, MT>(p);

  if (warp == WARP_TMA && lane == 0) {
    asm volatile("prefetch.tensormap [%0];" ::"l"(&tmA) : "memory");
    asm volatile("prefetch.tensormap [%0];" ::"l"(&tmB) : "memory");
    for (int s = 0; s < STAGES; ++s) {
      mbar_init(full_bar0 + 8 * s, 1);
      mbar_init(empty_bar0 + 8 * s, 8 * MT);
    }
    mbar_init(acc_full_bar, 256);
    mbar_init(acc_empty_bar, 256);
    asm volatile("fence.mbarrier_init.release.cluster;" ::: "memory");
  }
  if constexpr (PAIR) cluster_sync_all();
  else __syncthreads();
  pdl_wait();

  if (warp >= WARP_TMA) {
    if constexpr (!ONE_TILE) setmaxnreg_dec<GEMM_REGS_PRODUCER>();
    if (warp == WARP_TMA && elect_one()) {
      int stage = 0;
      uint32_t phase = 0;
      for (int t = work0; t < n_work; t += work_step) {
        const GemmTile tile = gemm_tile<BN, MT>(p, t, rank);
        const int a_col0 = p.a_col_base + tile.g * p.a_col_group_off;
        const int a_row0 = tile.m0 + tile.g * p.a_row_group_off;
        const int b_row0 = tile.n0 + tile.g * p.b_row_group_off;
        for (int kc = 0; kc < p.k_chunks; ++kc) {
          const int tap = kc / p.chunks_per_tap;
          const int kin = kc - tap * p.chunks_per_tap;
          mbar_wait(empty_bar0 + 8 * stage, phase ^ 1);
          const uint32_t sa = base + stage * STAGE_BYTES;
          const uint32_t fb = full_bar0 + 8 * stage;
          mbar_expect_tx(fb, STAGE_BYTES);
          tma_load_2d(sa, &tmA, fb, a_col0 + kin * BLOCK_K, a_row0 + p.tap_shift[tap]);
          if constexpr (PAIR) tma_load_2d_multicast(sa + A_BYTES + rank * (B_BYTES / 2), &tmB, fb, kc * BLOCK_K, b_row0 + rank * (BN / 2), 0x3);
          else tma_load_2d(sa + A_BYTES, &tmB, fb, kc * BLOCK_K, b_row0);
          if (++stage == STAGES) { stage = 0; phase ^= 1; }
        }
      }
    }
    __syncwarp();
    pdl_trigger();
    if constexpr (EPI == EPI_RESID_LN) { cluster_sync_all(); cluster_sync_all(); cluster_sync_all(); }
    if constexpr (PAIR) cluster_sync_all();
    return;
  }

  if (warp < GEMM_WARP_EPI) {
    const int wg = warp >> 2;
    int stage = 0;
    uint32_t phase = 0, acc_phase = 0;
    auto release = [&](int s) {
      if constexpr (PAIR) { mbar_arrive_cluster(empty_bar0 + 8 * s, 0); mbar_arrive_cluster(empty_bar0 + 8 * s, 1); }
      else mbar_arrive(empty_bar0 + 8 * s);
    };
    for (int t = work0; t < n_work; t += work_step) {
      float d[BN / 2];
#pragma unroll
      for (int i = 0; i < BN / 2; ++i) d[i] = 0.f;
      for (int kc = 0; kc < p.k_chunks; ++kc) {
        mbar_wait(full_bar0 + 8 * stage, phase);
        const uint32_t sa = base + stage * STAGE_BYTES;
        const uint64_t da = gmma_desc_sw128(sa + wg * (64 * 128));
        const uint64_t db = gmma_desc_sw128(sa + A_BYTES);
        wgmma_fence();
#pragma unroll
        for (int k = 0; k < BLOCK_K / WGMMA_K; ++k)
          wgmma_tile<BN>(d, da + (uint64_t)(k * 2), db + (uint64_t)(k * 2), 1u);
        wgmma_commit();
        wgmma_wait<1>();
        reg_fence(d);
        if (kc > 0 && lane == 0) release(stage == 0 ? STAGES - 1 : stage - 1);
        if (++stage == STAGES) { stage = 0; phase ^= 1; }
      }
      wgmma_wait<0>();
      reg_fence(d);
      if (lane == 0) release(stage == 0 ? STAGES - 1 : stage - 1);
      if (t + work_step >= n_work) pdl_trigger();

      if constexpr (ONE_TILE) consumer_sync();
      else mbar_wait(acc_empty_bar, acc_phase ^ 1);
      const int r_base = wg * 64 + (warp & 3) * 16 + (lane >> 2);
#pragma unroll
      for (int j = 0; j < BN / 8; ++j) {
#pragma unroll
        for (int h = 0; h < 2; ++h) {
          const int r = r_base + 8 * h, c = 8 * j + 2 * (lane & 3);
          float* dst = acc + ((r >> 5) + 4 * (c / W)) * acc_block_floats<BN>() + acc_idx<W>(r & 31, c % W);
          *reinterpret_cast<float2*>(dst) = make_float2(d[4 * j + 2 * h], d[4 * j + 2 * h + 1]);
        }
      }
      if constexpr (ONE_TILE) {
        consumer_sync();
        const GemmTile tile = gemm_tile<BN>(p, t);
        tile_epilogue<BN, EPI>(p, om, tile.g, tile.m0, tile.n0, tile.n_tile, warp & 3, warp >> 2, lane, acc,
                               reinterpret_cast<float*>(smem_raw + (red_saddr - raw)), red_saddr,
                               reinterpret_cast<float*>(gbase + warp * DUAL_STAGE_BYTES),
                               reinterpret_cast<float*>(gbase + 8 * DUAL_STAGE_BYTES) + warp * 64);
      } else {
        mbar_arrive(acc_full_bar);
        acc_phase ^= 1;
      }
    }
    if constexpr (EPI == EPI_DUAL) { if (p.out_tma && lane == 0) tma_store_wait_all(); }
    if constexpr (PAIR) cluster_sync_all();
    return;
  }

  if constexpr (ONE_TILE) return;
  setmaxnreg_inc<GEMM_REGS_EPILOGUE>();
  const int ew = warp - GEMM_WARP_EPI;
  uint32_t acc_phase = 0;
  for (int t = work0; t < n_work; t += work_step) {
    const GemmTile tile = gemm_tile<BN, MT>(p, t, rank);
    mbar_wait(acc_full_bar, acc_phase);
    if (t + work_step >= n_work) pdl_trigger();
    if (tile.m0 < p.M)
      tile_epilogue<BN, EPI>(p, om, tile.g, tile.m0, tile.n0, tile.n_tile, ew & 3, ew >> 2, lane, acc,
                             reinterpret_cast<float*>(smem_raw + (red_saddr - raw)), red_saddr,
                             reinterpret_cast<float*>(gbase + ew * DUAL_STAGE_BYTES),
                             reinterpret_cast<float*>(gbase + 8 * DUAL_STAGE_BYTES) + ew * 64);
    mbar_arrive(acc_empty_bar);
    acc_phase ^= 1;
  }
  if constexpr (PAIR) cluster_sync_all();
}

}
```

Before: 305.6.

## Add BN=192 persistent wgmma GEMM tile with four epilogue warps

Adds a 192-column wgmma tile (m64n192k16) for the persistent GEMM path. It comes with a 3-stage ring, four epilogue warps that each loop over both halves, and a column-chunked staged epilogue that handles W=96. The wider tile is meant to reuse each A tile across more output columns and cut tile count and wave quantization for N sizes that divide by 192. Register budgeting via setmaxnreg is disabled for this variant. A block-N query API is added, presumably so callers can choose the tile width, and that choice may route default calls to 192.

```diff
diff --git a/include/mickey_b200.h b/include/mickey_b200.h
--- a/include/mickey_b200.h
+++ b/include/mickey_b200.h
@@ -224,6 +224,7 @@
 } mk_gemm_args;
 
 int mk_op_gemm(const mk_gemm_args* args, void* stream);
+int mk_op_gemm_block_n(const mk_gemm_args* args, int sm_count);
 int mk_op_patch_gather(const float* img, void* patches_h, int n_img, int H, int W, int kpad, float* x_f,
                        const float* cls_pos, int D, void* stream);
 int mk_op_ingest_u8(const unsigned char* img_u8, void* patches_h, int n_img, int H, int W, int kpad, float* x_f,
diff --git a/mickey_b200/_lib.py b/mickey_b200/_lib.py
--- a/mickey_b200/_lib.py
+++ b/mickey_b200/_lib.py
@@ -169,6 +169,7 @@
     "mk_profile_enable": (C.c_int, [C.c_void_p, C.c_int]),
     "mk_profile_read": (C.c_int, [C.c_void_p, C.c_char_p, C.c_int]),
     "mk_op_gemm": (C.c_int, [C.POINTER(MkGemmArgs), C.c_void_p]),
+    "mk_op_gemm_block_n": (C.c_int, [C.POINTER(MkGemmArgs), C.c_int]),
     "mk_op_patch_gather": (C.c_int, [C.c_void_p, C.c_void_p, C.c_int, C.c_int, C.c_int, C.c_int, C.c_void_p, C.c_void_p,
                                      C.c_int, C.c_void_p]),
     "mk_op_ingest_u8": (C.c_int, [C.c_void_p, C.c_void_p, C.c_int, C.c_int, C.c_int, C.c_int, C.c_void_p, C.c_void_p,
diff --git a/mickey_b200/csrc/engine.cu b/mickey_b200/csrc/engine.cu
--- a/mickey_b200/csrc/engine.cu
+++ b/mickey_b200/csrc/engine.cu
@@ -829,6 +829,14 @@
   return launch_gemm(a->epi, A, B, p, (cudaStream_t)stream, a->impl);
 }
 
+int mk_op_gemm_block_n(const mk_gemm_args* a, int sms) {
+  if (!a || sms <= 0) { set_last_error("mk_op_gemm_block_n: NULL arguments or sm_count <= 0"); return MK_ERR_INVALID; }
+  GemmParams p;
+  memset(&p, 0, sizeof(p));
+  p.M = a->M; p.N = a->N; p.k_chunks = a->k_chunks; p.groups = a->groups;
+  return gemm_block_n(a->epi, p, a->impl, sms);
+}
+
 int mk_op_patch_gather(const float* img, void* P, int n_img, int H, int W, int kpad, float* X, const float* cls_pos,
                        int D, void* stream) {
   return patch_gather(img, P, n_img, H, W, kpad, X, cls_pos, D, (cudaStream_t)stream);
diff --git a/mickey_b200/csrc/epilogue.cuh b/mickey_b200/csrc/epilogue.cuh
--- a/mickey_b200/csrc/epilogue.cuh
+++ b/mickey_b200/csrc/epilogue.cuh
@@ -167,27 +167,6 @@
   return r * W + ((k ^ h) << 2) + (c & 3);
 }
 
-template <int CPL> struct VecF;
-template <> struct VecF<1> { using T = float; };
-template <> struct VecF<2> { using T = float2; };
-
-template <int CPL> __device__ __forceinline__ void ld_f(const float* p, float (&v)[CPL]) {
-  if constexpr (CPL == 2) { const float2 t = *reinterpret_cast<const float2*>(p); v[0] = t.x; v[1] = t.y; } else { v[0] = *p; }
-}
-template <int CPL> __device__ __forceinline__ void ldg_f(const float* p, float (&v)[CPL]) {
-  if constexpr (CPL == 2) { const float2 t = __ldg(reinterpret_cast<const float2*>(p)); v[0] = t.x; v[1] = t.y; } else { v[0] = __ldg(p); }
-}
-template <int CPL> __device__ __forceinline__ void st_f(float* p, const float (&v)[CPL]) {
-  if constexpr (CPL == 2) { *reinterpret_cast<float2*>(p) = make_float2(v[0], v[1]); } else { *p = v[0]; }
-}
-template <int CPL> __device__ __forceinline__ void st_h(__half* p, const float (&v)[CPL]) {
-  if constexpr (CPL == 2) { *reinterpret_cast<__half2*>(p) = __floats2half2_rn(v[0], v[1]); } else { *p = __float2half_rn(v[0]); }
-}
-template <int CPL> __device__ __forceinline__ void ld_h(const __half* p, float (&v)[CPL]) {
-  if constexpr (CPL == 2) { const float2 t = __half22float2(*reinterpret_cast<const __half2*>(p)); v[0] = t.x; v[1] = t.y; }
-  else { v[0] = __half2float(*p); }
-}
-
 __device__ __forceinline__ float warp_rowsum32(float (&part)[32], int lane) {
 #pragma unroll
   for (int o = 16; o >= 1; o >>= 1) {
@@ -290,20 +269,14 @@
 template <int EPI, int W, int ACT>
 __device__ __forceinline__ void epilogue_rows_impl(const GemmParams& p, int g, int row0, int lane, int col_base,
                                                    const float* __restrict__ stage, float mean_l, float rstd_l) {
-  constexpr int LPR = W / 8;
+  constexpr int PW = W == 96 ? 32 : W;
+  constexpr int LPR = PW / 8;
   constexpr int RPS = 32 / LPR;
   constexpr int STEPS = 32 / RPS;
   constexpr bool GLOBAL_IN = (EPI == EPI_RESID_F || EPI == EPI_PATCH || EPI == EPI_CONV || EPI == EPI_LN);
   constexpr int U = GLOBAL_IN ? 2 : 4;
-  static_assert(W % 8 == 0 && 32 % LPR == 0 && STEPS % U == 0, "staged epilogue: W in {32, 64}");
+  static_assert(W % PW == 0 && 32 % LPR == 0 && STEPS % U == 0, "staged epilogue: W in {32, 64, 96}");
   const int seg = lane % LPR, rsub = lane / LPR;
-  const int col = col_base + seg * 8;
-  float bias[8], gam[8], bet[8];
-#pragma unroll
-  for (int i = 0; i < 8; ++i) { bias[i] = 0.f; gam[i] = 1.f; bet[i] = 0.f; }
-  if constexpr (EPI == EPI_STORE_H || EPI == EPI_CONV) { if (p.bias) ldg8(p.bias + (size_t)g * p.bias_group_off + col, bias); }
-  if constexpr (EPI == EPI_RESID_F) { ldg8(p.bias + col, bias); ldg8(p.gamma + col, gam); }
-  if constexpr (EPI == EPI_LN) { ldg8(p.gamma + (size_t)g * p.ln_group_off + col, gam); ldg8(p.beta + (size_t)g * p.ln_group_off + col, bet); }
   const bool use_aux = (EPI == EPI_CONV) && p.aux && ((p.aux_group_mask >> g) & 1);
   const bool use_res = (EPI == EPI_CONV) && p.res_h;
   const bool ln_res = (EPI == EPI_LN) && p.out_f;
@@ -320,85 +293,95 @@
       my_orow = img * (p.tok_per_img + 1) + 1 + my_pos;
     }
   }
-  float* out_f = p.out_f ? p.out_f + (size_t)g * p.out_f_group_off + col : nullptr;
-  __half* out_h = p.out_h ? p.out_h + (size_t)g * p.out_h_group_off + col : nullptr;
 #pragma unroll 1
-  for (int s0 = 0; s0 < STEPS; s0 += U) {
-    float v[U][8], x[U][8], a[U][8];
-    int pos[U], orow[U];
-    bool valid[U], live[U];
-    float mean[U], rstd[U];
-#pragma unroll
-    for (int u = 0; u < U; ++u) {
-      const int r = (s0 + u) * RPS + rsub;
-      const size_t m = (size_t)(row0 + r);
-      live[u] = r < rows;
-      {
-        const float4 a = *reinterpret_cast<const float4*>(stage + acc_idx<W>(r, seg * 8));
-        const float4 b = *reinterpret_cast<const float4*>(stage + acc_idx<W>(r, seg * 8 + 4));
-        v[u][0] = a.x; v[u][1] = a.y; v[u][2] = a.z; v[u][3] = a.w; v[u][4] = b.x; v[u][5] = b.y; v[u][6] = b.z; v[u][7] = b.w;
+  for (int c0 = 0; c0 < W; c0 += PW) {
+    const int col = col_base + c0 + seg * 8;
+    float bias[8], gam[8], bet[8];
+#pragma unroll
+    for (int i = 0; i < 8; ++i) { bias[i] = 0.f; gam[i] = 1.f; bet[i] = 0.f; }
+    if constexpr (EPI == EPI_STORE_H || EPI == EPI_CONV) { if (p.bias) ldg8(p.bias + (size_t)g * p.bias_group_off + col, bias); }
+    if constexpr (EPI == EPI_RESID_F) { ldg8(p.bias + col, bias); ldg8(p.gamma + col, gam); }
+    if constexpr (EPI == EPI_LN) { ldg8(p.gamma + (size_t)g * p.ln_group_off + col, gam); ldg8(p.beta + (size_t)g * p.ln_group_off + col, bet); }
+    float* out_f = p.out_f ? p.out_f + (size_t)g * p.out_f_group_off + col : nullptr;
+    __half* out_h = p.out_h ? p.out_h + (size_t)g * p.out_h_group_off + col : nullptr;
+#pragma unroll 1
+    for (int s0 = 0; s0 < STEPS; s0 += U) {
+      float v[U][8], x[U][8], a[U][8];
+      int pos[U], orow[U];
+      bool valid[U], live[U];
+      float mean[U], rstd[U];
+#pragma unroll
+      for (int u = 0; u < U; ++u) {
+        const int r = (s0 + u) * RPS + rsub;
+        const size_t m = (size_t)(row0 + r);
+        live[u] = r < rows;
+        {
+          const float4 a = *reinterpret_cast<const float4*>(stage + acc_idx<W>(r, c0 + seg * 8));
+          const float4 b = *reinterpret_cast<const float4*>(stage + acc_idx<W>(r, c0 + seg * 8 + 4));
+          v[u][0] = a.x; v[u][1] = a.y; v[u][2] = a.z; v[u][3] = a.w; v[u][4] = b.x; v[u][5] = b.y; v[u][6] = b.z; v[u][7] = b.w;
+        }
+        pos[u] = __shfl_sync(0xffffffffu, my_pos, r);
+        orow[u] = __shfl_sync(0xffffffffu, my_orow, r);
+        valid[u] = __shfl_sync(0xffffffffu, my_valid, r) != 0;
+        mean[u] = 0.f; rstd[u] = 0.f;
+        if constexpr (EPI == EPI_LN) { mean[u] = __shfl_sync(0xffffffffu, mean_l, r); rstd[u] = __shfl_sync(0xffffffffu, rstd_l, r); }
+#pragma unroll
+        for (int k = 0; k < 8; ++k) { x[u][k] = 0.f; a[u][k] = 0.f; }
+        if (live[u]) {
+          if constexpr (EPI == EPI_RESID_F) ld8(out_f + m * p.out_f_ld, x[u]);
+          if constexpr (EPI == EPI_PATCH) ldg8(p.aux + (size_t)pos[u] * p.N + col, a[u]);
+          if constexpr (EPI == EPI_CONV) {
+            if (use_res) ld8h(p.res_h + (size_t)g * p.res_h_group_off + m * p.res_h_ld + col, x[u]);
+            if (use_aux) ldg8(p.aux + (size_t)pos[u] * p.N + col, a[u]);
+          }
+          if constexpr (EPI == EPI_LN) { if (ln_res) ld8(out_f + m * p.out_f_ld, x[u]); }
+        }
       }
-      pos[u] = __shfl_sync(0xffffffffu, my_pos, r);
-      orow[u] = __shfl_sync(0xffffffffu, my_orow, r);
-      valid[u] = __shfl_sync(0xffffffffu, my_valid, r) != 0;
-      mean[u] = 0.f; rstd[u] = 0.f;
-      if constexpr (EPI == EPI_LN) { mean[u] = __shfl_sync(0xffffffffu, mean_l, r); rstd[u] = __shfl_sync(0xffffffffu, rstd_l, r); }
-#pragma unroll
-      for (int k = 0; k < 8; ++k) { x[u][k] = 0.f; a[u][k] = 0.f; }
-      if (live[u]) {
-        if constexpr (EPI == EPI_RESID_F) ld8(out_f + m * p.out_f_ld, x[u]);
-        if constexpr (EPI == EPI_PATCH) ldg8(p.aux + (size_t)pos[u] * p.N + col, a[u]);
-        if constexpr (EPI == EPI_CONV) {
-          if (use_res) ld8h(p.res_h + (size_t)g * p.res_h_group_off + m * p.res_h_ld + col, x[u]);
-          if (use_aux) ldg8(p.aux + (size_t)pos[u] * p.N + col, a[u]);
+#pragma unroll
+      for (int u = 0; u < U; ++u) {
+        if (!live[u]) continue;
+        const int r = (s0 + u) * RPS + rsub;
+        const size_t m = (size_t)(row0 + r);
+        if constexpr (EPI == EPI_STORE_H) {
+          if constexpr (ACT == ACT_GELU) {
+#pragma unroll
+            for (int k = 0; k < 8; k += 2) gelu_erf2(v[u][k] + bias[k], v[u][k + 1] + bias[k + 1], v[u][k], v[u][k + 1]);
+          } else {
+#pragma unroll
+            for (int k = 0; k < 8; ++k) {
+              const float t = v[u][k] + bias[k];
+              v[u][k] = (ACT == ACT_RELU) ? fmaxf(t, 0.f) : t;
+            }
+          }
+          st8h(out_h + m * p.out_h_ld, v[u]);
+        } else if constexpr (EPI == EPI_RESID_F) {
+#pragma unroll
+          for (int k = 0; k < 8; ++k) x[u][k] = fmaf(gam[k], v[u][k] + bias[k], x[u][k]);
+          st8(out_f + m * p.out_f_ld, x[u]);
+        } else if constexpr (EPI == EPI_PATCH) {
+#pragma unroll
+          for (int k = 0; k < 8; ++k) v[u][k] += a[u][k];
+          st8(out_f + (size_t)orow[u] * p.out_f_ld, v[u]);
+        } else if constexpr (EPI == EPI_CONV) {
+#pragma unroll
+          for (int k = 0; k < 8; ++k) {
+            float t = v[u][k] + bias[k] + x[u][k];
+            t = ((ACT == ACT_RELU) ? fmaxf(t, 0.f) : ((ACT == ACT_GELU) ? gelu_erf(t) : t)) + a[u][k];
+            v[u][k] = valid[u] ? t : 0.f;
+          }
+          if (out_f) st8(out_f + m * p.out_f_ld, v[u]);
+          if (out_h) st8h(out_h + m * p.out_h_ld, v[u]);
+        } else if constexpr (EPI == EPI_STORE_F) {
+          st8(out_f + m * p.out_f_ld, v[u]);
+        } else if constexpr (EPI == EPI_LN) {
+#pragma unroll
+          for (int k = 0; k < 8; ++k) {
+            const float t = (v[u][k] - mean[u]) * rstd[u] * gam[k] + bet[k] + x[u][k];
+            v[u][k] = valid[u] ? t : 0.f;
+          }
+          if (ln_res) st8(out_f + m * p.out_f_ld, v[u]);
+          st8h(out_h + m * p.out_h_ld, v[u]);
         }
-        if constexpr (EPI == EPI_LN) { if (ln_res) ld8(out_f + m * p.out_f_ld, x[u]); }
-      }
-    }
-#pragma unroll
-    for (int u = 0; u < U; ++u) {
-      if (!live[u]) continue;
-      const int r = (s0 + u) * RPS + rsub;
-      const size_t m = (size_t)(row0 + r);
-      if constexpr (EPI == EPI_STORE_H) {
-        if constexpr (ACT == ACT_GELU) {
-#pragma unroll
-          for (int k = 0; k < 8; k += 2) gelu_erf2(v[u][k] + bias[k], v[u][k + 1] + bias[k + 1], v[u][k], v[u][k + 1]);
-        } else {
-#pragma unroll
-          for (int k = 0; k < 8; ++k) {
-            const float t = v[u][k] + bias[k];
-            v[u][k] = (ACT == ACT_RELU) ? fmaxf(t, 0.f) : t;
-          }
-        }
-        st8h(out_h + m * p.out_h_ld, v[u]);
-      } else if constexpr (EPI == EPI_RESID_F) {
-#pragma unroll
-        for (int k = 0; k < 8; ++k) x[u][k] = fmaf(gam[k], v[u][k] + bias[k], x[u][k]);
-        st8(out_f + m * p.out_f_ld, x[u]);
-      } else if constexpr (EPI == EPI_PATCH) {
-#pragma unroll
-        for (int k = 0; k < 8; ++k) v[u][k] += a[u][k];
-        st8(out_f + (size_t)orow[u] * p.out_f_ld, v[u]);
-      } else if constexpr (EPI == EPI_CONV) {
-#pragma unroll
-        for (int k = 0; k < 8; ++k) {
-          float t = v[u][k] + bias[k] + x[u][k];
-          t = ((ACT == ACT_RELU) ? fmaxf(t, 0.f) : ((ACT == ACT_GELU) ? gelu_erf(t) : t)) + a[u][k];
-          v[u][k] = valid[u] ? t : 0.f;
-        }
-        if (out_f) st8(out_f + m * p.out_f_ld, v[u]);
-        if (out_h) st8h(out_h + m * p.out_h_ld, v[u]);
-      } else if constexpr (EPI == EPI_STORE_F) {
-        st8(out_f + m * p.out_f_ld, v[u]);
-      } else if constexpr (EPI == EPI_LN) {
-#pragma unroll
-        for (int k = 0; k < 8; ++k) {
-          const float t = (v[u][k] - mean[u]) * rstd[u] * gam[k] + bet[k] + x[u][k];
-          v[u][k] = valid[u] ? t : 0.f;
-        }
-        if (ln_res) st8(out_f + m * p.out_f_ld, v[u]);
-        st8h(out_h + m * p.out_h_ld, v[u]);
       }
     }
   }
diff --git a/mickey_b200/csrc/gemm.cu b/mickey_b200/csrc/gemm.cu
--- a/mickey_b200/csrc/gemm.cu
+++ b/mickey_b200/csrc/gemm.cu
@@ -225,7 +225,7 @@
   constexpr int smem = gemm_smem_bytes<BN, EPI, STAGES, PERSISTENT>();
   auto kernel = gemm_tc_kernel<BN, EPI, STAGES, PERSISTENT, PAIR>;
   cudaLaunchConfig_t cfg = {};
-  cfg.blockDim = dim3(gemm_threads<PERSISTENT>()); cfg.dynamicSmemBytes = smem; cfg.stream = stream;
+  cfg.blockDim = dim3(gemm_threads<PERSISTENT, BN>()); cfg.dynamicSmemBytes = smem; cfg.stream = stream;
   cudaLaunchAttribute attr[2];
   int n_attr = 0;
   if constexpr (EPI == EPI_RESID_LN || PAIR) {
@@ -263,7 +263,7 @@
 static bool deep_ring(int tiles, const GemmParams& p) {
   return (long long)tiles <= (long long)sm_count() * 5 / 4 && p.k_chunks > 3;
 }
-static bool persistent_grid(int tiles) { return tiles > 8 * sm_count(); }
+static bool persistent_grid(long long tiles, int sms) { return tiles > 8LL * sms; }
 
 template <int BN, int EPI>
 static int launch_one(const GemmOperand& A, const GemmOperand& B, const GemmParams& p, cudaStream_t stream, int impl) {
@@ -272,7 +272,7 @@
     if (impl == GEMM_IMPL_SIMT || BN != 128 || p.N / BN > 8 || p.groups != 1) { set_last_error("EPI_RESID_LN: wgmma path, N <= 1024, one group"); return MK_ERR_UNSUPPORTED; }
   }
   if (impl == GEMM_IMPL_SIMT) {
-    if constexpr (EPI != EPI_RESID_LN)
+    if constexpr (EPI != EPI_RESID_LN && BN != 192)
     MK_CUDA_CHECK(launch_k(gemm_simt_kernel<BN, EPI>, dim3(tiles), dim3(128), 0, stream, reinterpret_cast<const __half*>(A.ptr),
                            (long long)A.rows, (long long)A.ld, reinterpret_cast<const __half*>(B.ptr), (long long)B.rows,
                            (long long)B.ld, p));
@@ -281,28 +281,30 @@
     int rc = make_tensor_map_f16(&tmA, A.ptr, A.rows, A.cols, A.ld, BLOCK_M);
     if (rc) return rc;
     if constexpr (persistent_epilogue<EPI>()) {
-      const bool forced = impl == GEMM_IMPL_TC_PAIRED || impl == GEMM_IMPL_TC_UNPAIRED;
-      if (forced || persistent_grid(tiles)) {
-        const bool pair = impl != GEMM_IMPL_TC_UNPAIRED;
+      const bool forced = BN == 192 || impl == GEMM_IMPL_TC_PAIRED || impl == GEMM_IMPL_TC_UNPAIRED;
+      if (forced || persistent_grid(tiles, sm_count())) {
+        const bool pair = impl != GEMM_IMPL_TC_UNPAIRED && impl != GEMM_IMPL_TC_UNPAIRED_192;
         rc = make_tensor_map_f16(&tmB, B.ptr, B.rows, B.cols, B.ld, pair ? BN / 2 : BN);
         if (rc) return rc;
         if (pair) return launch_tc<BN, EPI, ring_stages<BN>(), true, true>(tmA, tmB, p, stream);
         return launch_tc<BN, EPI, ring_stages<BN>(), true>(tmA, tmB, p, stream);
       }
     }
-    rc = make_tensor_map_f16(&tmB, B.ptr, B.rows, B.cols, B.ld, BN);
-    if (rc) return rc;
-    if constexpr (EPI == EPI_DUAL) {
-      if (p.out_tma) {
-        OutMaps om = {};
-        float* outs[3] = {p.scores, p.kp_scores, p.final_scores};
-        for (int i = 0; i < 3; ++i)
-          if (outs[i]) { rc = encode_tensor_map_out_f32(&om.m[i], outs[i], p.n_valid, p.out_pitch, p.groups); if (rc) return rc; }
-        return launch_tc<BN, EPI, shallow_stages<BN>(), false>(tmA, tmB, p, stream, om);
+    if constexpr (BN != 192) {
+      rc = make_tensor_map_f16(&tmB, B.ptr, B.rows, B.cols, B.ld, BN);
+      if (rc) return rc;
+      if constexpr (EPI == EPI_DUAL) {
+        if (p.out_tma) {
+          OutMaps om = {};
+          float* outs[3] = {p.scores, p.kp_scores, p.final_scores};
+          for (int i = 0; i < 3; ++i)
+            if (outs[i]) { rc = encode_tensor_map_out_f32(&om.m[i], outs[i], p.n_valid, p.out_pitch, p.groups); if (rc) return rc; }
+          return launch_tc<BN, EPI, shallow_stages<BN>(), false>(tmA, tmB, p, stream, om);
+        }
       }
-    }
-    if (deep_ring(tiles, p)) return launch_tc<BN, EPI, deep_stages<BN>(), false>(tmA, tmB, p, stream);
-    return launch_tc<BN, EPI, shallow_stages<BN>(), false>(tmA, tmB, p, stream);
+      if (deep_ring(tiles, p)) return launch_tc<BN, EPI, deep_stages<BN>(), false>(tmA, tmB, p, stream);
+      return launch_tc<BN, EPI, shallow_stages<BN>(), false>(tmA, tmB, p, stream);
+    }
   }
   MK_CUDA_CHECK(cudaGetLastError());
   return MK_OK;
@@ -310,6 +312,7 @@
 
 template <int EPI>
 static int launch_bn(int bn, const GemmOperand& A, const GemmOperand& B, const GemmParams& p, cudaStream_t s, int impl) {
+  if constexpr (EPI == EPI_STORE_H || EPI == EPI_RESID_F) { if (bn == 192) return launch_one<192, EPI>(A, B, p, s, impl); }
   if (bn == 128) return launch_one<128, EPI>(A, B, p, s, impl);
   if (bn == 64) return launch_one<64, EPI>(A, B, p, s, impl);
   set_last_error("unsupported BLOCK_N %d", bn);
@@ -321,6 +324,21 @@
   static int on = -1;
   if (on < 0) { const char* e = getenv("MICKEY_FUSE_LN"); on = (e && e[0] == '1') ? 1 : 0; }
   return on && !use_simt() && N % 128 == 0 && N <= 1024;
+}
+
+int gemm_block_n(int epi, const GemmParams& p, int impl, int sms) {
+  if (impl == GEMM_IMPL_DEFAULT) impl = use_simt() ? GEMM_IMPL_SIMT : GEMM_IMPL_TC;
+  const bool matcher = (epi == EPI_LSE || epi == EPI_DUAL);
+  const int bn = (matcher || p.N % 128 == 0) ? 128 : 64;
+  const bool wide_ok = (epi == EPI_STORE_H || epi == EPI_RESID_F) && p.N % 192 == 0;
+  if (impl == GEMM_IMPL_TC_PAIRED_192 || impl == GEMM_IMPL_TC_UNPAIRED_192) {
+    if (wide_ok) return 192;
+    set_last_error("GEMM: 192-wide tiles need EPI_STORE_H or EPI_RESID_F and N %% 192 == 0 (epi %d, N=%d)", epi, p.N);
+    return MK_ERR_UNSUPPORTED;
+  }
+  const long long tiles = (long long)((p.M + BLOCK_M - 1) / BLOCK_M) * ((p.N + bn - 1) / bn) * p.groups;
+  const bool wide_default = wide_ok && (epi == EPI_STORE_H || p.k_chunks >= 24);
+  return impl == GEMM_IMPL_TC && wide_default && persistent_grid(tiles, sms) ? 192 : bn;
 }
 
 int launch_gemm(int epi, const GemmOperand& A, const GemmOperand& B, const GemmParams& p, cudaStream_t stream, int impl) {
@@ -331,7 +349,8 @@
   if (matcher && (p.part_ld % 128 || p.part_ld < p.n_valid)) { set_last_error("matcher: part_ld must be n_valid rounded up to 128"); return MK_ERR_INVALID; }
   if (epi == EPI_DUAL && p.out_pitch < p.n_valid) { set_last_error("matcher: out_pitch %lld < n_valid %d", p.out_pitch, p.n_valid); return MK_ERR_INVALID; }
   if (!matcher && (p.N % 32)) { set_last_error("GEMM N=%d must be a multiple of 32", p.N); return MK_ERR_INVALID; }
-  int bn = (matcher || p.N % 128 == 0) ? 128 : 64;
+  const int bn = gemm_block_n(epi, p, impl, sm_count());
+  if (bn < 0) return bn;
   if (!matcher && p.N % bn) { set_last_error("GEMM N=%d not tileable", p.N); return MK_ERR_INVALID; }
   if (epi == EPI_LN && p.N != 128) { set_last_error("EPI_LN needs N == 128"); return MK_ERR_INVALID; }
   if (epi == EPI_RESID_LN && (p.N % 128 || p.N > 1024 || p.groups != 1 || !p.aux || !p.beta || !p.out_h || !p.out_f)) {
diff --git a/mickey_b200/csrc/gemm.h b/mickey_b200/csrc/gemm.h
--- a/mickey_b200/csrc/gemm.h
+++ b/mickey_b200/csrc/gemm.h
@@ -8,7 +8,8 @@
   long long rows, cols, ld;
 };
 
-enum GemmImpl : int { GEMM_IMPL_DEFAULT = 0, GEMM_IMPL_TC = 1, GEMM_IMPL_SIMT = 2, GEMM_IMPL_TC_PAIRED = 3, GEMM_IMPL_TC_UNPAIRED = 4 };
+enum GemmImpl : int { GEMM_IMPL_DEFAULT = 0, GEMM_IMPL_TC = 1, GEMM_IMPL_SIMT = 2, GEMM_IMPL_TC_PAIRED = 3, GEMM_IMPL_TC_UNPAIRED = 4,
+                      GEMM_IMPL_TC_PAIRED_192 = 5, GEMM_IMPL_TC_UNPAIRED_192 = 6 };
 
 int make_tensor_map_f16(CUtensorMap* map, const void* ptr, long long rows, long long cols, long long ld_elems, int box_rows);
 int encode_tensor_map_2d(CUtensorMap* map, CUtensorMapDataType dtype, const void* ptr, long long rows, long long cols,
@@ -17,6 +18,7 @@
 int sm_count();
 int launch_gemm(int epi, const GemmOperand& A, const GemmOperand& B, const GemmParams& p, cudaStream_t stream,
                 int impl = GEMM_IMPL_DEFAULT);
+int gemm_block_n(int epi, const GemmParams& p, int impl, int sms);
 bool gemm_resid_ln_supported(int M, int N, int k_chunks);
 const char* last_error();
 
diff --git a/mickey_b200/csrc/gemm_tc.cuh b/mickey_b200/csrc/gemm_tc.cuh
--- a/mickey_b200/csrc/gemm_tc.cuh
+++ b/mickey_b200/csrc/gemm_tc.cuh
@@ -9,12 +9,13 @@
 constexpr int WGMMA_K = 16;
 constexpr int GEMM_WARP_EPI = 8;
 
-template <int BN> constexpr int ring_stages() { return BN == 128 ? 4 : 6; }
+template <int BN> constexpr int ring_stages() { return BN == 192 ? 3 : BN == 128 ? 4 : 6; }
 template <int BN> constexpr int shallow_stages() { return BN == 128 ? 3 : 4; }
 template <int BN> constexpr int deep_stages() { return BN == 128 ? 6 : 8; }
 template <int EPI> constexpr bool persistent_epilogue() { return EPI != EPI_DUAL && EPI != EPI_RESID_LN && EPI != EPI_LN; }
-template <bool PERSISTENT> constexpr int gemm_threads() { return PERSISTENT ? 640 : 288; }
-template <bool PERSISTENT> constexpr int gemm_warp_tma() { return PERSISTENT ? 16 : 8; }
+template <int BN> constexpr int gemm_epilogue_warps() { return BN == 192 ? 4 : 8; }
+template <bool PERSISTENT, int BN> constexpr int gemm_threads() { return PERSISTENT ? 32 * (12 + gemm_epilogue_warps<BN>()) : 288; }
+template <bool PERSISTENT, int BN> constexpr int gemm_warp_tma() { return PERSISTENT ? 8 + gemm_epilogue_warps<BN>() : 8; }
 
 constexpr int DUAL_STAGE_BYTES = 3 * 4096;
 constexpr int DUAL_AUX_BYTES = 8 * 64 * 4;
@@ -144,9 +145,19 @@
       : "l"(desc_a), "l"(desc_b), "r"(scale_d));
 }
 
+__device__ __forceinline__ void wgmma_m64n192k16(float (&d)[96], uint64_t desc_a, uint64_t desc_b, uint32_t scale_d) {
+  asm volatile(
+      "{\n\t.reg .pred p;\n\tsetp.ne.b32 p, %98, 0;\n\t"
+      "wgmma.mma_async.sync.aligned.m64n192k16.f32.f16.f16 "
+      "{%0, %1, %2, %3, %4, %5, %6, %7, %8, %9, %10, %11, %12, %13, %14, %15, %16, %17, %18, %19, %20, %21, %22, %23, %24, %25, %26, %27, %28, %29, %30, %31, %32, %33, %34, %35, %36, %37, %38, %39, %40, %41, %42, %43, %44, %45, %46, %47, %48, %49, %50, %51, %52, %53, %54, %55, %56, %57, %58, %59, %60, %61, %62, %63, %64, %65, %66, %67, %68, %69, %70, %71, %72, %73, %74, %75, %76, %77, %78, %79, %80, %81, %82, %83, %84, %85, %86, %87, %88, %89, %90, %91, %92, %93, %94, %95}, %96, %97, p, 1, 1, 0, 0;\n\t}"
+      : "+f"(d[0]), "+f"(d[1]), "+f"(d[2]), "+f"(d[3]), "+f"(d[4]), "+f"(d[5]), "+f"(d[6]), "+f"(d[7]), "+f"(d[8]), "+f"(d[9]), "+f"(d[10]), "+f"(d[11]), "+f"(d[12]), "+f"(d[13]), "+f"(d[14]), "+f"(d[15]), "+f"(d[16]), "+f"(d[17]), "+f"(d[18]), "+f"(d[19]), "+f"(d[20]), "+f"(d[21]), "+f"(d[22]), "+f"(d[23]), "+f"(d[24]), "+f"(d[25]), "+f"(d[26]), "+f"(d[27]), "+f"(d[28]), "+f"(d[29]), "+f"(d[30]), "+f"(d[31]), "+f"(d[32]), "+f"(d[33]), "+f"(d[34]), "+f"(d[35]), "+f"(d[36]), "+f"(d[37]), "+f"(d[38]), "+f"(d[39]), "+f"(d[40]), "+f"(d[41]), "+f"(d[42]), "+f"(d[43]), "+f"(d[44]), "+f"(d[45]), "+f"(d[46]), "+f"(d[47]), "+f"(d[48]), "+f"(d[49]), "+f"(d[50]), "+f"(d[51]), "+f"(d[52]), "+f"(d[53]), "+f"(d[54]), "+f"(d[55]), "+f"(d[56]), "+f"(d[57]), "+f"(d[58]), "+f"(d[59]), "+f"(d[60]), "+f"(d[61]), "+f"(d[62]), "+f"(d[63]), "+f"(d[64]), "+f"(d[65]), "+f"(d[66]), "+f"(d[67]), "+f"(d[68]), "+f"(d[69]), "+f"(d[70]), "+f"(d[71]), "+f"(d[72]), "+f"(d[73]), "+f"(d[74]), "+f"(d[75]), "+f"(d[76]), "+f"(d[77]), "+f"(d[78]), "+f"(d[79]), "+f"(d[80]), "+f"(d[81]), "+f"(d[82]), "+f"(d[83]), "+f"(d[84]), "+f"(d[85]), "+f"(d[86]), "+f"(d[87]), "+f"(d[88]), "+f"(d[89]), "+f"(d[90]), "+f"(d[91]), "+f"(d[92]), "+f"(d[93]), "+f"(d[94]), "+f"(d[95])
+      : "l"(desc_a), "l"(desc_b), "r"(scale_d));
+}
+
 template <int BN>
 __device__ __forceinline__ void wgmma_tile(float (&d)[BN / 2], uint64_t desc_a, uint64_t desc_b, uint32_t scale_d) {
-  if constexpr (BN == 128) wgmma_m64n128k16(d, desc_a, desc_b, scale_d);
+  if constexpr (BN == 192) wgmma_m64n192k16(d, desc_a, desc_b, scale_d);
+  else if constexpr (BN == 128) wgmma_m64n128k16(d, desc_a, desc_b, scale_d);
   else wgmma_m64n64k16(d, desc_a, desc_b, scale_d);
 }
 
@@ -281,10 +292,10 @@
 }
 
 template <int BN, int EPI, int STAGES, bool PERSISTENT, bool PAIR = false>
-__global__ void __launch_bounds__((gemm_threads<PERSISTENT>()), (gemm_ctas_per_sm<BN, EPI, STAGES, PERSISTENT>()))
+__global__ void __launch_bounds__((gemm_threads<PERSISTENT, BN>()), (gemm_ctas_per_sm<BN, EPI, STAGES, PERSISTENT>()))
 gemm_tc_kernel(const __grid_constant__ CUtensorMap tmA, const __grid_constant__ CUtensorMap tmB, const GemmParams p,
                const __grid_constant__ OutMaps om) {
-  static_assert(BN == 64 || BN == 128, "wgmma tiles: N = 64 or 128");
+  static_assert(BN == 64 || BN == 128 || (BN == 192 && PERSISTENT), "wgmma tiles: N = 64 or 128, or 192 (persistent)");
   static_assert(gemm_smem_bytes<BN, EPI, STAGES, PERSISTENT>() <= 227 * 1024, "GEMM: shared memory");
   extern __shared__ uint8_t smem_raw[];
   constexpr int A_BYTES = BLOCK_M * BLOCK_K * 2;
@@ -294,7 +305,8 @@
   static_assert(!PERSISTENT || persistent_epilogue<EPI>(), "this epilogue runs one tile per CTA");
   static_assert(!PAIR || PERSISTENT, "CTA pairs: persistent kernel only");
   constexpr bool ONE_TILE = !PERSISTENT;
-  constexpr int WARP_TMA = gemm_warp_tma<PERSISTENT>();
+  constexpr int WARP_TMA = gemm_warp_tma<PERSISTENT, BN>();
+  constexpr bool BUDGETS = PERSISTENT && BN != 192;
   constexpr int MT = PAIR ? 2 : 1;
   const int rank = PAIR ? (int)(blockIdx.x & 1) : 0;
   const int work0 = PAIR ? (int)(blockIdx.x >> 1) : (int)blockIdx.x;
@@ -323,7 +335,7 @@
       mbar_init(empty_bar0 + 8 * s, 8 * MT);
     }
     mbar_init(acc_full_bar, 256);
-    mbar_init(acc_empty_bar, 256);
+    mbar_init(acc_empty_bar, 32 * gemm_epilogue_warps<BN>());
     asm volatile("fence.mbarrier_init.release.cluster;" ::: "memory");
   }
   if constexpr (PAIR) cluster_sync_all();
@@ -331,7 +343,7 @@
   pdl_wait();
 
   if (warp >= WARP_TMA) {
-    if constexpr (!ONE_TILE) setmaxnreg_dec<GEMM_REGS_PRODUCER>();
+    if constexpr (BUDGETS) setmaxnreg_dec<GEMM_REGS_PRODUCER>();
     if (warp == WARP_TMA && elect_one()) {
       int stage = 0;
       uint32_t phase = 0;
@@ -400,8 +412,8 @@
       for (int j = 0; j < BN / 8; ++j) {
 #pragma unroll
         for (int h = 0; h < 2; ++h) {
-          const int r = r_base + 8 * h, c = 8 * j + 2 * (lane & 3);
-          float* dst = acc + ((r >> 5) + 4 * (c / W)) * acc_block_floats<BN>() + acc_idx<W>(r & 31, c % W);
+          const int r = r_base + 8 * h, c = 8 * (j % (W / 8)) + 2 * (lane & 3);
+          float* dst = acc + ((r >> 5) + 4 * (j / (W / 8))) * acc_block_floats<BN>() + acc_idx<W>(r & 31, c);
           *reinterpret_cast<float2*>(dst) = make_float2(d[4 * j + 2 * h], d[4 * j + 2 * h + 1]);
         }
       }
@@ -423,7 +435,7 @@
   }
 
   if constexpr (ONE_TILE) return;
-  setmaxnreg_inc<GEMM_REGS_EPILOGUE>();
+  if constexpr (BUDGETS) setmaxnreg_inc<GEMM_REGS_EPILOGUE>();
   const int ew = warp - GEMM_WARP_EPI;
   uint32_t acc_phase = 0;
   for (int t = work0; t < n_work; t += work_step) {
@@ -431,10 +443,11 @@
     mbar_wait(acc_full_bar, acc_phase);
     if (t + work_step >= n_work) pdl_trigger();
     if (tile.m0 < p.M)
-      tile_epilogue<BN, EPI>(p, om, tile.g, tile.m0, tile.n0, tile.n_tile, ew & 3, ew >> 2, lane, acc,
-                             reinterpret_cast<float*>(smem_raw + (red_saddr - raw)), red_saddr,
-                             reinterpret_cast<float*>(gbase + ew * DUAL_STAGE_BYTES),
-                             reinterpret_cast<float*>(gbase + 8 * DUAL_STAGE_BYTES) + ew * 64);
+      for (int half = ew >> 2; half < 2; half += gemm_epilogue_warps<BN>() / 4)
+        tile_epilogue<BN, EPI>(p, om, tile.g, tile.m0, tile.n0, tile.n_tile, ew & 3, half, lane, acc,
+                               reinterpret_cast<float*>(smem_raw + (red_saddr - raw)), red_saddr,
+                               reinterpret_cast<float*>(gbase + ew * DUAL_STAGE_BYTES),
+                               reinterpret_cast<float*>(gbase + 8 * DUAL_STAGE_BYTES) + ew * 64);
     mbar_arrive(acc_empty_bar);
     acc_phase ^= 1;
   }
```

Result: faster. 313.3 (median of 6 runs) (+2.5%).
